# zhuzhui-2000/mobilesuperresolution

Measured on AMD Instinct MI355X. Metric: HR megapixels/sec (WDSR-B x4, 48x48 LR patches), full training step, higher is better.
Workload: dtype bf16; 1 GPU; WDSR-B x4, 16 blocks / 24 units, 48x48 LR patches, batch 32 per GPU, fwd+L1+bwd+Adam; global_batch=32, parallelism=dp1

## Files before the change

include/sr_hotpath.h:

```cpp
#ifndef SR_HOTPATH_H
#define SR_HOTPATH_H
#include <stddef.h>
#include <stdint.h>

#ifdef __cplusplus
extern "C" {
#endif

typedef void* sr_stream_t;

#define SR_DTYPE_F32 0
#define SR_DTYPE_BF16 1

int sr_abi_version(void);

int sr_wdsr_block_fwd(const void* x, void* y, const void* wblob, const float* cinit,
                      int N, int H, int W, int F, int dtype, sr_stream_t stream);

int sr_wdsr_block2_fwd(const void* x, void* ya, void* yb, const void* wblob_a, const void* wblob_b,
                       const float* cinit_a, const float* cinit_b, void* tsave_a, void* tsave_b, int N, int H, int W,
                       int F, int dtype, sr_stream_t stream);

int sr_wdsr_block2_bwd_data(const void* xa, const void* xb, const void* dyb, void* dxb, void* dxa,
                            const void* wblob_a, const void* wblob_b, const float* cinit_a, const float* cinit_b,
                            void* dtsave_a, void* dtsave_b, int N, int H, int W, int F, int dtype, sr_stream_t stream);
int sr_wdsr_block_wgrad_saved(const void* x, const void* dy, const void* tsave, const void* dtsave,
                              const void* wblob, const float* cinit, float* partial_a, float* partial_b, int layers,
                              int wgs, int N, int H, int W, int F, int dtype, long x_ls, long dy_ls, long side_ls,
                              long w_ls, long c_ls, sr_stream_t stream);

int sr_wdsr_fwd_rs(const void* x, void* ya, void* yb, const void* wblob_a, const void* wblob_b, const float* cinit_a,
                   const float* cinit_b, void* tsave_a, void* tsave_b, int nblk, int N, int H, int W, int F, int dtype,
                   sr_stream_t stream);
int sr_wdsr_fwd_rs_repeat(void* x, void* ya, void* yb, const void* wblob_a, const void* wblob_b, const float* cinit_a,
                          const float* cinit_b, void* tsave_a, void* tsave_b, int nblk, int N, int H, int W, int F, int dtype,
                          int reps, sr_stream_t stream);

int sr_wdsr_block_fwd_repeat(void* x, void* y, const void* wblob, const float* cinit,
                             int N, int H, int W, int F, int dtype, int reps, sr_stream_t stream);
int sr_wdsr_block2_fwd_repeat(void* x, void* ya, void* yb, const void* wblob_a, const void* wblob_b,
                              const float* cinit_a, const float* cinit_b, int N, int H, int W, int F, int dtype,
                              int reps, sr_stream_t stream);


int sr_wdsr_block_bwd_data(const void* x, const void* dy, void* dx, const void* wblob, const float* cinit,
                           int N, int H, int W, int F, int dtype, sr_stream_t stream);

int sr_wdsr_block_wgrad(const void* x, const void* dy, const void* wblob, const float* cinit,
                        float* partial_a, float* partial_b, int layers, int wgs_per_layer,
                        int N, int H, int W, int F, int dtype,
                        long x_ls, long dy_ls, long w_ls, long c_ls, sr_stream_t stream);
int sr_wdsr_block_slab_sizes(int F, int* slab_a, int* slab_b);

int sr_head_fwd(const float* x_nchw, void* y, const void* wblob, float mean, int N, int H, int W, int F,
                int dtype, sr_stream_t stream);
int sr_tail_fwd(const void* feat, const float* x_nchw, float* out, const void* wblob, float mean,
                int N, int H, int W, int F, int R, int dtype, sr_stream_t stream);
int sr_tail_bwd_data(const float* dout, void* dfeat, const void* wblob, int N, int H, int W, int F, int R,
                     int dtype, sr_stream_t stream);
int sr_tail_wgrad(const float* dout, const void* feat, const float* x_nchw, float mean, float* partial,
                  int wgs, int N, int H, int W, int F, int R, int dtype, sr_stream_t stream);
int sr_tail_bwd(const float* dout, const void* feat, const float* x, float mean, const void* wblob, void* dfeat,
                float* partial, int wgs, int N, int H, int W, int F, int R, int dtype, sr_stream_t stream);
int sr_head_wgrad(const void* dy0, const float* x_nchw, float mean, float* partial, int wgs,
                  int N, int H, int W, int F, int dtype, sr_stream_t stream);

int sr_c3_fwd(const void* x, const void* res, void* y, const void* wblob, int N, int H, int W, int CI, int act,
              int dtype, sr_stream_t stream);
int sr_c3_bwd_data(const void* dA, const void* A, const void* add, void* dx, const void* wblob, int N, int H,
                   int W, int CI, int act, int dtype, sr_stream_t stream);
int sr_c3_wgrad(const void* x, const void* dA, const void* A, float* partial, int wgs, int N, int H, int W,
                int CI, int act, int dtype, sr_stream_t stream);

typedef struct sr_c3_warp {
  const float* frame; long frame_bs;
  const void* state;
  const float* flow; long flow_bs;
  const float* flow_bound;
  void* dstate;
  float* dflow; long dflow_bs;
  void* x0_save;
} sr_c3_warp_t;

typedef struct sr_c3_unpack {
  const int* sidx0; const int* dst0; int n0;
  const int* sidx1; const int* dst1; int n1;
  float* gflat;
} sr_c3_unpack_t;

int sr_c3_trunk_fwd(const void* x0, const sr_c3_warp_t* warp, void* acts, void* mids, const void* blob,
                    const long* blob_off, int nb, int N, int H, int W, int ci0, int dtype, int n_dir, long blob_dir_stride,
                    sr_stream_t stream);
int sr_c3_trunk_bwd(const void* x0, const sr_c3_warp_t* warp, const void* acts, const void* mids, void* ga, void* gt,
                    const void* blob, const long* blob_off, float* parts, void* dx0, const sr_c3_unpack_t* unpack, int nb,
                    int wgs, int N, int H, int W, int ci0, int dtype, int n_dir, long blob_dir_stride, sr_stream_t stream);

int sr_c64_trunk_fwd(const void* x0, const sr_c3_warp_t* warp, void* ping, void* pong, void* out, const void* blob,
                     const long* blob_off, int nb, int N, int H, int W, int ci0, int dtype, int n_dir, long blob_dir_stride,
                     sr_stream_t stream);

int sr_c64_recon_fwd(const void* feat_b, const void* feat_f, int cw, const float* frame, long frame_bs, const void* blob,
                     const long* blob_off, void* fused, void* up1, void* up2, void* hr, float* out, long out_bs, int N, int H,
                     int W, int dtype, int stages, sr_stream_t stream);

int sr_mv_recon_fwd(const void* const* feat_b, const void* const* feat_f, int cw, const float* x, long x_bs, long x_fs,
                    const void* blob, float* out, long out_bs, long out_fs, void* u_save, int NF, int B, int H, int W, int dtype,
                    sr_stream_t stream);
int sr_mv_recon_bwd(const void* const* feat_b, const void* const* feat_f, const void* u_save, const float* g, long g_bs, long g_fs,
                    const void* blob, void* const* dfeat_b, void* const* dfeat_f, float* parts, int wgs, float* grads, int F, int NF,
                    int B, int H, int W, int dtype, sr_stream_t stream);
int sr_mv_recon_slab(void);

int sr_rm_block_fwd(const void* x, void* y, unsigned* mask, const void* wp, const float* bias, int N, int H, int W, int F, int K,
                    int dtype, sr_stream_t stream);
int sr_rm_block_bwd_data(const void* dy, const unsigned* mask, void* dx, const void* wpt, int N, int H, int W, int F, int K,
                         int dtype, sr_stream_t stream);
int sr_rm_wgrad(const void* g, const unsigned* mask, const void* xin, float* partial, int wgs, int N, int H, int W, int CA, int CB,
                int K, int dtype, sr_stream_t stream);
int sr_rm_tail_fwd(const void* feat, float* out, const void* wp, int N, int H, int W, int F, int R, int K, int dtype,
                   sr_stream_t stream);
int sr_rm_unshuffle(const float* dout, void* dconv, int N, int H, int W, int R, int dtype, sr_stream_t stream);
int sr_rm_tail_bwd_data(const void* dconv, void* dfeat, const void* wpt, int N, int H, int W, int F, int R, int K, int dtype,
                        sr_stream_t stream);

typedef struct sr_patch_rec {
  long lr_off, hr_off;
  int lr_w, hr_w;
  int x, y;
  int flags;
  int pad_;
} sr_patch_rec_t;
int sr_patch_gather(const unsigned char* cache, const void* recs, float* lr_out, float* hr_out, int B, int P, int scale,
                    sr_stream_t stream);

int sr_bicubic_resize_u8(const unsigned char* img, unsigned char* out_u8, float* out_f32, float* src_f32, int H, int W, int scale,
                         const double* wr, const int* ir, int taps_r, const double* wc, const int* ic, int taps_c,
                         sr_stream_t stream);

typedef struct sr_bicubic_rec {
  long hr_off;
  int hr_w;
  int x, y;
  int flags;
} sr_bicubic_rec_t;
int sr_bicubic_patch_gather(const unsigned char* cache, const void* recs, float* lr_out, float* hr_out, int B, int P, int scale,
                            int ig, const double* w, const int* idx, int taps, sr_stream_t stream);

typedef struct sr_clip_rec {
  long ids_off;
  int x, y;
  int flags;
  int T;
} sr_clip_rec_t;
typedef struct sr_clip_frame {
  long lr_off, hr_off;
  long mv_off;
  int lr_w, hr_w;
} sr_clip_frame_t;
int sr_clip_gather(const unsigned char* cache, const float* mv_cache, const void* frames, const int* ids, const void* recs,
                   float* lr_out, float* hr_out, int B, int T, int P, int scale, sr_stream_t stream);

int sr_psnr(const float* sr, const float* hr, float* partial, float* out, int N, int C, int H, int W, int shave, int luma,
            int wgs, sr_stream_t stream);

int sr_ssim(const float* sr, const float* hr, double* partial, double* out, int N, int H, int W, int shave, long n_partial,
            sr_stream_t stream);

int sr_eval_clip(const float* sr, const float* lr, const float* hr, float* partial, float* out, int F, int H, int W, int h,
                 int w, int lr_channels, int shave, int align_corners, int wgs, sr_stream_t stream);

int sr_eval_u8(const float* src, unsigned char* out, int F, int H, int W, int h, int w, int src_channels, int from_lr,
               int align_corners, sr_stream_t stream);

int sr_eval_variation(const float* lr, float* partial, float* out, int B, int N, int C, int h, int w, int wgs,
                      sr_stream_t stream);

int sr_flow_warp_fwd(const float* x, const float* flow, float* out, int N, int C, int H, int W, sr_stream_t stream);
int sr_flow_warp_bwd(const float* x, const float* flow, const float* gout, float* dx, float* dflow, int N, int C,
                     int H, int W, sr_stream_t stream);

int sr_nas_dw_fwd(const void* yin, void* V, const float* dwp, int N, int H, int W, int F, int dtype, sr_stream_t stream);
int sr_nas_pw_fwd(const void* yin, const void* V, void* y, const void* frags, const float* tabs, const float* scal,
                  int N, int H, int W, int F, int dtype, sr_stream_t stream);
int sr_nas_pw_bwd(const void* yin, const void* V, const void* gy, void* GZ, const void* frags, const float* tabs,
                  const float* scal, float* partial, int wgs, int N, int H, int W, int F, int dtype,
                  sr_stream_t stream);
int sr_nas_dw_bwd(const void* yin, const void* GZ, const void* gy, void* gyin, const float* dwp, float* partial,
                  int wgs, int N, int H, int W, int F, int dtype, sr_stream_t stream);
int sr_nas_dw_wgrad(const void* yin, const void* GZ, const float* dwp, float* partial, int wgs, int N, int H, int W,
                    int F, int dtype, sr_stream_t stream);

int sr_nas_scalars(const float* mask_w, const float* split_w, const float* alpha, const float* alpha1, const float* alpha2,
                   int nb, int F, float* out, float* src, long src_stride, int off_mg, float* scal, sr_stream_t stream);
int sr_nas_mask_grads(const float* dsrc, long ds, int off_r, int off_sxy, int off_sA, int off_sB, const float* ms, const float* p,
                      const float* beta, int nb, int F, float* out, sr_stream_t stream);
int sr_nas_body_fwd(void* ys, void* V, const float* dwp, long dwp_bs, const void* frags, long frags_bs, const float* tabs,
                    long tabs_bs, const float* scal, long scal_bs, int nb, int N, int H, int W, int F, int dtype,
                    int split, sr_stream_t stream);
int sr_nas_body_bwd(const void* ys, const void* V, const void* g_out, void* g_tmp0, void* g_tmp1, void* GZ, const float* dwp,
                    long dwp_bs, const void* frags, long frags_bs, const float* tabs, long tabs_bs, const float* scal,
                    long scal_bs, float* part_pw, long pw_bs, float* part_dw, long dw_bs, int wgs, int nb, int N, int H, int W,
                    int F, int dtype, int split, void** g_in, sr_stream_t stream);

typedef struct { const int* idx; void* out; long src_off, src_stride; int n, reps, as_float; } sr_pack_seg_t;
typedef struct { const float* partial; const int* sidx; const int* dst; long dst_off, dst_stride, slab; int wgs, n, reps; } sr_unpack_seg_t;
int sr_param_pack(const float* flat, float* src, const int* chan_tab, int n_chan, const int* bias_tab, const float* bias_const,
                  int n_bias, const sr_pack_seg_t* segs, int nseg, int dtype, sr_stream_t stream);
int sr_param_grads(const float* flat, float* dsrc, float* gflat, const int* chan_tab, int n_chan, const int* bias_tab,
                   int n_bias, const sr_unpack_seg_t* segs, int nseg, sr_stream_t stream);

typedef struct {
  int F, NB, R, dtype, N, H, W;
  float mean;
  const float* flat; float* gflat;
  const int* chan_tab; int n_chan;
  const int* bias_tab; const float* bias_const; int n_bias;
  float* src; float* dsrc;
  long src_head_off, src_body_off, src_body_stride, src_tail_off;
  const int* idx_head; int n_idx_head;
  const int* idx_body; int n_idx_body;
  const int* idx_cinit; int n_idx_cinit;
  const int* idx_tail; int n_idx_tail;
  void* blob_head; void* blob_body; float* cinit_body; void* blob_tail;
  float* part_a; float* part_b; float* part_tail; float* part_head;
  int wgs_body, wgs_tail, wgs_head;
  int slab_a, slab_b, slab_tail, slab_head;
  const int* ga_sidx; const int* ga_dst; int n_ga;
  const int* gb_sidx; const int* gb_dst; int n_gb;
  const int* gt_sidx; const int* gt_dst; int n_gt;
  const int* gh_sidx; const int* gh_dst; int n_gh;
  const float* x; void* acts; void* grads; float* out; const float* dout;
  void* tsave; void* dtsave;
  const float* hr; int loss_kind; float loss_gscale; float* loss_part;
  int nb_split, chan_split, bias_split;
  int adam_in_wn_bwd;
  int one_block32;
} sr_wdsr_net_t;

#define SR_NET_SAVE_ACTS 1
#define SR_NET_WEIGHTS_PACKED 2
#define SR_NET_PACK_ONLY 4
#define SR_NET_SKIP_TAIL 8
int sr_wdsr_net_forward(const sr_wdsr_net_t* net, int flags, sr_stream_t stream);
int sr_wdsr_net_backward(const sr_wdsr_net_t* net, sr_stream_t stream);
int sr_wdsr_net_backward_part(const sr_wdsr_net_t* net, int part, sr_stream_t stream);

int sr_pixel_shuffle(const float* in, float* out, int N, int C, int H, int W, int r, int inverse, sr_stream_t stream);

int sr_tail_bwd_loss(const float* sr, const float* hr, int loss_kind, float gscale, float* loss_part, const void* feat,
                     const float* x_nchw, float mean, const void* wblob, void* dfeat, float* partial, int wgs, int N, int H,
                     int W, int F, int R, int dtype, sr_stream_t stream);

int sr_tail_train(const float* hr, int loss_kind, float gscale, float* loss_part, const void* feat, const float* x_nchw, float mean,
                  const void* wblob, void* dfeat, float* partial, int wgs, int N, int H, int W, int F, int R, int dtype,
                  sr_stream_t stream);

typedef struct { float w_lerp, beta2, one_minus_beta2, bc2_sqrt, eps, neg_step_size; } sr_adam_t;
int sr_adam_step(float* param, const float* grad, float* exp_avg, float* exp_avg_sq, long n, const sr_adam_t* a,
                 const float* loss_part, int n_loss, float loss_scale, float* loss_out, sr_stream_t stream);
int sr_loss_value(const float* loss_part, int n_loss, float loss_scale, float* loss_out, sr_stream_t stream);
int sr_scale_by(void* y, const void* x, long n, const float* scale, int dtype, sr_stream_t stream);
int sr_wdsr_net_train_step(const sr_wdsr_net_t* net, float* exp_avg, float* exp_avg_sq, long n_params, const sr_adam_t* a,
                           float loss_scale, float* loss_out, sr_stream_t stream);

int sr_conv7_fwd(const void* x, const void* wpacked, const float* bias, void* y, int N, int H, int W, int CIN, int COUT, int relu,
                 int out_f32, sr_stream_t stream);

#define SR_FN_ENCODER 1
#define SR_FN_BLOCKS 2
#define SR_FN_LAST 4
#define SR_FN_UP 8
#define SR_FN_WRITE_D 16
#define SR_FN_ALL 15
int sr_fn_net_fwd(const float* frames, const void* blob, const long* conv_off, const void* head_blob, void* s0, void* s1, void* s2,
                  float* out, long out_is, int nb, int N, int H, int W, int dtype, int stages, sr_stream_t stream);

int sr_probe_mfma_bf16(const void* a_frag, const void* b_frag, float* acc_out, sr_stream_t stream);
int sr_probe_mfma_f32(const float* a_frag, const float* b_frag, float* acc_out, sr_stream_t stream);
int sr_probe_tr_read(const void* img_bf16, int n_elems, const int* lane_elem_off, void* out_bf16x4,
                     sr_stream_t stream);
int sr_probe_copy(const void* src, void* dst, size_t n_bytes, sr_stream_t stream);
int sr_probe_launch_floor(void* out, int gx, int gy, int threads, int lds_bytes, int reps, sr_stream_t stream);
int sr_probe_launch_floor_graph(void* out, int gx, int gy, int threads, int lds_bytes, int reps, int iters,
                                float* us_per_launch, float* host_us_per_graph );
int sr_debug_set_stamps(void* buf, long n_workgroups);

#ifdef __cplusplus
}
#endif
#endif
```

mobilesuperresolution_amd/_lib.py:

```python
from __future__ import annotations

import ctypes
import os
from ctypes import c_int, c_size_t, c_void_p

import torch

_HERE = os.path.dirname(os.path.abspath(__file__))
LIB_PATH = os.environ.get("SR_HOTPATH_LIB_PATH") or os.path.join(
    _HERE, "libsr_hotpath_dbg.so" if os.environ.get("SR_HOTPATH_DEBUG_LIB") == "1" else "libsr_hotpath.so")
ABI_VERSION = 23
DTYPE_CODE = {torch.float32: 0, torch.bfloat16: 1}
_HOT_DTYPES = {"fp32": torch.float32, "float32": torch.float32, "bf16": torch.bfloat16, "bfloat16": torch.bfloat16}


def hot_dtype(name=None) -> torch.dtype:
    name = name or os.environ.get("SR_HOT_DTYPE", "fp32")
    return name if isinstance(name, torch.dtype) else _HOT_DTYPES[str(name).lower()]


_P, _I, _Z, _L, _F = c_void_p, c_int, c_size_t, ctypes.c_long, ctypes.c_float
SIGNATURES = {
    "sr_abi_version": ([], _I),
    "sr_wdsr_block_fwd": ([_P, _P, _P, _P, _I, _I, _I, _I, _I, _P], _I),
    "sr_wdsr_block2_fwd": ([_P] * 9 + [_I] * 5 + [_P], _I),
    "sr_wdsr_fwd_rs": ([_P] * 9 + [_I] * 6 + [_P], _I),
    "sr_conv7_fwd": ([_P] * 4 + [_I] * 7 + [_P], _I),
    "sr_wdsr_fwd_rs_repeat": ([_P] * 9 + [_I] * 7 + [_P], _I),
    "sr_wdsr_block_wgrad_saved": ([_P] * 8 + [_I] * 7 + [_L] * 5 + [_P], _I),
    "sr_wdsr_block2_bwd_data": ([_P] * 11 + [_I] * 5 + [_P], _I),
    "sr_wdsr_block2_fwd_repeat": ([_P] * 7 + [_I] * 6 + [_P], _I),
    "sr_probe_launch_floor": ([_P, _I, _I, _I, _I, _I, _P], _I),
    "sr_probe_launch_floor_graph": ([_P, _I, _I, _I, _I, _I, _I, _P, _P], _I),
    "sr_debug_set_stamps": ([_P, _L], _I),
    "sr_c3_trunk_fwd": ([_P] * 6 + [_I] * 7 + [_L, _P], _I),
    "sr_c3_trunk_bwd": ([_P] * 11 + [_I] * 8 + [_L, _P], _I),
    "sr_c64_trunk_fwd": ([_P] * 7 + [_I] * 7 + [_L, _P], _I),
    "sr_c64_recon_fwd": ([_P, _P, _I, _P, _L, _P, _P, _P, _P, _P, _P, _P, _L] + [_I] * 5 + [_P], _I),
    "sr_mv_recon_fwd": ([_P, _P, _I, _P, _L, _L, _P, _P, _L, _L, _P] + [_I] * 5 + [_P], _I),
    "sr_mv_recon_bwd": ([_P, _P, _P, _P, _L, _L, _P, _P, _P, _P, _I, _P] + [_I] * 6 + [_P], _I),
    "sr_mv_recon_slab": ([], _I),
    "sr_tail_bwd": ([_P, _P, _P, _F, _P, _P, _P] + [_I] * 7 + [_P], _I),
    "sr_nas_dw_wgrad": ([_P, _P, _P, _P, _I, _I, _I, _I, _I, _I, _P], _I),
    "sr_wdsr_block_fwd_repeat": ([_P, _P, _P, _P, _I, _I, _I, _I, _I, _I, _P], _I),
    "sr_wdsr_block_bwd_data": ([_P, _P, _P, _P, _P, _I, _I, _I, _I, _I, _P], _I),
    "sr_wdsr_block_wgrad": ([_P, _P, _P, _P, _P, _P, _I, _I, _I, _I, _I, _I, _I, _L, _L, _L, _L, _P], _I),
    "sr_wdsr_block_slab_sizes": ([_I, _P, _P], _I),
    "sr_head_fwd": ([_P, _P, _P, _F, _I, _I, _I, _I, _I, _P], _I),
    "sr_tail_fwd": ([_P, _P, _P, _P, _F, _I, _I, _I, _I, _I, _I, _P], _I),
    "sr_tail_bwd_data": ([_P, _P, _P, _I, _I, _I, _I, _I, _I, _P], _I),
    "sr_tail_wgrad": ([_P, _P, _P, _F, _P, _I, _I, _I, _I, _I, _I, _I, _P], _I),
    "sr_head_wgrad": ([_P, _P, _F, _P, _I, _I, _I, _I, _I, _I, _P], _I),
    "sr_c3_fwd": ([_P, _P, _P, _P, _I, _I, _I, _I, _I, _I, _P], _I),
    "sr_c3_bwd_data": ([_P, _P, _P, _P, _P, _I, _I, _I, _I, _I, _I, _P], _I),
    "sr_c3_wgrad": ([_P, _P, _P, _P, _I, _I, _I, _I, _I, _I, _I, _P], _I),
    "sr_flow_warp_fwd": ([_P, _P, _P, _I, _I, _I, _I, _P], _I),
    "sr_flow_warp_bwd": ([_P, _P, _P, _P, _P, _I, _I, _I, _I, _P], _I),
    "sr_nas_dw_fwd": ([_P, _P, _P, _I, _I, _I, _I, _I, _P], _I),
    "sr_nas_pw_fwd": ([_P, _P, _P, _P, _P, _P, _I, _I, _I, _I, _I, _P], _I),
    "sr_nas_pw_bwd": ([_P, _P, _P, _P, _P, _P, _P, _P, _I, _I, _I, _I, _I, _I, _P], _I),
    "sr_nas_dw_bwd": ([_P, _P, _P, _P, _P, _P, _I, _I, _I, _I, _I, _I, _P], _I),
    "sr_patch_gather": ([_P, _P, _P, _P, _I, _I, _I, _P], _I),
    "sr_clip_gather": ([_P] * 7 + [_I] * 4 + [_P], _I),
    "sr_bicubic_resize_u8": ([_P] * 4 + [_I] * 3 + [_P, _P, _I, _P, _P, _I, _P], _I),
    "sr_bicubic_patch_gather": ([_P] * 4 + [_I] * 4 + [_P, _P, _I, _P], _I),
    "sr_param_pack": ([_P, _P, _P, _I, _P, _P, _I, _P, _I, _I, _P], _I),
    "sr_param_grads": ([_P, _P, _P, _P, _I, _P, _I, _P, _I, _P], _I),
    "sr_nas_scalars": ([_P] * 5 + [_I, _I, _P, _P, _L, _I, _P, _P], _I),
    "sr_nas_mask_grads": ([_P, _L, _I, _I, _I, _I, _P, _P, _P, _I, _I, _P, _P], _I),
    "sr_nas_body_fwd": ([_P, _P, _P, _L, _P, _L, _P, _L, _P, _L] + [_I] * 7 + [_P], _I),
    "sr_nas_body_bwd": ([_P] * 7 + [_L, _P, _L, _P, _L, _P, _L, _P, _L, _P, _L] + [_I] * 8 + [_P, _P], _I),
    "sr_psnr": ([_P, _P, _P, _P] + [_I] * 7 + [_P], _I),
    "sr_ssim": ([_P, _P, _P, _P] + [_I] * 4 + [_L, _P], _I),
    "sr_eval_clip": ([_P] * 5 + [_I] * 9 + [_P], _I),
    "sr_eval_u8": ([_P, _P] + [_I] * 8 + [_P], _I),
    "sr_eval_variation": ([_P] * 3 + [_I] * 6 + [_P], _I),
    "sr_pixel_shuffle": ([_P, _P, _I, _I, _I, _I, _I, _I, _P], _I),
    "sr_tail_bwd_loss": ([_P, _P, _I, _F, _P, _P, _P, _F, _P, _P, _P] + [_I] * 7 + [_P], _I),
    "sr_tail_train": ([_P, _I, _F, _P, _P, _P, _F, _P, _P, _P] + [_I] * 7 + [_P], _I),
    "sr_adam_step": ([_P, _P, _P, _P, _L, _P, _P, _I, _F, _P, _P], _I),
    "sr_loss_value": ([_P, _I, _F, _P, _P], _I),
    "sr_scale_by": ([_P, _P, _L, _P, _I, _P], _I),
    "sr_wdsr_net_train_step": ([_P, _P, _P, _L, _P, _F, _P, _P], _I),
    "sr_wdsr_net_forward": ([_P, _I, _P], _I),
    "sr_wdsr_net_backward": ([_P, _P], _I),
    "sr_wdsr_net_backward_part": ([_P, _I, _P], _I),
    "sr_probe_mfma_bf16": ([_P, _P, _P, _P], _I),
    "sr_probe_mfma_f32": ([_P, _P, _P, _P], _I),
    "sr_probe_tr_read": ([_P, _I, _P, _P, _P], _I),
    "sr_probe_copy": ([_P, _P, _Z, _P], _I),
    "sr_rm_block_fwd": ([_P] * 5 + [_I] * 6 + [_P], _I),
    "sr_rm_block_bwd_data": ([_P] * 4 + [_I] * 6 + [_P], _I),
    "sr_rm_wgrad": ([_P] * 4 + [_I] * 8 + [_P], _I),
    "sr_rm_tail_fwd": ([_P] * 3 + [_I] * 7 + [_P], _I),
    "sr_rm_unshuffle": ([_P, _P] + [_I] * 5 + [_P], _I),
    "sr_rm_tail_bwd_data": ([_P] * 3 + [_I] * 7 + [_P], _I),
    "sr_fn_net_fwd": ([_P] * 8 + [_L] + [_I] * 6 + [_P], _I),
}

class WdsrNet(ctypes.Structure):
    _fields_ = (
        [(n, _I) for n in ("F", "NB", "R", "dtype", "N", "H", "W")] + [("mean", _F)] +
        [("flat", _P), ("gflat", _P), ("chan_tab", _P), ("n_chan", _I),
         ("bias_tab", _P), ("bias_const", _P), ("n_bias", _I), ("src", _P), ("dsrc", _P)] +
        [(n, _L) for n in ("src_head_off", "src_body_off", "src_body_stride", "src_tail_off")] +
        [("idx_head", _P), ("n_idx_head", _I), ("idx_body", _P), ("n_idx_body", _I),
         ("idx_cinit", _P), ("n_idx_cinit", _I), ("idx_tail", _P), ("n_idx_tail", _I),
         ("blob_head", _P), ("blob_body", _P), ("cinit_body", _P), ("blob_tail", _P),
         ("part_a", _P), ("part_b", _P), ("part_tail", _P), ("part_head", _P)] +
        [(n, _I) for n in ("wgs_body", "wgs_tail", "wgs_head", "slab_a", "slab_b", "slab_tail", "slab_head")] +
        [("ga_sidx", _P), ("ga_dst", _P), ("n_ga", _I), ("gb_sidx", _P), ("gb_dst", _P), ("n_gb", _I),
         ("gt_sidx", _P), ("gt_dst", _P), ("n_gt", _I), ("gh_sidx", _P), ("gh_dst", _P), ("n_gh", _I),
         ("x", _P), ("acts", _P), ("grads", _P), ("out", _P), ("dout", _P), ("tsave", _P), ("dtsave", _P),
         ("hr", _P), ("loss_kind", _I), ("loss_gscale", _F), ("loss_part", _P),
         ("nb_split", _I), ("chan_split", _I), ("bias_split", _I), ("adam_in_wn_bwd", _I),
         ("one_block32", _I)])


class C3Warp(ctypes.Structure):
    _fields_ = [("frame", _P), ("frame_bs", _L), ("state", _P), ("flow", _P), ("flow_bs", _L), ("flow_bound", _P),
                ("dstate", _P), ("dflow", _P), ("dflow_bs", _L), ("x0_save", _P)]


class C3Unpack(ctypes.Structure):
    _fields_ = [("sidx0", _P), ("dst0", _P), ("n0", _I), ("sidx1", _P), ("dst1", _P), ("n1", _I), ("gflat", _P)]


class PackSeg(ctypes.Structure):
    _fields_ = [("idx", _P), ("out", _P), ("src_off", _L), ("src_stride", _L), ("n", _I), ("reps", _I), ("as_float", _I)]


class UnpackSeg(ctypes.Structure):
    _fields_ = [("partial", _P), ("sidx", _P), ("dst", _P), ("dst_off", _L), ("dst_stride", _L), ("slab", _L), ("wgs", _I),
                ("n", _I), ("reps", _I)]


class AdamScalars(ctypes.Structure):
    _fields_ = [(n, _F) for n in ("w_lerp", "beta2", "one_minus_beta2", "bc2_sqrt", "eps", "neg_step_size")]


_lib = None


class HotpathError(RuntimeError):
    pass


def _declare(lib):
    for name, (args, res) in SIGNATURES.items():
        fn = getattr(lib, name)
        fn.argtypes = args
        fn.restype = res


def lib():
    global _lib
    if _lib is None:
        if not os.path.exists(LIB_PATH):
            raise HotpathError(
                f"{LIB_PATH} not found: build it with `python -m mobilesuperresolution_amd.build` "
                "(the SR hot path has no CPU / ATen fallback)")
        if os.environ.get("SR_HOTPATH_LIB_PATH") or os.environ.get("SR_HOTPATH_DEBUG_LIB") == "1":
            import warnings
            warnings.warn(f"SR hot path: loading a NON-DEFAULT library ({LIB_PATH}) because SR_HOTPATH_LIB_PATH / "
                          "SR_HOTPATH_DEBUG_LIB is set (meant for tools/ only)", RuntimeWarning, stacklevel=2)
        l = ctypes.CDLL(LIB_PATH)
        _declare(l)
        if l.sr_abi_version() != ABI_VERSION:
            raise HotpathError(f"libsr_hotpath ABI {l.sr_abi_version()} != expected {ABI_VERSION}; rebuild")
        _lib = l
    return _lib


def stream_ptr(device=None) -> int:
    return torch.cuda.current_stream(device).cuda_stream


class _NoGuard:
    __slots__ = ()

    def __enter__(self):
        return self

    def __exit__(self, *exc):
        return False


_NOGUARD = _NoGuard()


def device_guard(device):
    idx = device.index
    if idx is None or idx == torch.cuda.current_device():
        return _NOGUARD
    return torch.cuda.device(idx)


def check(rc: int, what: str):
    if rc != 0:
        kind = {-1: "unsupported geometry/dtype", -2: "bad argument"}.get(rc, f"hipError_t {rc}")
        raise HotpathError(f"{what} failed: {kind}")


def ptr(t: torch.Tensor) -> int:
    if not t.is_cuda:
        raise HotpathError("SR hot path needs device tensors (no CPU fallback)")
    if not t.is_contiguous():
        raise HotpathError("SR hot path needs contiguous tensors")
    return t.data_ptr()


class KernelTimer:

    def __init__(self):
        self.events = {}

    def run(self, name, fn, *args):
        e0, e1 = torch.cuda.Event(enable_timing=True), torch.cuda.Event(enable_timing=True)
        e0.record()
        rc = fn(*args)
        e1.record()
        self.events.setdefault(name, []).append((e0, e1))
        return rc

    def summary(self):
        torch.cuda.synchronize()
        return {k: (len(v), sum(a.elapsed_time(b) for a, b in v) / len(v)) for k, v in self.events.items()}


_TIMER = None


def set_timer(t):
    global _TIMER
    _TIMER = t


def launch(name, fn, *args):
    rc = fn(*args) if _TIMER is None else _TIMER.run(name, fn, *args)
    check(rc, name)
```

mobilesuperresolution_amd/csrc/sr_abi.hip:

```cpp
#include <algorithm>
#include <cmath>
#include "../../include/sr_hotpath.h"
#include "wdsr_block.h"
#include "wdsr_fwd_rs.h"
#include "wdsr_fwd_stream.h"
#include "wdsr_bwd_rs.h"
#include "wdsr_bwd_pair_lds.h"
#include "wdsr_wgrad_rs.h"
#include "wdsr_ends.h"
#include "wdsr_prep.h"
#include "conv3x3.h"
#include "conv64.h"
#include "vsr_recon.h"
#include "mv_recon.h"
#include "spynet_conv.h"
#include "nas_block.h"
#include "nas_dw_lc.h"
#include "nas_bwd_fused.h"
#include "flow_warp.h"
#include "metrics.h"
#include "ssim.h"
#include "eval.h"
#include "patches.h"
#include "clips.h"
#include "bicubic.h"
#include "train_step.h"
#include "pixel_shuffle.h"
#include "result_block.h"
#include "frame_net.h"

extern "C" int sr_abi_version(void) { return 23; }

namespace {

template <int F_, int E_, int L_>
struct WdsrDimsOf {
  static constexpr int F = F_, E = E_, L = L_;
  typedef BlockCfg<F_, E_, L_> Cfg;
};
template <int F> struct WdsrDims;
template <> struct WdsrDims<24> : WdsrDimsOf<24, 144, 20> {};
template <> struct WdsrDims<32> : WdsrDimsOf<32, 192, 26> {};

template <typename Fn>
int dispatch_f(int F, Fn&& fn) {
  if (F == 24) return fn(WdsrDims<24>{});
  if (F == 32) return fn(WdsrDims<32>{});
  return -1;
}
template <typename Fn>
int dispatch_ft(int F, int dtype, Fn&& fn) {
  return dispatch_f(F, [&](auto d) {
    if (dtype == SR_DTYPE_BF16) return fn(d, __bf16{});
    if (dtype == SR_DTYPE_F32) return fn(d, float{});
    return -1;
  });
}

struct Tiles { int x, y; };
template <typename C = WdsrDims<24>::Cfg>
Tiles block_tiles(int H, int W) {
  return Tiles{(W + C::TW - 1) / C::TW, (H + C::TH - 1) / C::TH};
}

template <typename T, int F>
int launch_block_fwd(const void* x, void* y, const void* wblob, const float* cinit, int N, int H, int W,
                     hipStream_t st, void* tsave = nullptr) {
  typedef typename WdsrDims<F>::Cfg C;
  const auto [tiles_x, tiles_y] = block_tiles<C>(H, W);
  dim3 grid(tiles_x * tiles_y, N), block(64 * C::NPT_H);
  hipLaunchKernelGGL((wdsr_block_fwd_kernel<T, F, C::E, C::L>), grid, block, 0, st, (const T*)x, (T*)y, (const T*)wblob,
                     cinit, H, W, tiles_x, (T*)tsave);
  SR_HIP_CHECK_LAUNCH();
  return 0;
}

template <typename T, int F>
int launch_block_bwd_data(const void* x, const void* dy, void* dx, const void* wblob, const float* cinit, int N,
                          int H, int W, hipStream_t st, void* dtsave = nullptr) {
  typedef typename WdsrDims<F>::Cfg C;
  const auto [tiles_x, tiles_y] = block_tiles<C>(H, W);
  dim3 grid(tiles_x * tiles_y, N), block(64 * C::NPT_O);
  hipLaunchKernelGGL((wdsr_block_bwd_data_kernel<T, F, C::E, C::L>), grid, block, 0, st, (const T*)x, (const T*)dy, (T*)dx,
                     (const T*)wblob, cinit, H, W, tiles_x, (T*)dtsave);
  SR_HIP_CHECK_LAUNCH();
  return 0;
}

template <typename T, int F>
int launch_block_wgrad(const void* x, const void* dy, const void* wblob, const float* cinit, float* pa, float* pb,
                       int layers, int wgs, int N, int H, int W, long x_ls, long dy_ls, long w_ls, long c_ls,
                       hipStream_t st) {
  typedef typename WdsrDims<F>::Cfg C;
  const auto [tiles_x, tiles_y] = block_tiles<C>(H, W);
  dim3 grid(wgs, layers);
  hipLaunchKernelGGL((wdsr_block_wgrad_kernel<T, F, C::E, C::L, 0>), grid, dim3(64 * WgradCfg<F, C::E, C::L, 0>::NWAVES), 0, st,
                     (const T*)x, (const T*)dy, (const T*)wblob, cinit, pa, N, H, W, tiles_x, tiles_x * tiles_y, x_ls,
                     dy_ls, w_ls, c_ls);
  hipLaunchKernelGGL((wdsr_block_wgrad_kernel<T, F, C::E, C::L, 1>), grid, dim3(64 * WgradCfg<F, C::E, C::L, 1>::NWAVES), 0, st,
                     (const T*)x, (const T*)dy, (const T*)wblob, cinit, pb, N, H, W, tiles_x, tiles_x * tiles_y, x_ls,
                     dy_ls, w_ls, c_ls);
  SR_HIP_CHECK_LAUNCH();
  return 0;
}

}

static bool fwd_stream_applies(long N, int H, int W) {
  if (W != 48 || H % 4 != 0 || H < 8 || H > 4096 || N < 256) return false;
  const long rounds = (N + 255) / 256;
  return N * 10 >= rounds * 256 * 7;
}

template <int F, int NBLK>
static int launch_fwd_rs16(const void* x, void* ya, void* yb, const void* wa, const void* wb, const float* cia, const float* cib,
                           void* tsa, void* tsb, int N, int H, int W, hipStream_t st) {
  typedef typename WdsrDims<F>::Cfg C;
  typedef __bf16 T;
  constexpr int E = C::E, L = C::L;
  const auto [tiles_x, tiles_y] = block_tiles<C>(H, W);
  if (tsa && (NBLK == 1 || tsb))
    hipLaunchKernelGGL((wdsr_fwd_rs16_kernel<F, E, L, NBLK, true>), dim3(tiles_x * tiles_y, N), dim3(1024), 0, st, (const T*)x, (T*)ya,
                       (T*)yb, (const T*)wa, (const T*)wb, cia, cib, (T*)tsa, (T*)tsb, H, W, tiles_x);
  else
    hipLaunchKernelGGL((wdsr_fwd_rs16_kernel<F, E, L, NBLK, false>), dim3(tiles_x * tiles_y, N), dim3(1024), 0, st, (const T*)x, (T*)ya,
                       (T*)yb, (const T*)wa, (const T*)wb, cia, cib, (T*)tsa, (T*)tsb, H, W, tiles_x);
  SR_HIP_CHECK_LAUNCH();
  return 0;
}

template <int F, int NBLK>
static int launch_fwd_rs(const void* x, void* ya, void* yb, const void* wa, const void* wb, const float* cia, const float* cib,
                         void* tsa, void* tsb, int N, int H, int W, hipStream_t st) {
  typedef typename WdsrDims<F>::Cfg C;
  typedef __bf16 T;
  constexpr int E = C::E, L = C::L;
  const auto [tiles_x, tiles_y] = block_tiles<C>(H, W);
  constexpr int persist_from = 768;
  const long total = (long)N * tiles_x * tiles_y;
  if constexpr (NBLK == 2) {
    if (fwd_stream_applies(N, H, W)) {
      if (tsa && tsb)
        hipLaunchKernelGGL((wdsr_fwd_stream12_kernel<F, E, L, true>), dim3(256), dim3(768), 0, st, (const T*)x, (T*)ya, (T*)yb, (const T*)wa,
                           (const T*)wb, cia, cib, (T*)tsa, (T*)tsb, N, H);
      else
        hipLaunchKernelGGL((wdsr_fwd_stream12_kernel<F, E, L, false>), dim3(256), dim3(768), 0, st, (const T*)x, (T*)ya, (T*)yb, (const T*)wa,
                           (const T*)wb, cia, cib, (T*)nullptr, (T*)nullptr, N, H);
      SR_HIP_CHECK_LAUNCH();
      return 0;
    }
  }
  if (total >= persist_from && total < (1L << 31)) {
    const int wgs = 256;
    const bool save = tsa && (NBLK == 1 || tsb);
    if (save && NBLK == 1) {
      hipLaunchKernelGGL((wdsr_fwd_rs_persist_kernel<F, E, L, 1, true>), dim3(wgs), dim3(512), 0, st, (const T*)x, (T*)ya, (T*)yb,
                         (const T*)wa, (const T*)wb, cia, cib, (T*)tsa, (T*)tsb, N, H, W, tiles_x, tiles_x * tiles_y);
      SR_HIP_CHECK_LAUNCH();
      return 0;
    }
    if constexpr (NBLK == 2) {
      if (!save) {
        hipLaunchKernelGGL((wdsr_fwd_rs_pipe_kernel<F, E, L>), dim3(wgs), dim3(512), 0, st, (const T*)x, (T*)ya, (T*)yb, (const T*)wa,
                           (const T*)wb, cia, cib, N, H, W, tiles_x, tiles_x * tiles_y);
        SR_HIP_CHECK_LAUNCH();
        return 0;
      }
    } else if (!save) {
      hipLaunchKernelGGL((wdsr_fwd_rs_persist_kernel<F, E, L, 1, false>), dim3(wgs), dim3(512), 0, st, (const T*)x, (T*)ya, (T*)yb,
                         (const T*)wa, (const T*)wb, cia, cib, (T*)tsa, (T*)tsb, N, H, W, tiles_x, tiles_x * tiles_y);
      SR_HIP_CHECK_LAUNCH();
      return 0;
    }
  }
  if (tsa && (NBLK == 1 || tsb))
    hipLaunchKernelGGL((wdsr_fwd_rs_kernel<F, E, L, NBLK, true>), dim3(tiles_x * tiles_y, N), dim3(512), 0, st, (const T*)x, (T*)ya,
                       (T*)yb, (const T*)wa, (const T*)wb, cia, cib, (T*)tsa, (T*)tsb, H, W, tiles_x);
  else
    hipLaunchKernelGGL((wdsr_fwd_rs_kernel<F, E, L, NBLK, false>), dim3(tiles_x * tiles_y, N), dim3(512), 0, st, (const T*)x, (T*)ya,
                       (T*)yb, (const T*)wa, (const T*)wb, cia, cib, (T*)tsa, (T*)tsb, H, W, tiles_x);
  SR_HIP_CHECK_LAUNCH();
  return 0;
}
template <int F, int NBLK>
static int launch_fwd_rs_any(const void* x, void* ya, void* yb, const void* wa, const void* wb, const float* cia, const float* cib,
                             void* tsa, void* tsb, int N, int H, int W, hipStream_t st) {
  if constexpr (F == 24) return launch_fwd_rs<F, NBLK>(x, ya, yb, wa, wb, cia, cib, tsa, tsb, N, H, W, st);
  else return launch_fwd_rs16<F, NBLK>(x, ya, yb, wa, wb, cia, cib, tsa, tsb, N, H, W, st);
}
extern "C" int sr_wdsr_fwd_rs(const void* x, void* ya, void* yb, const void* wa, const void* wb, const float* cia,
                              const float* cib, void* tsa, void* tsb, int nblk, int N, int H, int W, int F, int dtype,
                              sr_stream_t stream) {
  if (!x || !yb || !wa || !cia || N <= 0 || H <= 0 || W <= 0 || N > 65535 || (nblk == 2 && (!wb || !cib))) return -2;
  if (dtype != SR_DTYPE_BF16) return -1;
  hipStream_t st = (hipStream_t)stream;
  return dispatch_f(F, [&](auto d) {
    if (nblk == 2) return launch_fwd_rs_any<decltype(d)::F, 2>(x, ya, yb, wa, wb, cia, cib, tsa, tsb, N, H, W, st);
    if (nblk == 1) return launch_fwd_rs_any<decltype(d)::F, 1>(x, nullptr, yb, wa, nullptr, cia, nullptr, tsa, nullptr, N, H, W, st);
    return -1;
  });
}
extern "C" int sr_wdsr_block2_fwd(const void* x, void* ya, void* yb, const void* wa, const void* wb, const float* cia,
                                  const float* cib, void* tsa, void* tsb, int N, int H, int W, int F, int dtype,
                                  sr_stream_t stream) {
  if (F != 24 && F != 32) return (!x || !yb || !wa || !wb || !cia || !cib || N <= 0 || H <= 0 || W <= 0 || N > 65535) ? -2 : -1;
  return sr_wdsr_fwd_rs(x, ya, yb, wa, wb, cia, cib, tsa, tsb, 2, N, H, W, F, dtype, stream);
}
extern "C" int sr_wdsr_fwd_rs_repeat(void* x, void* ya, void* yb, const void* wa, const void* wb, const float* cia,
                                     const float* cib, void* tsa, void* tsb, int nblk, int N, int H, int W, int F, int dtype,
                                     int reps, sr_stream_t stream) {
  for (int i = 0; i < reps; ++i) {
    const int rc = (i & 1) ? sr_wdsr_fwd_rs(yb, ya, x, wa, wb, cia, cib, tsa, tsb, nblk, N, H, W, F, dtype, stream)
                           : sr_wdsr_fwd_rs(x, ya, yb, wa, wb, cia, cib, tsa, tsb, nblk, N, H, W, F, dtype, stream);
    if (rc) return rc;
  }
  return 0;
}

extern "C" int sr_wdsr_block_fwd_repeat(void* x, void* y, const void* wblob, const float* cinit, int N, int H, int W,
                                        int F, int dtype, int reps, sr_stream_t stream) {
  for (int i = 0; i < reps; ++i) {
    const int rc = (i & 1) ? sr_wdsr_block_fwd(y, x, wblob, cinit, N, H, W, F, dtype, stream)
                           : sr_wdsr_block_fwd(x, y, wblob, cinit, N, H, W, F, dtype, stream);
    if (rc) return rc;
  }
  return 0;
}

extern "C" int sr_wdsr_block2_fwd_repeat(void* x, void* ya, void* yb, const void* wa, const void* wb, const float* cia,
                                         const float* cib, int N, int H, int W, int F, int dtype, int reps,
                                         sr_stream_t stream) {
  for (int i = 0; i < reps; ++i) {
    const int rc = (i & 1) ? sr_wdsr_block2_fwd(yb, ya, x, wa, wb, cia, cib, nullptr, nullptr, N, H, W, F, dtype, stream)
                           : sr_wdsr_block2_fwd(x, ya, yb, wa, wb, cia, cib, nullptr, nullptr, N, H, W, F, dtype, stream);
    if (rc) return rc;
  }
  return 0;
}

extern "C" int sr_wdsr_block_bwd_data(const void* x, const void* dy, void* dx, const void* wblob,
                                      const float* cinit, int N, int H, int W, int F, int dtype,
                                      sr_stream_t stream) {
  if (!x || !dy || !dx || !wblob || !cinit || N <= 0 || H <= 0 || W <= 0 || N > 65535) return -2;
  return dispatch_ft(F, dtype, [&](auto d, auto t) {
    return launch_block_bwd_data<decltype(t), decltype(d)::F>(x, dy, dx, wblob, cinit, N, H, W, (hipStream_t)stream);
  });
}

extern "C" int sr_wdsr_block2_bwd_data(const void* xa, const void* xb, const void* dyb, void* dxb, void* dxa,
                                       const void* wa, const void* wb, const float* cia, const float* cib, void* dta,
                                       void* dtb, int N, int H, int W, int F, int dtype, sr_stream_t stream) {
  if (!xa || !xb || !dyb || !dxb || !dxa || !wa || !wb || !cia || !cib || N <= 0 || H <= 0 || W <= 0 || N > 65535)
    return -2;
  if ((F != 24 && F != 32) || dtype != SR_DTYPE_BF16) return -1;
  const auto [tiles_x, tiles_y] = block_tiles(H, W);
  if (F == 32) {
    typedef WdsrDims<32> D;
    hipLaunchKernelGGL((wdsr_bwd_pair_lds_kernel<32, D::E, D::L>), dim3(tiles_x * tiles_y, N), dim3(BwdPairCfg<32, D::E, D::L>::NTHREADS),
                       0, (hipStream_t)stream, (const __bf16*)xa, (const __bf16*)xb, (const __bf16*)dyb, (__bf16*)dxb, (__bf16*)dxa,
                       (const __bf16*)wa, (const __bf16*)wb, cia, cib, (__bf16*)dta, (__bf16*)dtb, H, W, tiles_x);
  } else {
    typedef WdsrDims<24> D;
    hipLaunchKernelGGL((wdsr_bwd_rs_kernel<24, D::E, D::L>), dim3(tiles_x * tiles_y, N), dim3(512), 0, (hipStream_t)stream,
                       (const __bf16*)xa, (const __bf16*)xb, (const __bf16*)dyb, (__bf16*)dxb, (__bf16*)dxa, (const __bf16*)wa,
                       (const __bf16*)wb, (__bf16*)dta, (__bf16*)dtb, H, W, tiles_x);
  }
  SR_HIP_CHECK_LAUNCH();
  return 0;
}

extern "C" int sr_wdsr_block_wgrad(const void* x, const void* dy, const void* wblob, const float* cinit,
                                   float* pa, float* pb, int layers, int wgs, int N, int H, int W, int F,
                                   int dtype, long x_ls, long dy_ls, long w_ls, long c_ls, sr_stream_t stream) {
  if (!x || !dy || !wblob || !cinit || !pa || !pb || layers <= 0 || wgs <= 0 || N <= 0 || H <= 0 || W <= 0 ||
      layers > 65535)
    return -2;
  return dispatch_ft(F, dtype, [&](auto d, auto t) {
    return launch_block_wgrad<decltype(t), decltype(d)::F>(x, dy, wblob, cinit, pa, pb, layers, wgs, N, H, W, x_ls, dy_ls, w_ls, c_ls,
                                                           (hipStream_t)stream);
  });
}

namespace {
template <int F>
int launch_wgrad_saved(const void* x, const void* dy, const void* tsave, const void* dtsave, const void* wblob,
                       const float* cinit, float* pa, float* pb, int layers, int wgs, int N, int H, int W, long x_ls,
                       long dy_ls, long side_ls, long w_ls, long c_ls, hipStream_t st) {
  typedef typename WdsrDims<F>::Cfg C;
  typedef __bf16 T;
  constexpr int E = C::E, L = C::L;
  const auto [tiles_x, tiles_y] = block_tiles<C>(H, W);
  dim3 grid(wgs, layers);
  const bool old_a = (long)N * tiles_x * tiles_y * C::TH * C::TW >= (1L << 31);
  if constexpr (F == 24) {
    if (!old_a)
      hipLaunchKernelGGL((wdsr_wgrad_a8_kernel<F, E, L>), grid, dim3(WgradA8Cfg<F, E, L>::NTHREADS), 0, st, (const T*)x, (const T*)dtsave,
                         (const T*)wblob, pa, N, H, W, tiles_x, tiles_x * tiles_y, x_ls, side_ls, w_ls);
  }
  if (F != 24 || old_a)
    hipLaunchKernelGGL((wdsr_block_wgrad_saved_kernel<T, F, E, L, 0>), grid, dim3(64 * WgradSavedCfg<F, E, L>::NWAVES), 0, st,
                       (const T*)x, (const T*)dtsave, (const T*)wblob, cinit, pa, N, H, W, tiles_x, tiles_x * tiles_y, x_ls,
                       side_ls, w_ls, c_ls);
  hipLaunchKernelGGL((wdsr_wgrad_b8_kernel<F, E, L>), grid, dim3(WgradB8Cfg<F, E, L>::NTHREADS), 0, st, (const T*)dy, (const T*)tsave,
                     pb, N, H, W, tiles_x, tiles_x * tiles_y, dy_ls, side_ls);
  SR_HIP_CHECK_LAUNCH();
  return 0;
}
}

extern "C" int sr_wdsr_block_wgrad_saved(const void* x, const void* dy, const void* tsave, const void* dtsave,
                                         const void* wblob, const float* cinit, float* pa, float* pb, int layers, int wgs,
                                         int N, int H, int W, int F, int dtype, long x_ls, long dy_ls, long side_ls,
                                         long w_ls, long c_ls, sr_stream_t stream) {
  if (!x || !dy || !tsave || !dtsave || !wblob || !cinit || !pa || !pb || layers <= 0 || wgs <= 0 || N <= 0 || H <= 0 ||
      W <= 0 || layers > 65535)
    return -2;
  if (dtype != SR_DTYPE_BF16) return -1;
  return dispatch_f(F, [&](auto d) {
    return launch_wgrad_saved<decltype(d)::F>(x, dy, tsave, dtsave, wblob, cinit, pa, pb, layers, wgs, N, H, W, x_ls, dy_ls, side_ls,
                                                  w_ls, c_ls, (hipStream_t)stream);
  });
}

extern "C" int sr_wdsr_block_slab_sizes(int F, int* slab_a, int* slab_b) {
  if (!slab_a || !slab_b) return -2;
  return dispatch_f(F, [&](auto d) {
    typedef BwdCfg<typename decltype(d)::Cfg> B;
    *slab_a = B::SLAB_A;
    *slab_b = B::SLAB_B;
    return 0;
  });
}

extern "C" int sr_wdsr_block_fwd(const void* x, void* y, const void* wblob, const float* cinit, int N, int H,
                                 int W, int F, int dtype, sr_stream_t stream) {
  if (!x || !y || !wblob || !cinit || N <= 0 || H <= 0 || W <= 0 || N > 65535) return -2;
  return dispatch_ft(F, dtype, [&](auto d, auto t) {
    return launch_block_fwd<decltype(t), decltype(d)::F>(x, y, wblob, cinit, N, H, W, (hipStream_t)stream);
  });
}

namespace {
template <typename E> dim3 tile_grid(int N, int H, int W, int* tiles_x) {
  *tiles_x = (W + E::TW - 1) / E::TW;
  return dim3(*tiles_x * ((H + E::TH - 1) / E::TH), N);
}
#define SR_DISPATCH_TF(CALL)                                                     \
  if (F == 24 && dtype == SR_DTYPE_BF16) { CALL(__bf16, 24) }                    \
  else if (F == 24 && dtype == SR_DTYPE_F32) { CALL(float, 24) }                 \
  else if (F == 32 && dtype == SR_DTYPE_BF16) { CALL(__bf16, 32) }               \
  else if (F == 32 && dtype == SR_DTYPE_F32) { CALL(float, 32) }                 \
  else return -1;
#define SR_DISPATCH_R(CALL, T, F_)                                               \
  if (R == 4) { CALL(T, F_, 4) } else if (R == 2) { CALL(T, F_, 2) } else if (R == 3) { CALL(T, F_, 3) } else return -1;
// ... 556 lines not shown

extern "C" int sr_flow_warp_fwd(const float* x, const float* flow, float* out, int N, int C, int H, int W,
                                sr_stream_t stream) {
  if (!x || !flow || !out || N <= 0 || C <= 0 || H <= 0 || W <= 0 || N > 65535) return -2;
  const int blocks = std::min((H * W + 15) / 16, 8192);
  hipLaunchKernelGGL(flow_warp_fwd_kernel, dim3(blocks, N), dim3(64), 0, (hipStream_t)stream, x, flow, out, C, H, W);
  SR_HIP_CHECK_LAUNCH();
  return 0;
}
extern "C" int sr_flow_warp_bwd(const float* x, const float* flow, const float* gout, float* dx, float* dflow, int N,
                                int C, int H, int W, sr_stream_t stream) {
  if (!x || !flow || !gout || N <= 0 || C <= 0 || H <= 0 || W <= 0 || N > 65535) return -2;
  const int blocks = std::min((H * W + 15) / 16, 8192);
  hipLaunchKernelGGL(flow_warp_bwd_kernel, dim3(blocks, N), dim3(64), 0, (hipStream_t)stream, x, flow, gout, dx, dflow,
                     C, H, W);
  SR_HIP_CHECK_LAUNCH();
  return 0;
}

#define SR_NAS_DISPATCH(CALL)                                                                   \
  if (F == 24 && dtype == SR_DTYPE_BF16) { CALL(__bf16, 24) } else if (F == 24 && dtype == SR_DTYPE_F32) { CALL(float, 24) } \
  else if (F == 32 && dtype == SR_DTYPE_BF16) { CALL(__bf16, 32) } else if (F == 32 && dtype == SR_DTYPE_F32) { CALL(float, 32) } \
  else return -1;
#define SR_NAS_DISPATCH_F32(CALL)                                                               \
  if (F == 24 && dtype == SR_DTYPE_F32) { CALL(float, 24) } else if (F == 32 && dtype == SR_DTYPE_F32) { CALL(float, 32) } \
  else return -1;

extern "C" int sr_nas_dw_fwd(const void* yin, void* V, const float* dwp, int N, int H, int W, int F, int dtype,
                             sr_stream_t stream) {
  if (!yin || !V || !dwp || N <= 0 || H <= 0 || W <= 0 || N > 65535) return -2;
  hipStream_t st = (hipStream_t)stream;
  const long vs = (long)N * H * W * F;
  if (dtype == SR_DTYPE_BF16) {
    typedef NasCfg<24> C;
    const int tx = (W + C::TW - 1) / C::TW;
    dim3 g(tx * ((H + C::TH - 1) / C::TH), N);
    if (F == 24) hipLaunchKernelGGL((nas_dw_fwd_lc_kernel<24>), g, dim3(512), 0, st, (const __bf16*)yin, (__bf16*)V, dwp, H, W, tx, vs);
    else if (F == 32) hipLaunchKernelGGL((nas_dw_fwd_lc_kernel<32>), g, dim3(512), 0, st, (const __bf16*)yin, (__bf16*)V, dwp, H, W, tx, vs);
    else return -1;
    SR_HIP_CHECK_LAUNCH();
    return 0;
  }
#define CALL(T, F_) { typedef NasCfg<F_> C; const int tx = (W + C::TW - 1) / C::TW; dim3 g(tx * ((H + C::TH - 1) / C::TH), N); \
    hipLaunchKernelGGL((nas_dw_fwd_kernel<T, F_>), g, dim3(512), 0, st, (const T*)yin, (T*)V, dwp, H, W, tx, vs); }
  SR_NAS_DISPATCH_F32(CALL)
#undef CALL
  SR_HIP_CHECK_LAUNCH();
  return 0;
}
extern "C" int sr_nas_pw_fwd(const void* yin, const void* V, void* y, const void* frags, const float* tabs,
                             const float* scal, int N, int H, int W, int F, int dtype, sr_stream_t stream) {
  if (!yin || !V || !y || !frags || !tabs || !scal || N <= 0 || H <= 0 || W <= 0 || N > 65535) return -2;
  hipStream_t st = (hipStream_t)stream;
  const long vs = (long)N * H * W * F;
#define CALL(T, F_) { typedef NasCfg<F_> C; const int tx = (W + C::TW - 1) / C::TW; dim3 g(tx * ((H + C::TH - 1) / C::TH), N); \
    hipLaunchKernelGGL((nas_pw_fwd_kernel<T, F_>), g, dim3(576), 0, st, (const T*)yin, (const T*)V, (T*)y, (const T*)frags, tabs, scal, H, W, tx, vs); }
  SR_NAS_DISPATCH(CALL)
#undef CALL
  SR_HIP_CHECK_LAUNCH();
  return 0;
}
extern "C" int sr_nas_pw_bwd(const void* yin, const void* V, const void* gy, void* GZ, const void* frags,
                             const float* tabs, const float* scal, float* partial, int wgs, int N, int H, int W, int F,
                             int dtype, sr_stream_t stream) {
  if (!yin || !V || !gy || !GZ || !frags || !tabs || !scal || !partial || wgs <= 0 || N <= 0 || H <= 0 || W <= 0) return -2;
  hipStream_t st = (hipStream_t)stream;
  const long vs = (long)N * H * W * F;
#define CALL(T, F_) { typedef NasCfg<F_> C; const int tx = (W + C::TW - 1) / C::TW, tpi = tx * ((H + C::TH - 1) / C::TH); \
    hipLaunchKernelGGL((nas_pw_bwd_kernel<T, F_>), dim3(wgs), dim3(NasPwb<T>::THREADS), 0, st, (const T*)yin, (const T*)V, (const T*)gy, (T*)GZ, (const T*)frags, tabs, scal, partial, N, H, W, tx, tpi, vs); }
  SR_NAS_DISPATCH(CALL)
#undef CALL
  SR_HIP_CHECK_LAUNCH();
  return 0;
}
extern "C" int sr_nas_dw_bwd(const void* yin, const void* GZ, const void* gy, void* gyin, const float* dwp,
                             float* partial, int wgs, int N, int H, int W, int F, int dtype, sr_stream_t stream) {
  if (!yin || !GZ || !gy || !gyin || !dwp || !partial || wgs <= 0 || N <= 0 || H <= 0 || W <= 0) return -2;
  hipStream_t st = (hipStream_t)stream;
  const long vs = (long)N * H * W * F;
  if (dtype == SR_DTYPE_BF16) {
    typedef NasCfg<24> C;
    const int tx = (W + C::TW - 1) / C::TW, tpi = tx * ((H + C::TH - 1) / C::TH);
    if (F == 24) hipLaunchKernelGGL((nas_dw_bwd_lc_kernel<24>), dim3(wgs), dim3(NAS_DW_BWD_THREADS), 0, st, (const __bf16*)yin, (const __bf16*)GZ, (const __bf16*)gy, (__bf16*)gyin, dwp, partial, N, H, W, tx, tpi, vs);
    else if (F == 32) hipLaunchKernelGGL((nas_dw_bwd_lc_kernel<32>), dim3(wgs), dim3(NAS_DW_BWD_THREADS), 0, st, (const __bf16*)yin, (const __bf16*)GZ, (const __bf16*)gy, (__bf16*)gyin, dwp, partial, N, H, W, tx, tpi, vs);
    else return -1;
    SR_HIP_CHECK_LAUNCH();
    return 0;
  }
#define CALL(T, F_) { typedef NasCfg<F_> C; const int tx = (W + C::TW - 1) / C::TW, tpi = tx * ((H + C::TH - 1) / C::TH); \
    hipLaunchKernelGGL((nas_dw_bwd_kernel<T, F_>), dim3(wgs), dim3(512), 0, st, (const T*)yin, (const T*)GZ, (const T*)gy, (T*)gyin, dwp, partial, N, H, W, tx, tpi, vs); }
  SR_NAS_DISPATCH_F32(CALL)
#undef CALL
  SR_HIP_CHECK_LAUNCH();
  return 0;
}

extern "C" int sr_nas_dw_wgrad(const void* yin, const void* GZ, const float* dwp, float* partial, int wgs, int N, int H,
                               int W, int F, int dtype, sr_stream_t stream) {
  if (!yin || !GZ || !dwp || !partial || wgs <= 0 || N <= 0 || H <= 0 || W <= 0) return -2;
  hipStream_t st = (hipStream_t)stream;
  const long vs = (long)N * H * W * F;
  if (dtype == SR_DTYPE_BF16) {
    typedef NasCfg<24> C;
    const int tx = (W + C::TW - 1) / C::TW, tpi = tx * ((H + C::TH - 1) / C::TH);
    if (F == 24) hipLaunchKernelGGL((nas_dw_wgrad3_kernel<24>), dim3(wgs), dim3(768), 0, st, (const __bf16*)yin, (const __bf16*)GZ, dwp, partial, N, H, W, tx, tpi, vs);
    else if (F == 32) hipLaunchKernelGGL((nas_dw_wgrad3_kernel<32>), dim3(wgs), dim3(768), 0, st, (const __bf16*)yin, (const __bf16*)GZ, dwp, partial, N, H, W, tx, tpi, vs);
    else return -1;
    SR_HIP_CHECK_LAUNCH();
    return 0;
  }
#define CALL(T, F_) { typedef NasCfg<F_> C; const int tx = (W + C::TW - 1) / C::TW, tpi = tx * ((H + C::TH - 1) / C::TH); \
    hipLaunchKernelGGL((nas_dw_wgrad_kernel<T, F_>), dim3(wgs, 3), dim3(768), 0, st, (const T*)yin, (const T*)GZ, dwp, partial, N, H, W, tx, tpi, vs); }
  SR_NAS_DISPATCH_F32(CALL)
#undef CALL
  SR_HIP_CHECK_LAUNCH();
  return 0;
}

namespace {
template <typename T> int net_pack(const sr_wdsr_net_t* n, hipStream_t st) {
  const int cb = (n->n_chan + 3) / 4, bb = (n->n_bias + 255) / 256;
  hipLaunchKernelGGL(wn_src_kernel, dim3(cb + bb), dim3(256), 0, st, n->flat, n->src, (const int4*)n->chan_tab,
                     n->n_chan, n->bias_tab, n->bias_const, n->n_bias, cb);
  PackSegs ps;
  ps.nseg = 4;
  int blk = 0;
  auto add = [&](int k, const int* idx, void* out, long off, long stride, int cnt, int reps, int as_float) {
    ps.s[k] = PackSeg{idx, out, off, stride, cnt, reps, as_float, blk};
    blk += reps * ((cnt + 255) / 256);
  };
  add(0, n->idx_head, n->blob_head, n->src_head_off, 0, n->n_idx_head, 1, 0);
  add(1, n->idx_body, n->blob_body, n->src_body_off, n->src_body_stride, n->n_idx_body, n->NB, 0);
  add(2, n->idx_cinit, n->cinit_body, n->src_body_off, n->src_body_stride, n->n_idx_cinit, n->NB, 1);
  add(3, n->idx_tail, n->blob_tail, n->src_tail_off, 0, n->n_idx_tail, 1, 0);
  hipLaunchKernelGGL((pack_all_kernel<T>), dim3(blk), dim3(256), 0, st, n->src, ps);
  SR_HIP_CHECK_LAUNCH();
  return 0;
}
}

static bool net_saves_side_images(const sr_wdsr_net_t* n, bool backward) {
  return (n->F == 24 || n->F == 32) && n->dtype == SR_DTYPE_BF16 && n->tsave && (!backward || n->dtsave);
}
static long net_tiles(const sr_wdsr_net_t* n) {
  const Tiles t = block_tiles(n->H, n->W);
  return (long)n->N * t.x * t.y;
}
static bool net_uses_pairs(const sr_wdsr_net_t* n) {
  return n->dtype == SR_DTYPE_BF16 && net_tiles(n) <= 384 && (n->F == 24 || (n->F == 32 && !n->one_block32));
}
static bool net_step_fuses_tail(const sr_wdsr_net_t* n) {
  return n->dtype == SR_DTYPE_BF16 && n->R == 4 && (n->F == 24 || n->F == 32) && n->hr && n->N <= 65535;
}
static size_t side_image_bytes(const sr_wdsr_net_t* n) {
  typedef WdsrDims<24>::Cfg C;
  const Tiles t = block_tiles<C>(n->H, n->W);
  const int lp = n->F == 24 ? C::LP : WdsrDims<32>::Cfg::LP;
  return (size_t)n->N * ((size_t)t.x * t.y) * C::TH * C::TW * lp * 2;
}
struct NetView {
  const sr_wdsr_net_t* n;
  bool keeps_side;
  size_t esz = n->dtype == SR_DTYPE_BF16 ? 2 : 4;
  size_t act_bytes = (size_t)n->N * n->H * n->W * n->F * esz, blob_bytes = (size_t)n->n_idx_body * esz;
  size_t side_bytes = side_image_bytes(n);
  char* act(int i) const { return (char*)n->acts + (size_t)i * act_bytes; }
  char* grad(int i) const { return (char*)n->grads + (size_t)i * act_bytes; }
  char* blob(int i) const { return (char*)n->blob_body + (size_t)i * blob_bytes; }
  const float* cinit(int i) const { return n->cinit_body + (size_t)i * n->n_idx_cinit; }
  char* tsave(int i) const { return keeps_side ? (char*)n->tsave + (size_t)i * side_bytes : nullptr; }
  char* dtsave(int i) const { return keeps_side ? (char*)n->dtsave + (size_t)i * side_bytes : nullptr; }
};

extern "C" int sr_wdsr_net_forward(const sr_wdsr_net_t* n, int flags, sr_stream_t stream) {
  if (!n || !n->flat || !n->src) return -2;
  if (!(flags & SR_NET_PACK_ONLY) && (!n->x || !n->acts || !n->out)) return -2;
  hipStream_t st = (hipStream_t)stream;
  const int save_acts = flags & SR_NET_SAVE_ACTS;
  int rc = 0;
  if (!(flags & SR_NET_WEIGHTS_PACKED)) rc = n->dtype == SR_DTYPE_BF16 ? net_pack<__bf16>(n, st) : net_pack<float>(n, st);
  if (rc || (flags & SR_NET_PACK_ONLY)) return rc;
  const NetView v{n, save_acts && net_saves_side_images(n, false)};
  char* acts = v.act(0);
  if ((rc = sr_head_fwd(n->x, acts, n->blob_head, n->mean, n->N, n->H, n->W, n->F, n->dtype, stream))) return rc;
  char* cur = acts;
  const bool pairs = net_uses_pairs(n) || (n->F == 24 && n->dtype == SR_DTYPE_BF16 &&
                                           ((!save_acts && net_tiles(n) >= 768) || fwd_stream_applies(n->N, n->H, n->W)));
  for (int i = 0, nb; i < n->NB; i += nb) {
    nb = pairs && i + 1 < n->NB ? 2 : 1;
    char* nxt = save_acts ? v.act(i + nb) : (cur == acts ? v.act(1) : acts);
    if (nb == 2)
      rc = sr_wdsr_block2_fwd(cur, save_acts ? v.act(i + 1) : nullptr, nxt, v.blob(i), v.blob(i + 1), v.cinit(i), v.cinit(i + 1),
                              v.tsave(i), v.tsave(i + 1), n->N, n->H, n->W, n->F, n->dtype, stream);
    else if (pairs)
      rc = sr_wdsr_fwd_rs(cur, nullptr, nxt, v.blob(i), nullptr, v.cinit(i), nullptr, v.tsave(i), nullptr, 1, n->N, n->H, n->W, n->F,
                          n->dtype, stream);
    else if (v.keeps_side)
      rc = dispatch_f(n->F, [&](auto d) {
        return launch_block_fwd<__bf16, decltype(d)::F>(cur, nxt, v.blob(i), v.cinit(i), n->N, n->H, n->W, st, v.tsave(i));
      });
    else
      rc = sr_wdsr_block_fwd(cur, nxt, v.blob(i), v.cinit(i), n->N, n->H, n->W, n->F, n->dtype, stream);
    if (rc) return rc;
    cur = nxt;
  }
  if (flags & SR_NET_SKIP_TAIL) return 0;
  return sr_tail_fwd(cur, n->x, n->out, n->blob_tail, n->mean, n->N, n->H, n->W, n->F, n->R, n->dtype, stream);
}

namespace {
struct FusedAdam { float* m; float* v; AdamArgs a; const float* loss_part; int n_loss; float loss_scale; float* loss_out; };
}
static int net_backward_part_impl(const sr_wdsr_net_t* n, int part, sr_stream_t stream, const FusedAdam* fa, bool tail_train = false) {
  if (!n || !n->flat || !n->gflat || !n->dsrc || !n->x || !n->acts || !n->grads || part < 0 || part > 2) return -2;
  if (tail_train && (part != 0 || !n->hr)) return -2;
  if (part != 2 && (n->hr ? ((!n->out && !tail_train) || !n->loss_part || (n->loss_kind != 1 && n->loss_kind != 2)) : !n->dout)) return -2;
  hipStream_t st = (hipStream_t)stream;
  const long act_e = (long)n->N * n->H * n->W * n->F;
  const bool pairs = net_uses_pairs(n);
  const bool saved = net_saves_side_images(n, true);
  const NetView v{n, saved};
  int split = part == 0 ? 0 : n->nb_split;
  if (part != 0 && (split <= 0 || split >= n->NB || (pairs && ((n->NB - split) & 1)))) return -2;
  const int b0 = part == 1 ? split : 0, b1 = part == 2 ? split : n->NB;
  int rc;
  if (part != 2) {
    if (tail_train)
      rc = sr_tail_train(n->hr, n->loss_kind, n->loss_gscale, n->loss_part, v.act(n->NB), n->x, n->mean, n->blob_tail, v.grad(n->NB),
                         n->part_tail, n->wgs_tail, n->N, n->H, n->W, n->F, n->R, n->dtype, stream);
    else if (n->hr)
      rc = sr_tail_bwd_loss(n->out, n->hr, n->loss_kind, n->loss_gscale, n->loss_part, v.act(n->NB), n->x, n->mean, n->blob_tail,
                            v.grad(n->NB), n->part_tail, n->wgs_tail, n->N, n->H, n->W, n->F, n->R, n->dtype, stream);
    else if (n->dtype == SR_DTYPE_BF16)
      rc = sr_tail_bwd(n->dout, v.act(n->NB), n->x, n->mean, n->blob_tail, v.grad(n->NB), n->part_tail, n->wgs_tail, n->N, n->H, n->W,
                       n->F, n->R, n->dtype, stream);
    else if (!(rc = sr_tail_bwd_data(n->dout, v.grad(n->NB), n->blob_tail, n->N, n->H, n->W, n->F, n->R, n->dtype, stream)))
      rc = sr_tail_wgrad(n->dout, v.act(n->NB), n->x, n->mean, n->part_tail, n->wgs_tail, n->N, n->H, n->W, n->F, n->R, n->dtype,
                         stream);
    if (rc) return rc;
  }
  for (int i = b1 - 1, nb; i >= b0; i -= nb) {
    nb = pairs && i >= b0 + 1 ? 2 : 1;
    if (nb == 2)
      rc = sr_wdsr_block2_bwd_data(v.act(i - 1), v.act(i), v.grad(i + 1), v.grad(i), v.grad(i - 1), v.blob(i - 1), v.blob(i),
                                   v.cinit(i - 1), v.cinit(i), v.dtsave(i - 1), v.dtsave(i), n->N, n->H, n->W, n->F, n->dtype, stream);
    else if (saved)
      rc = dispatch_f(n->F, [&](auto d) {
        return launch_block_bwd_data<__bf16, decltype(d)::F>(v.act(i), v.grad(i + 1), v.grad(i), v.blob(i), v.cinit(i), n->N, n->H,
                                                                 n->W, st, v.dtsave(i));
      });
    else
      rc = sr_wdsr_block_bwd_data(v.act(i), v.grad(i + 1), v.grad(i), v.blob(i), v.cinit(i), n->N, n->H, n->W, n->F, n->dtype, stream);
    if (rc) return rc;
  }
  const int nl = b1 - b0;
  const int wgs_part = nl > 0 ? (n->wgs_body * n->NB) / nl : 0;
  if (nl > 0) {
    float* pa0 = n->part_a;
    float* pb0 = n->part_b;
    if (saved)
      rc = sr_wdsr_block_wgrad_saved(v.act(b0), v.grad(b0 + 1), v.tsave(b0), v.dtsave(b0), v.blob(b0), v.cinit(b0), pa0, pb0, nl,
                                     wgs_part, n->N, n->H, n->W, n->F, n->dtype, act_e, act_e, (long)(v.side_bytes / v.esz),
                                     (long)n->n_idx_body, (long)n->n_idx_cinit, stream);
    else
      rc = sr_wdsr_block_wgrad(v.act(b0), v.grad(b0 + 1), v.blob(b0), v.cinit(b0), pa0, pb0, nl, wgs_part, n->N, n->H, n->W, n->F,
                               n->dtype, act_e, act_e, (long)n->n_idx_body, (long)n->n_idx_cinit, stream);
    if (rc) return rc;
  }
  if (part != 1)
    if ((rc = sr_head_wgrad(v.grad(0), n->x, n->mean, n->part_head, n->wgs_head, n->N, n->H, n->W, n->F, n->dtype, stream)))
      return rc;
  {
    UnpackSegs us;
    us.nseg = 0;
    int blk = 0;
    auto add = [&](const float* part_, const int* sidx, const int* dst, long off, long stride, long slab, int wgs, int cnt,
                   int reps) {
      us.s[us.nseg++] = UnpackSeg{part_, sidx, dst, off, stride, slab, wgs, cnt, reps, blk};
      blk += reps * unpack_blocks(cnt, wgs);
    };
    if (nl > 0) {
      add(n->part_a, n->ga_sidx, n->ga_dst, n->src_body_off + b0 * n->src_body_stride, n->src_body_stride, n->slab_a, wgs_part,
          n->n_ga, nl);
      add(n->part_b, n->gb_sidx, n->gb_dst, n->src_body_off + b0 * n->src_body_stride, n->src_body_stride, n->slab_b, wgs_part,
          n->n_gb, nl);
    }
    if (part != 2) add(n->part_tail, n->gt_sidx, n->gt_dst, n->src_tail_off, 0, n->slab_tail, n->wgs_tail, n->n_gt, 1);
    if (part != 1) add(n->part_head, n->gh_sidx, n->gh_dst, n->src_head_off, 0, n->slab_head, n->wgs_head, n->n_gh, 1);
    hipLaunchKernelGGL(unpack_all_kernel, dim3(blk), dim3(64 * UNPACK_Q), 0, st, n->dsrc, us);
  }
  const int c0 = part == 1 ? n->chan_split : 0, c1 = part == 2 ? n->chan_split : n->n_chan;
  const int d0 = part == 1 ? n->bias_split : 0, d1 = part == 2 ? n->bias_split : n->n_bias;
  const int cb = (c1 - c0 + 3) / 4, bb = (d1 - d0 + 255) / 256;
  if (fa)
    hipLaunchKernelGGL(wn_bwd_adam_kernel, dim3(cb + bb), dim3(256), 0, st, const_cast<float*>(n->flat), n->dsrc, n->gflat, fa->m, fa->v,
                       (const int4*)n->chan_tab + c0, c1 - c0, n->bias_tab + 3 * d0, d1 - d0, cb, fa->a, fa->loss_part, fa->n_loss,
                       fa->loss_scale, fa->loss_out);
  else
    hipLaunchKernelGGL(wn_bwd_kernel, dim3(cb + bb), dim3(256), 0, st, n->flat, n->dsrc, n->gflat, (const int4*)n->chan_tab + c0,
                       c1 - c0, n->bias_tab + 3 * d0, d1 - d0, cb);
  SR_HIP_CHECK_LAUNCH();
  return 0;
}
extern "C" int sr_wdsr_net_backward_part(const sr_wdsr_net_t* n, int part, sr_stream_t stream) {
  return net_backward_part_impl(n, part, stream, nullptr);
}

extern "C" int sr_wdsr_net_backward(const sr_wdsr_net_t* n, sr_stream_t stream) { return sr_wdsr_net_backward_part(n, 0, stream); }

extern "C" int sr_param_pack(const float* flat, float* src, const int* chan_tab, int n_chan, const int* bias_tab,
                             const float* bias_const, int n_bias, const sr_pack_seg_t* segs, int nseg, int dtype,
                             sr_stream_t stream) {
  if (!flat || !src || !chan_tab || n_chan <= 0 || n_bias < 0 || (n_bias > 0 && (!bias_tab || !bias_const)) || !segs || nseg < 1 ||
      nseg > 4 || (dtype != SR_DTYPE_F32 && dtype != SR_DTYPE_BF16))
    return -2;
  hipStream_t st = (hipStream_t)stream;
  const int cb = (n_chan + 3) / 4, bb = (n_bias + 255) / 256;
  hipLaunchKernelGGL(wn_src_kernel, dim3(cb + bb), dim3(256), 0, st, flat, src, (const int4*)chan_tab, n_chan, bias_tab, bias_const,
                     n_bias, cb);
  PackSegs ps;
  ps.nseg = nseg;
  int blk = 0;
  for (int k = 0; k < nseg; ++k) {
    const sr_pack_seg_t& g = segs[k];
    if (!g.idx || !g.out || g.n <= 0 || g.reps <= 0) return -2;
    ps.s[k] = PackSeg{g.idx, g.out, g.src_off, g.src_stride, g.n, g.reps, g.as_float, blk};
    blk += g.reps * ((g.n + 255) / 256);
  }
  if (dtype == SR_DTYPE_BF16) hipLaunchKernelGGL((pack_all_kernel<__bf16>), dim3(blk), dim3(256), 0, st, src, ps);
  else hipLaunchKernelGGL((pack_all_kernel<float>), dim3(blk), dim3(256), 0, st, src, ps);
  SR_HIP_CHECK_LAUNCH();
  return 0;
}

extern "C" int sr_param_grads(const float* flat, float* dsrc, float* gflat, const int* chan_tab, int n_chan, const int* bias_tab,
                              int n_bias, const sr_unpack_seg_t* segs, int nseg, sr_stream_t stream) {
  if (!flat || !dsrc || !gflat || !chan_tab || n_chan <= 0 || n_bias < 0 || (n_bias > 0 && !bias_tab) || !segs || nseg < 1 || nseg > 4)
    return -2;
  hipStream_t st = (hipStream_t)stream;
  UnpackSegs us;
  us.nseg = nseg;
  int blk = 0;
  for (int k = 0; k < nseg; ++k) {
    const sr_unpack_seg_t& g = segs[k];
    if (!g.partial || !g.sidx || !g.dst || g.n <= 0 || g.reps <= 0 || g.wgs <= 0) return -2;
    us.s[k] = UnpackSeg{g.partial, g.sidx, g.dst, g.dst_off, g.dst_stride, g.slab, g.wgs, g.n, g.reps, blk};
    blk += g.reps * unpack_blocks(g.n, g.wgs);
  }
  hipLaunchKernelGGL(unpack_all_kernel, dim3(blk), dim3(64 * UNPACK_Q), 0, st, dsrc, us);
  const int cb = (n_chan + 3) / 4, bb = (n_bias + 255) / 256;
  hipLaunchKernelGGL(wn_bwd_kernel, dim3(cb + bb), dim3(256), 0, st, flat, dsrc, gflat, (const int4*)chan_tab, n_chan, bias_tab,
                     n_bias, cb);
  SR_HIP_CHECK_LAUNCH();
  return 0;
}

extern "C" int sr_nas_scalars(const float* mask_w, const float* split_w, const float* alpha, const float* alpha1,
                              const float* alpha2, int nb, int F, float* out, float* src, long src_stride, int off_mg, float* scal,
                              sr_stream_t stream) {
  if (!mask_w || !split_w || !alpha || !alpha1 || !alpha2 || !out || nb <= 0 || F < 8 || (src && (src_stride <= 0 || off_mg < 0)))
    return -2;
  if ((long)(nb + 1) * F > NAS_SCALARS_MAX) return -1;
  hipLaunchKernelGGL(nas_scalars_kernel, dim3(1), dim3(1024), 0, (hipStream_t)stream, mask_w, split_w, alpha, alpha1, alpha2, nb,
                     F, out, src, src_stride, off_mg, scal);
  SR_HIP_CHECK_LAUNCH();
  return 0;
}

extern "C" int sr_nas_mask_grads(const float* dsrc, long ds, int off_r, int off_sxy, int off_sA, int off_sB, const float* ms,
                                 const float* p, const float* beta, int nb, int F, float* out, sr_stream_t stream) {
  if (!dsrc || !ms || !p || !beta || !out || nb <= 0 || nb > 1024 || F <= 0 || ds <= 0) return -2;
  hipLaunchKernelGGL(nas_mask_grads_kernel, dim3(1), dim3(1024), 0, (hipStream_t)stream, dsrc, ds, off_r, off_sxy, off_sA, off_sB, ms,
                     p, beta, nb, F, out);
  SR_HIP_CHECK_LAUNCH();
  return 0;
}

extern "C" int sr_nas_body_fwd(void* ys, void* V, const float* dwp, long dwp_bs, const void* frags, long frags_bs, const float* tabs,
                               long tabs_bs, const float* scal, long scal_bs, int nb, int N, int H, int W, int F, int dtype,
                               int split, sr_stream_t stream) {
  if (!ys || !V || !dwp || !frags || !tabs || !scal || nb <= 0 || N <= 0 || H <= 0 || W <= 0) return -2;
  const size_t act = (size_t)N * H * W * F * (dtype == SR_DTYPE_BF16 ? 2 : 4);
  const bool fused = dtype == SR_DTYPE_BF16 && (F == 24 || F == 32) && N <= 65535 && !split;
  for (int i = 0; i < nb; ++i) {
    char* yi = (char*)ys + (size_t)i * act;
    char* Vi = (char*)V + (size_t)i * 3 * act;
    int rc;
    if (fused) {
      typedef NasCfg<24> C;
      const int tx = (W + C::TW - 1) / C::TW;
      const dim3 g(tx * ((H + C::TH - 1) / C::TH), N);
      const long vs = (long)N * H * W * F;
      const float* dw_i = (const float*)((const char*)dwp + (size_t)i * dwp_bs);
      const __bf16* fr_i = (const __bf16*)((const char*)frags + (size_t)i * frags_bs);
      const float* tb_i = (const float*)((const char*)tabs + (size_t)i * tabs_bs);
      const float* sc_i = (const float*)((const char*)scal + (size_t)i * scal_bs);
// ... 608 lines not shown
```

mobilesuperresolution_amd/csrc/wdsr_bwd_rs.h:

```cpp
#pragma once
#include <type_traits>
#include "wdsr_fwd_rs.h"

template <int F_, int E_, int L_> struct BwdRsCfg {
  typedef BlockCfg<F_, E_, L_> C;
  typedef BwdCfg<C> B;
  static constexpr int NW = 8, NTHREADS = 64 * NW;
  static constexpr int rw(int k) { return C::TW + 2 * (2 - k); }
  static constexpr int rh(int k) { return C::TH + 2 * (2 - k); }
  static constexpr int np(int k) { return rw(k) * rh(k); }
  static constexpr int npad(int k) { return (np(k) + 31) / 32 * 32; }
  static constexpr int KXL = C::F;
  static constexpr int DTL = 24;
  static_assert(C::F == 24 && C::L <= DTL && C::FOLD_B1, "24 units");
  static constexpr int PXP = 63 / C::FC;
  static constexpr int pieces(int npx) { return (npx + PXP - 1) / PXP; }
  static constexpr int dma_bytes(int npx) { return pieces(npx) * PXP * C::FC * 16 + 16; }
  static constexpr int DY_ELEMS = npad(0) * KXL;
  static constexpr int DT_ELEMS = npad(1) * DTL;
  static constexpr int XB_ELEMS = npad(1) * KXL;
  static constexpr int DX_ELEMS = (npad(1) + 2) * KXL;
  static_assert(dma_bytes(npad(0)) <= (DY_ELEMS + DT_ELEMS) * 2, "dy staging spills into the (not yet written) dt image only");
  static_assert(dma_bytes(npad(1)) <= (XB_ELEMS + DX_ELEMS) * 2, "x_b staging spills into the (not yet written) dx image only");
  static_assert(dma_bytes(np(2)) <= DY_ELEMS * 2, "x_a fits the dy buffer");
  static constexpr int NF1 = C::NET * C::KS1, NF3 = B::KS3B, NF2T = 2 * C::NET, NF1T = C::KS2;
  static constexpr int NFR = NF1 + NF3 + NF2T + NF1T;
  static constexpr int L_W1 = 0, L_W3T = NF1, L_W2T = L_W3T + NF3, L_W1T = L_W2T + NF2T;
  static constexpr int src_frag(int fr) { return fr < NF1 ? fr : B::W3T_OFF + (fr - NF1); }
  static_assert(B::W2T_OFF == B::W3T_OFF + NF3 && B::W1T_OFF == B::W2T_OFF + NF2T, "W3T | W2T | W1T are contiguous in the blob");
  static constexpr int W_ELEMS = NFR * 512;
  static constexpr int ONES_ELEMS = 8;
  static constexpr int LDS_BYTES = (DY_ELEMS + DT_ELEMS + XB_ELEMS + DX_ELEMS + W_ELEMS + ONES_ELEMS) * 2;
  static_assert(LDS_BYTES <= 160 * 1024, "LDS budget");
};

template <typename R> struct BwP1 {
  static constexpr int N = R::NF3;
  bf16x8 w[N];
  SR_DEV void load_one(const __bf16* wl, int lane, int i) { if (i < N) w[i] = lds_chunk<__bf16>(wl, ((R::L_W3T + i) * 64 + lane) * 8); }
  SR_DEV void load(const __bf16* wl, int lane) {
#pragma unroll
    for (int i = 0; i < N; ++i) load_one(wl, lane, i);
  }
};
template <typename R> struct BwP2 {
  static constexpr int N = R::NF1 + R::NF2T + R::NF1T;
  bf16x8 w1[R::NF1], w2t[R::NF2T], w1t[R::NF1T];
  SR_DEV void load_one(const __bf16* wl, int lane, int i) {
    if (i < R::NF1) w1[i] = lds_chunk<__bf16>(wl, ((R::L_W1 + i) * 64 + lane) * 8);
    else if (i < R::NF1 + R::NF2T) w2t[i - R::NF1] = lds_chunk<__bf16>(wl, ((R::L_W2T + i - R::NF1) * 64 + lane) * 8);
    else if (i < N) w1t[i - R::NF1 - R::NF2T] = lds_chunk<__bf16>(wl, ((R::L_W1T + i - R::NF1 - R::NF2T) * 64 + lane) * 8);
  }
  SR_DEV void load(const __bf16* wl, int lane) {
#pragma unroll
    for (int i = 0; i < N; ++i) load_one(wl, lane, i);
  }
};

template <typename R, int RWO, int NPO, int HALOO, typename PF>
SR_DEV void bw_phase_dt(const __bf16* DYimg, __bf16* DT, const BwP1<R>& w, __bf16* dtsave_tile, int H, int W, int ty0, int tx0, int wave,
                        int lane, PF prefetch) {
  typedef typename R::C C;
  constexpr int NT = (NPO + 31) / 32, RWI = RWO + 2, KS = R::NF3;
  static_assert(KS == 14, "27 chunks of 8 channels + one of padding");
  const int r = lane & 31, hh = lane >> 5;
  auto do_tile = [&](int tile, auto pfon) {
    const int hp = tile * 32 + r;
    const int hpc = hp < NPO ? hp : 0;
    const int hy = hpc / RWO, hx = hpc - hy * RWO;
    const __bf16* const base = DYimg + (hy * RWI + hx) * R::KXL + hh * 8;
    const __bf16* const alt4 = hh ? DYimg + ((hy + 1) * RWI + hx) * R::KXL : base + 8 * 8;
    const __bf16* const alt13 = hh ? base : base + 2 * RWI * R::KXL + 8 * 8;
    auto frag = [&](int s) {
      const int q0 = 2 * s;
      const int off = (q0 / 9) * RWI * R::KXL + (q0 % 9) * 8;
      if (s == 4) return *reinterpret_cast<const bf16x8*>(alt4);
      if (s == 13) return *reinterpret_cast<const bf16x8*>(alt13);
      return *reinterpret_cast<const bf16x8*>(base + off);
    };
    bf16x8 f[KS];
#pragma unroll
    for (int s = 0; s < 4; ++s) f[s] = frag(s);
    f32x16 acc = zero16();
    __builtin_amdgcn_s_setprio(2);
    __builtin_amdgcn_sched_barrier(0);
#pragma unroll
    for (int s = 0; s < KS; ++s) {
      acc = mma16<__bf16>(w.w[s], f[s], acc);
      if (s + 4 < KS) f[s + 4] = frag(s + 4);
      if constexpr (decltype(pfon)::value) prefetch(2 * s, 2 * s + 2);
      __builtin_amdgcn_sched_barrier(0);
    }
    __builtin_amdgcn_s_setprio(0);
    if constexpr (decltype(pfon)::value) prefetch(2 * KS, 64);
    bf16x4 v[3];
#pragma unroll
    for (int g = 0; g < 3; ++g) v[g] = acc_group<__bf16>(acc, g);
#pragma unroll
    for (int g = 0; g < 3; ++g) *reinterpret_cast<bf16x4*>(DT + hp * R::DTL + (g < 2 ? 8 * hh + 4 * g : 16 + 4 * hh)) = v[g];
    if (dtsave_tile) {
      const int cy = hy - HALOO, cx = hx - HALOO;
      if (hp < NPO && cy >= 0 && cy < C::TH && cx >= 0 && cx < C::TW) {
        if (!(ty0 + cy < H && tx0 + cx < W)) {
#pragma unroll
          for (int g = 0; g < 3; ++g)
#pragma unroll
            for (int k = 0; k < 4; ++k) v[g][k] = (__bf16)0.f;
        }
        __bf16* o = dtsave_tile + (cy * C::TW + cx) * C::LP + hh * 4;
#pragma unroll
        for (int g = 0; g < 3; ++g) stream_store(reinterpret_cast<bf16x4*>(o + g * 8), v[g]);
      }
    }
  };
  if (wave >= NT) {
    prefetch(0, 64);
    return;
  }
  do_tile(wave, std::true_type{});
#pragma unroll 1
  for (int tile = wave + R::NW; tile < NT; tile += R::NW) do_tile(tile, std::false_type{});
}

template <typename R, int RWO, int NPO, int HALOO>
SR_DEV void bw_phase_dx(const __bf16* Ximg, const __bf16* ones, const __bf16* DT, const __bf16* DYimg, __bf16* DXimg, __bf16* dxout,
                        const BwP2<R>& w, int H, int W, int ty0, int tx0, int wave, int lane) {
  typedef typename R::C C;
  typedef __attribute__((ext_vector_type(4))) unsigned u32x4_;
  typedef __attribute__((ext_vector_type(2))) unsigned u32x2_;
  constexpr int NT = (NPO + 31) / 32, RWI = RWO + 2;
  const int r = lane & 31, hh = lane >> 5;
  const __amdgpu_buffer_rsrc_t yrs = __builtin_amdgcn_make_buffer_rsrc(dxout, 0, H * W * C::F * 2, 0x00020000);
#pragma unroll 1
  for (int tile = wave; tile < NT; tile += R::NW) {
    const int hp = tile * 32 + r;
    const int hpc = hp < NPO ? hp : 0;
    const int hy = hpc / RWO, hx = hpc - hy * RWO;
    bf16x8 xb[C::KS1], dtb[2];
    rw_x_frags<C, R::KXL>(xb, Ximg, ones, hpc, hh);
#pragma unroll
    for (int s = 0; s < 2; ++s) dtb[s] = *reinterpret_cast<const bf16x8*>(DT + hpc * R::DTL + 16 * s + 8 * hh);
    f32x16 dx = rw_resid_init<C>(DYimg + ((hy + 1) * RWI + hx + 1) * R::KXL, hh);
    auto conv1 = [&](int et) {
      f32x16 h = mma16<__bf16>(w.w1[et * C::KS1], xb[0], zero16());
      return mma16<__bf16>(w.w1[et * C::KS1 + 1], xb[1], h);
    };
    auto dhof = [&](int et) {
      f32x16 d = mma16<__bf16>(w.w2t[2 * et], dtb[0], zero16());
      return mma16<__bf16>(w.w2t[2 * et + 1], dtb[1], d);
    };
    __builtin_amdgcn_s_setprio(2);
    f32x16 h = conv1(0), dh = dhof(0);
#pragma unroll
    for (int et = 0; et < C::NET; ++et) {
      f32x16 hn = h, dhn = dh;
      if (et + 1 < C::NET) {
        hn = conv1(et + 1);
        dhn = dhof(et + 1);
      }
      bf16x8 hr[2] = {acc_to_frag_relu<__bf16, 0>(h), acc_to_frag_relu<__bf16, 1>(h)};
      bf16x8 dq[2] = {acc_to_frag<__bf16, 0>(dh), acc_to_frag<__bf16, 1>(dh)};
#pragma unroll
      for (int s = 0; s < 2; ++s) {
        const u32x4_ hq = __builtin_bit_cast(u32x4_, hr[s]);
        u32x4_ dd = __builtin_bit_cast(u32x4_, dq[s]);
#pragma unroll
        for (int j = 0; j < 4; ++j) {
          unsigned m;
          asm volatile("v_pk_min_u16 %0, %1, %2" : "=v"(m) : "v"(hq[j]), "s"(0x00010001u));
          asm volatile("v_pk_mul_lo_u16 %0, %1, %2" : "=v"(dd[j]) : "v"(dd[j]), "v"(m));
        }
        dq[s] = __builtin_bit_cast(bf16x8, dd);
      }
      asm volatile("s_nop 4" ::: "memory");
      if (2 * et < C::KS2) dx = mma16<__bf16>(w.w1t[2 * et], dq[0], dx);
      if (2 * et + 1 < C::KS2) dx = mma16<__bf16>(w.w1t[2 * et + 1], dq[1], dx);
      h = hn;
      dh = dhn;
    }
    __builtin_amdgcn_s_setprio(0);
    const int Y = ty0 - HALOO + hy, X = tx0 - HALOO + hx;
    const bool live = hp < NPO, inimg = live && Y >= 0 && Y < H && X >= 0 && X < W;
    bf16x4 v[C::FC];
#pragma unroll
    for (int g = 0; g < C::FC; ++g) {
      v[g] = acc_group<__bf16>(dx, g);
      if (!inimg) {
#pragma unroll
        for (int k = 0; k < 4; ++k) v[g][k] = (__bf16)0.f;
      }
    }
    if (DXimg) {
#pragma unroll
      for (int g = 0; g < C::FC; ++g) *reinterpret_cast<bf16x4*>(DXimg + hp * R::KXL + g * 8 + hh * 4) = v[g];
    }
    const int cy = hy - HALOO, cx = hx - HALOO;
    const bool core = inimg && cy >= 0 && cy < C::TH && cx >= 0 && cx < C::TW;
    const unsigned off = core ? (unsigned)((Y * W + X) * C::F * 2) + hh * 8 : 0xFFFFFF00u;
#pragma unroll
    for (int g = 0; g < C::FC; ++g)
      __builtin_amdgcn_raw_buffer_store_b64(__builtin_bit_cast(u32x2_, v[g]), yrs, off + g * 16, 0, 2 );
  }
}

template <int F, int E, int L>
__global__ __launch_bounds__(512) void wdsr_bwd_rs_kernel(const __bf16* __restrict__ xa, const __bf16* __restrict__ xb,
                                                          const __bf16* __restrict__ dyb, __bf16* __restrict__ dxb,
                                                          __bf16* __restrict__ dxa, const __bf16* __restrict__ wa,
                                                          const __bf16* __restrict__ wb, __bf16* __restrict__ dta,
                                                          __bf16* __restrict__ dtb, int H, int W, int tiles_x) {
  typedef BwdRsCfg<F, E, L> R;
  typedef typename R::C C;
  __shared__ __attribute__((aligned(16))) char smem_raw[R::LDS_BYTES];
  __bf16* const DY = reinterpret_cast<__bf16*>(smem_raw);
  __bf16* const DT = DY + R::DY_ELEMS;
  __bf16* const XB = DT + R::DT_ELEMS;
  __bf16* const DX = XB + R::XB_ELEMS;
  __bf16* const WL = DX + R::DX_ELEMS;
  __bf16* const ONES = WL + R::W_ELEMS;
  const int tid = threadIdx.x, lane = tid & 63;
  const int wave = __builtin_amdgcn_readfirstlane(tid >> 6);
  const int n = blockIdx.y, tile = blockIdx.x;
  const int ty0 = (tile / tiles_x) * C::TH, tx0 = (tile % tiles_x) * C::TW;
  const size_t img = (size_t)n * H * W * F;
  const size_t tile_g = (size_t)n * gridDim.x + tile;
  const char* zeros = reinterpret_cast<const char*>(g_sr_const_chunks) + 16;
  const int lq = lane / C::FC, lc = lane - lq * C::FC;
  SR_STAMP_DECL;
  SR_STAMP();

  auto stage_region = [&](__bf16* dst, const __bf16* src, int y0, int x0, int rw, int npx, int p0) {
    const int np_ = R::pieces(npx);
#pragma unroll 1
    for (int p = (wave - p0) & 7; p < np_; p += 8) {
      const int px_ = p * R::PXP + lq;
      const int py = px_ / rw, pxx = px_ - py * rw;
      const int Y = y0 + py, X = x0 + pxx;
      const char* s = zeros;
      if (px_ < npx && Y >= 0 && Y < H && X >= 0 && X < W) s = reinterpret_cast<const char*>(src + img + ((size_t)Y * W + X) * C::F + lc * 8);
      dma_piece16(s, lds_addr(dst) + p * (R::PXP * C::FC * 16));
    }
  };
  auto stage_w = [&](const __bf16* wsrc, int lo, int hi, int p0) {
#pragma unroll 1
    for (int fr = lo + ((wave - p0 - lo) & 7); fr < hi; fr += 8)
      dma_piece16(reinterpret_cast<const char*>(wsrc + (size_t)R::src_frag(fr) * 512 + lane * 8), lds_addr(WL) + fr * 1024);
  };
  constexpr int SET2_REAL = R::pieces(R::np(1)) + R::NF1 + R::NF2T + R::NF1T;
  constexpr int SET2 = (SET2_REAL + 7) / 8 * 8;
  stage_w(wb, R::L_W3T, R::L_W3T + R::NF3, 0);
  stage_region(DY, dyb, ty0 - 2, tx0 - 2, R::rw(0), R::np(0), 6);
  {
    constexpr int NPX1 = R::pieces(R::np(1));
#pragma unroll 1
    for (int p = wave; p < SET2; p += 8) {
      if (p < NPX1) {
        const int px_ = p * R::PXP + lq;
        const int py = px_ / R::rw(1), pxx = px_ - py * R::rw(1);
        const int Y = ty0 - 1 + py, X = tx0 - 1 + pxx;
        const char* sp = zeros;
        if (px_ < R::np(1) && Y >= 0 && Y < H && X >= 0 && X < W) sp = reinterpret_cast<const char*>(xb + img + ((size_t)Y * W + X) * C::F + lc * 8);
        dma_piece16(sp, lds_addr(XB) + p * (R::PXP * C::FC * 16));
      } else {
        const int k0 = p - NPX1, k = k0 < R::NF1 + R::NF2T + R::NF1T ? k0 : 0, fr = k < R::NF1 ? k : R::L_W2T + (k - R::NF1);
        dma_piece16(reinterpret_cast<const char*>(wb + (size_t)R::src_frag(fr) * 512 + lane * 8), lds_addr(WL) + fr * 1024);
      }
    }
  }
  if (tid < 8) ONES[tid] = tid == 0 ? (__bf16)1.f : (__bf16)0.f;
  for (int i = tid; i < (R::npad(1) + 2 - R::np(1)) * R::KXL / 8; i += R::NTHREADS) {
    bf16x8 z;
#pragma unroll
    for (int j = 0; j < 8; ++j) z[j] = (__bf16)0.f;
    *reinterpret_cast<bf16x8*>(DX + R::np(1) * R::KXL + i * 8) = z;
  }
  SR_STAMP();
  wait_vmcnt<SET2 / 8>();
  __syncthreads();
  SR_STAMP();

  BwP1<R> w1;
  BwP2<R> w2;
  w1.load(WL, lane);
  auto pf2 = [&](int lo, int hi) {
#pragma unroll
    for (int i = 0; i < BwP2<R>::N; ++i)
      if (i >= lo && i < hi) w2.load_one(WL, lane, i);
  };
  __bf16* const dtb_tile = dtb ? dtb + tile_g * (C::TH * C::TW) * C::LP : nullptr;
  __bf16* const dta_tile = dta ? dta + tile_g * (C::TH * C::TW) * C::LP : nullptr;
  bw_phase_dt<R, R::rw(1), R::np(1), 1>(DY, DT, w1, dtb_tile, H, W, ty0, tx0, wave, lane, [](int, int) {});
  SR_STAMP();
  wait_vmcnt<3>();
  if (!dtb_tile) wait_vmcnt<0>();
  __syncthreads();
  w2.load(WL, lane);
  __syncthreads();
  stage_w(wa, 0, R::NFR, 0);
  SR_STAMP();
  bw_phase_dx<R, R::rw(1), R::np(1), 1>(XB, ONES, DT, DY, DX, dxb + img, w2, H, W, ty0, tx0, wave, lane);
  SR_STAMP();
  static_assert((R::np(1) + 31) / 32 >= R::NW, "every wave stores at least one tile of dx_b after its weight pieces");
  wait_vmcnt<3>();
  __syncthreads();
  SR_STAMP();
  stage_region(DY, xa, ty0, tx0, R::rw(2), R::np(2), 0);
  w1.load(WL, lane);
  bw_phase_dt<R, R::rw(2), R::np(2), 0>(DX, DT, w1, dta_tile, H, W, ty0, tx0, wave, lane, pf2);
  SR_STAMP();
  static_assert((R::np(2) + 31) / 32 >= R::NW, "every wave has a tile of dt_a");
  if (dta_tile) wait_vmcnt<3>();
  else wait_vmcnt<0>();
  __syncthreads();
  SR_STAMP();
  bw_phase_dx<R, R::rw(2), R::np(2), 0>(DY, ONES, DT, DX, nullptr, dxa + img, w2, H, W, ty0, tx0, wave, lane);
  SR_STAMP();
}
```

mobilesuperresolution_amd/csrc/wdsr_fwd_rs.h:

```cpp
#pragma once
#include <type_traits>
#include "wdsr_block.h"

__device__ __attribute__((aligned(16))) const unsigned short g_sr_const_chunks[16] = {0x3F80, 0, 0, 0, 0, 0, 0, 0,
                                                                                      0,      0, 0, 0, 0, 0, 0, 0};

SR_DEV unsigned lds_addr(const void* p) {
  return (unsigned)(size_t)(__attribute__((address_space(3))) const char*)p;
}
SR_DEV void dma_piece16(const void* gsrc, unsigned lds_base) {
  unsigned keep;
  const unsigned base = __builtin_amdgcn_readfirstlane(lds_base);
  asm volatile("s_mov_b32 %0, m0\n\ts_mov_b32 m0, %2\n\ts_nop 0\n\tglobal_load_lds_dwordx4 %1, off\n\ts_mov_b32 m0, %0"
               : "=&s"(keep) : "v"(gsrc), "s"(base) : "memory");
}
SR_DEV void dma_piece4(const void* gsrc, unsigned lds_base) {
  unsigned keep;
  const unsigned base = __builtin_amdgcn_readfirstlane(lds_base);
  asm volatile("s_mov_b32 %0, m0\n\ts_mov_b32 m0, %2\n\ts_nop 0\n\tglobal_load_lds_dword %1, off\n\ts_mov_b32 m0, %0"
               : "=&s"(keep) : "v"(gsrc), "s"(base) : "memory");
}
template <int N> SR_DEV void wait_vmcnt() {
  static_assert(N >= 0 && N < 64, "vmcnt is 6 bits");
  asm volatile("s_waitcnt vmcnt(%0)" :: "n"(N) : "memory");
}
constexpr int pieces_of_wave(int lo, int hi, int w, int nw) {
  int c = 0;
  for (int p = lo; p < hi; ++p) c += (p % nw == w) ? 1 : 0;
  return c;
}

template <int F_, int E_, int L_, int NBLK_> struct RsCfg {
  typedef BlockCfg<F_, E_, L_> C;
  static constexpr int NBLK = NBLK_, NWAVES = 8, NTHREADS = 64 * NWAVES;
  static constexpr int rw(int k) { return C::TW + 2 * (NBLK - k); }
  static constexpr int rh(int k) { return C::TH + 2 * (NBLK - k); }
  static constexpr int np(int k) { return rw(k) * rh(k); }
  static constexpr int npad(int k) { return (np(k) + 31) / 32 * 32; }
  static constexpr int KXL = C::F;
  static constexpr int X0_ELEMS = npad(0) * KXL;
  static_assert(C::DENSE3, "the register-resident forward runs the 3x3 conv in its dense-K form");
  static constexpr int TD = C::TD;
  static constexpr int TT_ELEMS = npad(0) * TD;
  static constexpr int X1_ELEMS = NBLK > 1 ? npad(1) * KXL : 0;
  static constexpr int ONES_ELEMS = 8;
  static constexpr int NFR_A = C::W2_OFF + C::KS2, NFR = NFR_A + C::KS3D, W3D_SRC = BwdCfg<C>::NFRAG;
  static constexpr int W_ELEMS = NFR * 512;
  static constexpr int src_frag(int fr) { return fr < NFR_A ? fr : W3D_SRC + (fr - NFR_A); }
  static constexpr int CL_FLOATS = (C::CINIT_FWD + 63) / 64 * 64;
  static constexpr bool REUSE_W = (X0_ELEMS + TT_ELEMS + X1_ELEMS + NBLK * W_ELEMS + ONES_ELEMS) * 2 + NBLK * CL_FLOATS * 4 > 160 * 1024;
  static constexpr int W_REGIONS = REUSE_W ? 1 : NBLK;
  static constexpr int LDS_BYTES = (X0_ELEMS + TT_ELEMS + X1_ELEMS + W_REGIONS * W_ELEMS + ONES_ELEMS) * 2 + NBLK * CL_FLOATS * 4;
  static_assert(LDS_BYTES <= 160 * 1024, "LDS budget");
  static constexpr int PXP = (C::FC == 3 ? 63 : 64) / C::FC, P_X = 0, NPX = (npad(0) + PXP - 1) / PXP;
  static_assert(C::FC == 3 || C::FC == 4, "piece geometry: 3 or 4 chunks per pixel");
  static_assert(NPX * PXP * C::FC * 16 + 16 <= (X0_ELEMS + TT_ELEMS) * 2, "the last x piece may spill into the (not yet written) t image only");
  static constexpr int P_C = P_X + NPX, NPC = NBLK * (CL_FLOATS / 64);
  static constexpr int P_W = P_C + NPC, P_W1 = P_W + NFR, P_END = P_W + NBLK * NFR;
};

template <typename C> struct RwA {
  static constexpr int N = C::NET * C::KS1 + C::KS2;
  bf16x8 w1[C::NET * C::KS1], w2[C::KS2];
  SR_DEV void load_one(const __bf16* wl, int lane, int i) {
    if (i < C::NET * C::KS1) w1[i] = lds_chunk<__bf16>(wl, ((C::W1_OFF + i) * 64 + lane) * 8);
    else if (i < N) w2[i - C::NET * C::KS1] = lds_chunk<__bf16>(wl, ((C::W2_OFF + i - C::NET * C::KS1) * 64 + lane) * 8);
  }
  SR_DEV void load(const __bf16* wl, int lane) {
#pragma unroll
    for (int i = 0; i < C::NET * C::KS1; ++i) w1[i] = lds_chunk<__bf16>(wl, ((C::W1_OFF + i) * 64 + lane) * 8);
#pragma unroll
    for (int i = 0; i < C::KS2; ++i) w2[i] = lds_chunk<__bf16>(wl, ((C::W2_OFF + i) * 64 + lane) * 8);
  }
};
template <typename C> struct RwB {
  static constexpr int N = C::KS3D, OFF = C::W2_OFF + C::KS2;
  bf16x8 w3[N];
  SR_DEV void load_one(const __bf16* wl, int lane, int i) {
    if (i < N) w3[i] = lds_chunk<__bf16>(wl, ((OFF + i) * 64 + lane) * 8);
  }
  SR_DEV void load(const __bf16* wl, int lane) {
#pragma unroll
    for (int i = 0; i < N; ++i) w3[i] = lds_chunk<__bf16>(wl, ((OFF + i) * 64 + lane) * 8);
  }
};

template <typename C, int PFN = 0, typename PF>
SR_DEV f32x16 rw_t_tile(const bf16x8 (&xb)[C::KS1], const RwA<C>& w, const float* cl, int hh, PF pf) {
  typedef __attribute__((ext_vector_type(8))) short s16x8;
  f32x16 tacc = load_cinit(cl, hh);
  auto conv1_step = [&](f32x16 acc, int et, int s) { return mma16<__bf16>(w.w1[et * C::KS1 + s], xb[s], acc); };
  auto conv1_init = [&](int et) { return C::FOLD_B1 ? zero16() : load_cinit(cl + 32 + et * 32, hh); };
  auto cvt4 = [&](const f32x16& a, int base) {
    bf16x8 f;
#pragma unroll
    for (int j = 0; j < 8; j += 2) {
      __bf16 lo, hi;
      cvt_pair<__bf16>(lo, hi, a[base + j], a[base + j + 1]);
      f[j] = lo;
      f[j + 1] = hi;
    }
    return f;
  };
  auto relu8 = [&](bf16x8 f) {
    s16x8 v = __builtin_bit_cast(s16x8, f);
    const s16x8 z = {0, 0, 0, 0, 0, 0, 0, 0};
    return __builtin_bit_cast(bf16x8, __builtin_elementwise_max(v, z));
  };
  static_assert(C::KS1 == 2, "two conv1 k-steps per e-tile");
  __builtin_amdgcn_s_setprio(2);
  f32x16 h = conv1_init(0);
  h = conv1_step(h, 0, 0);
  h = conv1_step(h, 0, 1);
  bf16x8 f1prev = {};
#pragma unroll
  for (int et = 0; et < C::NET; ++et) {
    const bool more = et + 1 < C::NET;
    f32x16 hn = h;
    pf(et);
    if (more) hn = conv1_step(conv1_init(et + 1), et + 1, 0);
    bf16x8 f0 = cvt4(h, 0);
    if (more) hn = conv1_step(hn, et + 1, 1);
    f0 = relu8(f0);
    if (et > 0 && 2 * (et - 1) + 1 < C::KS2) tacc = mma16<__bf16>(w.w2[2 * et - 1], f1prev, tacc);
    bf16x8 f1 = cvt4(h, 8);
    if (2 * et < C::KS2) tacc = mma16<__bf16>(w.w2[2 * et], f0, tacc);
    f1prev = relu8(f1);
    h = hn;
#pragma unroll
    for (int k = 0; k < 4; ++k) {
      __builtin_amdgcn_sched_group_barrier(0x008, 1, 0);
      __builtin_amdgcn_sched_group_barrier(0x002, 4, 0);
      if (k < PFN) __builtin_amdgcn_sched_group_barrier(0x100, 1, 0);
    }
  }
  if (2 * (C::NET - 1) + 1 < C::KS2) tacc = mma16<__bf16>(w.w2[2 * C::NET - 1], f1prev, tacc);
  __builtin_amdgcn_s_setprio(0);
  return tacc;
}

struct RwPix {
  int hp;
  int tso;
  bool valid;
};
template <typename C, int RW, int NP, int HALO>
SR_DEV RwPix rw_pix_a(int hp, int H, int W, int ty0, int tx0) {
  RwPix p;
  p.hp = hp;
  const int hy = hp / RW, hx = hp - hy * RW;
  const int Y = ty0 - HALO + hy, X = tx0 - HALO + hx;
  p.valid = hp < NP && Y >= 0 && Y < H && X >= 0 && X < W;
  const bool core = hp < NP && hy >= HALO && hy < HALO + C::TH && hx >= HALO && hx < HALO + C::TW;
  p.tso = core ? ((hy - HALO) * C::TW + hx - HALO) * C::LP : -1;
  return p;
}
template <typename C, bool SAVE_T>
SR_DEV void rw_store_t(const f32x16& tacc, const RwPix& p, __bf16* TT, __bf16* tsave_tile, int hh) {
  bf16x4 v[C::CPT];
#pragma unroll
  for (int g = 0; g < C::CPT; ++g) {
    v[g] = acc_group<__bf16>(tacc, g);
    if (!p.valid) {
#pragma unroll
      for (int j = 0; j < 4; ++j) v[g][j] = (__bf16)0.f;
    }
  }
#pragma unroll
  for (int g = 0; g < C::CPT; ++g) {
    if (g * 8 + 8 <= C::TD) *reinterpret_cast<bf16x4*>(TT + p.hp * C::TD + g * 8 + hh * 4) = v[g];
    else if (g * 8 + 4 <= C::TD) { if (hh == 0) *reinterpret_cast<bf16x4*>(TT + p.hp * C::TD + g * 8) = v[g]; }
  }
  if constexpr (SAVE_T) {
    if (p.tso >= 0) {
#pragma unroll
      for (int g = 0; g < C::CPT; ++g) stream_store(reinterpret_cast<bf16x4*>(tsave_tile + p.tso + g * 8 + hh * 4), v[g]);
    }
  }
}

template <typename C, int KXL>
SR_DEV void rw_x_frags(bf16x8 (&xb)[C::KS1], const __bf16* Xin, const __bf16* ones, int hp, int hh) {
#pragma unroll
  for (int s = 0; s < C::KS1; ++s) {
    const int q = 2 * s + hh;
    const __bf16* src = Xin + hp * KXL + q * 8;
    if (C::FOLD_B1 && 2 * s + 1 >= C::FC) src = q < C::FC ? src : ones;
    xb[s] = *reinterpret_cast<const bf16x8*>(src);
  }
}

template <typename C, int KXL, int RW, int NP, int HALO, int NW, bool SAVE_T, typename PF, typename BS>
SR_DEV void rw_phase_a(const __bf16* Xin, const __bf16* ones, __bf16* TT, const RwA<C>& w, const float* cl, __bf16* tsave_tile,
                       int H, int W, int ty0, int tx0, int wave, int lane, PF prefetch, BS before_stores) {
  constexpr int NT = (NP + 31) / 32;
  const int r = lane & 31, hh = lane >> 5;
  if (wave >= NT) {
    prefetch(0, 64);
    before_stores();
    return;
  }
  RwPix p = rw_pix_a<C, RW, NP, HALO>(wave * 32 + r, H, W, ty0, tx0);
  bf16x8 xb[C::KS1];
  rw_x_frags<C, KXL>(xb, Xin, ones, p.hp, hh);
  SR_STAMP_AT(11);
  constexpr int PFN = 4;
  {
    const f32x16 t = rw_t_tile<C, PFN>(xb, w, cl, hh, [&](int et) { prefetch(et * PFN, et * PFN + PFN); });
    SR_STAMP_AT(12);
    const RwPix pc = p;
    if (wave + NW < NT) {
      p = rw_pix_a<C, RW, NP, HALO>((wave + NW) * 32 + r, H, W, ty0, tx0);
      rw_x_frags<C, KXL>(xb, Xin, ones, p.hp, hh);
    }
    prefetch(C::NET * PFN, 64);
    before_stores();
    rw_store_t<C, SAVE_T>(t, pc, TT, tsave_tile, hh);
    SR_STAMP_AT(13);
  }
#pragma unroll 1
  for (int tile = wave + NW; tile < NT; tile += NW) {
    const f32x16 t = rw_t_tile<C>(xb, w, cl, hh, [](int) {});
    const RwPix pc = p;
    if (tile + NW < NT) {
      p = rw_pix_a<C, RW, NP, HALO>((tile + NW) * 32 + r, H, W, ty0, tx0);
      rw_x_frags<C, KXL>(xb, Xin, ones, p.hp, hh);
    }
    rw_store_t<C, SAVE_T>(t, pc, TT, tsave_tile, hh);
  }
}

template <typename C, int RWI> struct RwBAddrD {
  static constexpr int TD = C::TD, KS = C::KS3D, KPR = C::KPR;
  static_assert(C::DENSE3, "dense-K layout");
  typedef __attribute__((address_space(3))) const volatile bf16x4* lds_chunk_p;
  lds_chunk_p b0;
  lds_chunk_p last;
  SR_DEV void init(const __bf16* TT, const __bf16* ones, int hy, int hx, int hh) {
    const __bf16* g0 = TT + (hy * RWI + hx) * TD + hh * (C::HALF * 4);
    b0 = (lds_chunk_p)(g0);
    last = (lds_chunk_p)(hh ? ones : g0 + 2 * RWI * TD + C::QONE * 8 + 4);
  }
  SR_DEV bf16x8 frag(int s) const {
    const int off = ((s / KPR) * RWI * TD + (s % KPR) * 8) / 4;
    const bf16x4 lo = b0[off];
    const bf16x4 hi = s == 2 * KPR + C::QONE ? *last : b0[off + 1];
    bf16x8 f;
    f[0] = lo[0]; f[1] = lo[1]; f[2] = lo[2]; f[3] = lo[3];
    f[4] = hi[0]; f[5] = hi[1]; f[6] = hi[2]; f[7] = hi[3];
    return f;
  }
};
template <typename C> SR_DEV f32x16 rw_resid_init(const __bf16* xrow, int hh) {
  f32x16 acc;
#pragma unroll
  for (int g = 0; g < 4; ++g) {
    if (g < C::FC) {
      const bf16x4 v = *reinterpret_cast<const bf16x4*>(xrow + g * 8 + hh * 4);
#pragma unroll
      for (int k = 0; k < 4; ++k) acc[4 * g + k] = (float)v[k];
    } else {
#pragma unroll
      for (int k = 0; k < 4; ++k) acc[4 * g + k] = 0.f;
    }
  }
  return acc;
}

struct RwPixB {
  int hy, hx;
  int xno;
  unsigned go;
};
template <typename C, int KXL, int RWO, int NPO, int HALOO>
SR_DEV RwPixB rw_pix_b(int tile, int r, int H, int W, int ty0, int tx0) {
  RwPixB p;
  const int hp = tile * 32 + r;
  const int hpc = hp < NPO ? hp : 0;
  p.hy = hpc / RWO;
  p.hx = hpc - p.hy * RWO;
  p.xno = hp * KXL;
  const int Y = ty0 - HALOO + p.hy, X = tx0 - HALOO + p.hx;
  const bool st = hp < NPO && p.hy >= HALOO && p.hy < HALOO + C::TH && p.hx >= HALOO && p.hx < HALOO + C::TW && Y < H && X < W;
  p.go = st ? (unsigned)((Y * W + X) * C::F * 2) : 0xFFFFFF00u;
  return p;
}
template <typename C>
SR_DEV void rw_store_y(const f32x16& oacc, const RwPixB& p, __bf16* Xnext, __amdgpu_buffer_rsrc_t yrs, bool to_global, int hh) {
  typedef __attribute__((ext_vector_type(2))) unsigned u32x2_;
  bf16x4 v[C::FC];
#pragma unroll
  for (int g = 0; g < C::FC; ++g) v[g] = acc_group<__bf16>(oacc, g);
  if (Xnext) {
#pragma unroll
    for (int g = 0; g < C::FC; ++g) *reinterpret_cast<bf16x4*>(Xnext + p.xno + g * 8 + hh * 4) = v[g];
  }
  if (to_global) {
    const unsigned off = p.go + hh * 8;
#pragma unroll
    for (int g = 0; g < C::FC; ++g) {
      __builtin_amdgcn_raw_buffer_store_b64(__builtin_bit_cast(u32x2_, v[g]), yrs, off + g * 16, 0, 2 );
    }
  }
}

template <typename C, typename A, int AHEAD, int LAG, typename MID, typename PF>
SR_DEV f32x16 rw_b_chain(const A& a, const RwB<C>& w, f32x16 acc, MID mid, PF pf) {
  constexpr int KS = C::KS3D;
  bf16x8 f[KS];
#pragma unroll
  for (int s = 0; s < AHEAD; ++s) f[s] = a.frag(s);
  __builtin_amdgcn_s_setprio(2);
  __builtin_amdgcn_sched_barrier(0);
#pragma unroll
  for (int s = 0; s < KS; ++s) {
    acc = mma16<__bf16>(w.w3[s], f[s], acc);
    if (s + AHEAD < KS) f[s + AHEAD] = a.frag(s + AHEAD);
    pf(s);
    __builtin_amdgcn_sched_barrier(0);
    if (s == LAG) {
      mid();
      __builtin_amdgcn_sched_barrier(0);
    }
  }
  __builtin_amdgcn_s_setprio(0);
  return acc;
}

template <typename C, int KXL, int RWO, int NPO, int HALOO, int NW, typename PF>
SR_DEV void rw_phase_b(const __bf16* TT, const __bf16* Xin, const __bf16* ones, __bf16* Xnext, __bf16* yout, const RwB<C>& w, int H,
                       int W, int ty0, int tx0, int wave, int lane, PF prefetch) {
  constexpr int NT = (NPO + 31) / 32, RWI = RWO + 2, AHEAD = 4, LAG = 4;
  typedef RwBAddrD<C, RWI> A;
  const int r = lane & 31, hh = lane >> 5;
  if (wave >= NT) {
    prefetch(0, 64);
    return;
  }
  SR_STAMP_AT(6);
  const bool to_global = yout != nullptr;
  const __amdgpu_buffer_rsrc_t yrs = __builtin_amdgcn_make_buffer_rsrc(yout, 0, to_global ? H * W * C::F * 2 : 0, 0x00020000);
  RwPixB p = rw_pix_b<C, KXL, RWO, NPO, HALOO>(wave, r, H, W, ty0, tx0);
  A a;
  a.init(TT, ones, p.hy, p.hx, hh);
  SR_STAMP_AT(7);
  f32x16 acc = rw_b_chain<C, A, AHEAD, LAG>(a, w, rw_resid_init<C>(Xin + ((p.hy + 1) * RWI + p.hx + 1) * KXL, hh), [] {},
                                            [&](int s) { prefetch(2 * s, 2 * s + 2); });
  prefetch(2 * C::KS3D, 128);
  SR_STAMP_AT(8);
#pragma unroll 1
  for (int tile = wave + NW; tile < NT; tile += NW) {
    const RwPixB pp = p;
    const f32x16 pacc = acc;
    p = rw_pix_b<C, KXL, RWO, NPO, HALOO>(tile, r, H, W, ty0, tx0);
    a.init(TT, ones, p.hy, p.hx, hh);
    acc = rw_b_chain<C, A, AHEAD, LAG>(a, w, rw_resid_init<C>(Xin + ((p.hy + 1) * RWI + p.hx + 1) * KXL, hh),
                                       [&] { rw_store_y<C>(pacc, pp, Xnext, yrs, to_global, hh); }, [](int) {});
  }
  SR_STAMP_AT(9);
  rw_store_y<C>(acc, p, Xnext, yrs, to_global, hh);
  SR_STAMP_AT(10);
}

template <int F, int E, int L, int NBLK, bool SAVE_T>
__global__ __launch_bounds__(512) void wdsr_fwd_rs_kernel(const __bf16* __restrict__ x, __bf16* __restrict__ ya,
                                                          __bf16* __restrict__ yb, const __bf16* __restrict__ wa,
                                                          const __bf16* __restrict__ wb, const float* __restrict__ cia,
                                                          const float* __restrict__ cib, __bf16* __restrict__ tsa,
                                                          __bf16* __restrict__ tsb, int H, int W, int tiles_x) {
  typedef BlockCfg<F, E, L> C;
  typedef RsCfg<F, E, L, NBLK> R;
  constexpr int NTHREADS = R::NTHREADS, NW = R::NWAVES;
  __shared__ __attribute__((aligned(16))) char smem_raw[R::LDS_BYTES];
  __bf16* const X0 = reinterpret_cast<__bf16*>(smem_raw);
  __bf16* const TT = X0 + R::X0_ELEMS;
  __bf16* const X1 = TT + R::TT_ELEMS;
  __bf16* const WL = X1 + R::X1_ELEMS;
  __bf16* const ONES = WL + NBLK * R::W_ELEMS;
  float* const CL = reinterpret_cast<float*>(ONES + R::ONES_ELEMS);
  constexpr int KXL = R::KXL;
  const int tid = threadIdx.x, lane = tid & 63;
  const int wave = __builtin_amdgcn_readfirstlane(tid >> 6);
  const int n = blockIdx.y, tile = blockIdx.x;
  const int ty0 = (tile / tiles_x) * C::TH, tx0 = (tile % tiles_x) * C::TW;
  const size_t img = (size_t)n * H * W * F;
  const size_t tile_g = (size_t)n * gridDim.x + tile;
  SR_STAMP_DECL;
  SR_STAMP();

  auto stage_pieces = [&](int lo, int hi) {
    const char* zeros = reinterpret_cast<const char*>(g_sr_const_chunks) + 16;
    const int y0 = ty0 - NBLK, x0 = tx0 - NBLK;
    const int lq = lane / C::FC, lc = lane - lq * C::FC;
#pragma unroll 1
    for (int p = lo + ((wave - lo) & (NW - 1)); p < hi; p += NW) {
      if (p < R::P_C) {
        const int px_ = p * R::PXP + lq;
        const int py = px_ / R::rw(0), pxx = px_ - py * R::rw(0);
        const int Y = y0 + py, X = x0 + pxx;
        const char* src = zeros;
        if (px_ < R::np(0) && Y >= 0 && Y < H && X >= 0 && X < W)
          src = reinterpret_cast<const char*>(x + img + ((size_t)Y * W + X) * C::F + lc * 8);
        dma_piece16(src, lds_addr(X0) + p * (R::PXP * C::FC * 16));
      } else if (p < R::P_W) {
        const int k = p - R::P_C, blk = k / (R::CL_FLOATS / 64), i = (k % (R::CL_FLOATS / 64)) * 64 + lane;
        const float* tab = (NBLK > 1 && blk == 1) ? cib : cia;
        const char* src = i < C::CINIT_FWD ? reinterpret_cast<const char*>(tab + i) : zeros + (lane & 3) * 4;
        dma_piece4(src, lds_addr(CL) + k * 256);
      } else {
        const int fr = p - R::P_W;
        const __bf16* wsrc = (NBLK > 1 && fr >= R::NFR) ? wb + (size_t)R::src_frag(fr - R::NFR) * 512 : wa + (size_t)R::src_frag(fr) * 512;
        dma_piece16(reinterpret_cast<const char*>(wsrc + lane * 8), lds_addr(WL) + fr * 1024);
      }
    }
  };
  static_assert((NW & (NW - 1)) == 0, "power-of-two wave count");
  stage_pieces(0, R::P_W1);
  if (tid < 8) ONES[tid] = tid == 0 ? (__bf16)1.f : (__bf16)0.f;
  SR_STAMP();
  wait_vmcnt<0>();
  __syncthreads();
  SR_STAMP();
  if constexpr (NBLK > 1) stage_pieces(R::P_W1, R::P_END);

  __bf16* const tsa_tile = SAVE_T ? tsa + tile_g * (C::TH * C::TW) * C::LP : nullptr;
  __bf16* const tsb_tile = (SAVE_T && NBLK > 1) ? tsb + tile_g * (C::TH * C::TW) * C::LP : nullptr;
  RwA<C> rwa;
  RwB<C> rwb;
  rwa.load(WL, lane);
  auto pf_a = [&](const __bf16* wl, int lo, int hi) {
#pragma unroll
    for (int i = 0; i < RwA<C>::N; ++i)
      if (i >= lo && i < hi) rwa.load_one(wl, lane, i);
  };
  auto pf_b = [&](const __bf16* wl, int lo, int hi) {
#pragma unroll
    for (int i = 0; i < RwB<C>::N; ++i)
      if (i >= lo && i < hi) rwb.load_one(wl, lane, i);
  };
  rw_phase_a<C, KXL, R::rw(0), R::np(0), NBLK, NW, SAVE_T>(X0, ONES, TT, rwa, CL, tsa_tile, H, W, ty0, tx0, wave, lane,
                                                             [&](int lo, int hi) { pf_b(WL, lo, hi); }, [] { wait_vmcnt<0>(); });
  SR_STAMP();
  __syncthreads();
  SR_STAMP();
  if constexpr (NBLK == 1) {
    rw_phase_b<C, KXL, C::TW, C::TH * C::TW, 0, NW>(TT, X0, ONES, nullptr, yb + img, rwb, H, W, ty0, tx0, wave, lane, [](int, int) {});
  } else {
    rw_phase_b<C, KXL, R::rw(1), R::np(1), NBLK - 1, NW>(TT, X0, ONES, X1, ya ? ya + img : nullptr, rwb, H, W, ty0, tx0, wave, lane,
                                                         [&](int lo, int hi) { pf_a(WL + R::W_ELEMS, lo, hi); });
    SR_STAMP();
    __syncthreads();
    SR_STAMP();
    rw_phase_a<C, KXL, R::rw(1), R::np(1), NBLK - 1, NW, SAVE_T>(X1, ONES, TT, rwa, CL + R::CL_FLOATS, tsb_tile, H, W, ty0, tx0, wave,
                                                                 lane, [&](int lo, int hi) { pf_b(WL + R::W_ELEMS, lo, hi); }, [] {});
    SR_STAMP();
    __syncthreads();
    SR_STAMP();
    rw_phase_b<C, KXL, C::TW, C::TH * C::TW, 0, NW>(TT, X1, ONES, nullptr, yb + img, rwb, H, W, ty0, tx0, wave, lane, [](int, int) {});
  }
  SR_STAMP();
}

template <typename C>
SR_DEV f32x16 rw_t_tile_lds(const bf16x8 (&xb)[C::KS1], const __bf16* wl, int lane, const float* cl, int hh) {
  typedef __attribute__((ext_vector_type(8))) short s16x8;
  static_assert(C::KS1 == 2, "two conv1 k-steps per e-tile");
  RwA<C> w;
  constexpr int W2 = C::NET * C::KS1;
  auto need = [&](int et) {
    if (et < 0) { w.load_one(wl, lane, 0); w.load_one(wl, lane, 1); return; }
    if (et + 1 < C::NET) { w.load_one(wl, lane, 2 * (et + 1)); w.load_one(wl, lane, 2 * (et + 1) + 1); }
    if (et > 0 && 2 * et - 1 < C::KS2) w.load_one(wl, lane, W2 + 2 * et - 1);
    if (2 * et < C::KS2) w.load_one(wl, lane, W2 + 2 * et);
  };
  f32x16 tacc = load_cinit(cl, hh);
  auto cvt4 = [&](const f32x16& a, int base) {
    bf16x8 f;
#pragma unroll
    for (int j = 0; j < 8; j += 2) {
      __bf16 lo, hi;
      cvt_pair<__bf16>(lo, hi, a[base + j], a[base + j + 1]);
      f[j] = lo;
      f[j + 1] = hi;
    }
    return f;
  };
  auto relu8 = [&](bf16x8 f) {
    s16x8 v = __builtin_bit_cast(s16x8, f);
    const s16x8 z = {0, 0, 0, 0, 0, 0, 0, 0};
    return __builtin_bit_cast(bf16x8, __builtin_elementwise_max(v, z));
  };
  need(-1);
  need(0);
  auto conv1_init = [&](int et) { return C::FOLD_B1 ? zero16() : load_cinit(cl + 32 + et * 32, hh); };
  f32x16 h = conv1_init(0);
  h = mma16<__bf16>(w.w1[0], xb[0], h);
  h = mma16<__bf16>(w.w1[1], xb[1], h);
  bf16x8 f1prev = {};
#pragma unroll
  for (int et = 0; et < C::NET; ++et) {
    const bool more = et + 1 < C::NET;
    f32x16 hn = h;
    if (more) need(et + 1);
    else if (2 * C::NET - 1 < C::KS2) w.load_one(wl, lane, W2 + 2 * C::NET - 1);
    if (more) hn = mma16<__bf16>(w.w1[2 * (et + 1)], xb[0], conv1_init(et + 1));
    bf16x8 f0 = cvt4(h, 0);
    if (more) hn = mma16<__bf16>(w.w1[2 * (et + 1) + 1], xb[1], hn);
    f0 = relu8(f0);
    if (et > 0 && 2 * (et - 1) + 1 < C::KS2) tacc = mma16<__bf16>(w.w2[2 * et - 1], f1prev, tacc);
    bf16x8 f1 = cvt4(h, 8);
    if (2 * et < C::KS2) tacc = mma16<__bf16>(w.w2[2 * et], f0, tacc);
    f1prev = relu8(f1);
    h = hn;
#pragma unroll
    for (int k = 0; k < 4; ++k) {
      __builtin_amdgcn_sched_group_barrier(0x008, 1, 0);
      __builtin_amdgcn_sched_group_barrier(0x002, 4, 0);
      __builtin_amdgcn_sched_group_barrier(0x100, 1, 0);
    }
  }
  if (2 * (C::NET - 1) + 1 < C::KS2) tacc = mma16<__bf16>(w.w2[2 * C::NET - 1], f1prev, tacc);
  return tacc;
}

template <typename C, typename A, int AHEAD>
SR_DEV f32x16 rw_b_chain_lds(const A& a, const __bf16* wl, int lane, f32x16 acc) {
  constexpr int KS = C::KS3D;
  RwB<C> w;
  bf16x8 f[KS];
#pragma unroll
  for (int s = 0; s < AHEAD; ++s) {
    w.load_one(wl, lane, s);
    f[s] = a.frag(s);
  }
  __builtin_amdgcn_sched_barrier(0);
#pragma unroll
  for (int s = 0; s < KS; ++s) {
    acc = mma16<__bf16>(w.w3[s], f[s], acc);
    if (s + AHEAD < KS) {
      w.load_one(wl, lane, s + AHEAD);
      f[s + AHEAD] = a.frag(s + AHEAD);
    }
    __builtin_amdgcn_sched_barrier(0);
  }
  return acc;
}

template <int F, int E, int L, int NBLK, bool SAVE_T>
__global__ __launch_bounds__(1024) void wdsr_fwd_rs16_kernel(const __bf16* __restrict__ x, __bf16* __restrict__ ya,
                                                             __bf16* __restrict__ yb, const __bf16* __restrict__ wa,
                                                             const __bf16* __restrict__ wb, const float* __restrict__ cia,
                                                             const float* __restrict__ cib, __bf16* __restrict__ tsa,
                                                             __bf16* __restrict__ tsb, int H, int W, int tiles_x) {
  typedef BlockCfg<F, E, L> C;
  typedef RsCfg<F, E, L, NBLK> R;
  constexpr int NW = 16;
  __shared__ __attribute__((aligned(16))) char smem_raw[R::LDS_BYTES];
  __bf16* const X0 = reinterpret_cast<__bf16*>(smem_raw);
  __bf16* const TT = X0 + R::X0_ELEMS;
  __bf16* const X1 = TT + R::TT_ELEMS;
  __bf16* const WL = X1 + R::X1_ELEMS;
  __bf16* const ONES = WL + R::W_REGIONS * R::W_ELEMS;
  __bf16* const WL1 = R::REUSE_W ? WL : WL + R::W_ELEMS;
  float* const CL = reinterpret_cast<float*>(ONES + R::ONES_ELEMS);
  constexpr int KXL = R::KXL;
  const int tid = threadIdx.x, lane = tid & 63, r = lane & 31, hh = lane >> 5;
  const int wave = __builtin_amdgcn_readfirstlane(tid >> 6);
  const int n = blockIdx.y, tile = blockIdx.x;
  const int ty0 = (tile / tiles_x) * C::TH, tx0 = (tile % tiles_x) * C::TW;
  const size_t img = (size_t)n * H * W * F;
  const size_t tile_g = (size_t)n * gridDim.x + tile;

  auto stage_pieces = [&](int lo, int hi) {
    const char* zeros = reinterpret_cast<const char*>(g_sr_const_chunks) + 16;
    const int y0 = ty0 - NBLK, x0 = tx0 - NBLK;
    const int lq = lane / C::FC, lc = lane - lq * C::FC;
#pragma unroll 1
    for (int p = lo + ((wave - lo) & (NW - 1)); p < hi; p += NW) {
      if (p < R::P_C) {
        const int px_ = p * R::PXP + lq;
        const int py = px_ / R::rw(0), pxx = px_ - py * R::rw(0);
        const int Y = y0 + py, X = x0 + pxx;
        const char* src = zeros;
        if (px_ < R::np(0) && Y >= 0 && Y < H && X >= 0 && X < W)
          src = reinterpret_cast<const char*>(x + img + ((size_t)Y * W + X) * C::F + lc * 8);
        dma_piece16(src, lds_addr(X0) + p * (R::PXP * C::FC * 16));
      } else if (p < R::P_W) {
        const int k = p - R::P_C, blk = k / (R::CL_FLOATS / 64), i = (k % (R::CL_FLOATS / 64)) * 64 + lane;
        const float* tab = (NBLK > 1 && blk == 1) ? cib : cia;
        const char* src = i < C::CINIT_FWD ? reinterpret_cast<const char*>(tab + i) : zeros + (lane & 3) * 4;
        dma_piece4(src, lds_addr(CL) + k * 256);
      } else {
        const int fr = p - R::P_W;
        const __bf16* wsrc = (NBLK > 1 && fr >= R::NFR) ? wb + (size_t)R::src_frag(fr - R::NFR) * 512 : wa + (size_t)R::src_frag(fr) * 512;
        dma_piece16(reinterpret_cast<const char*>(wsrc + lane * 8), lds_addr(WL) + ((R::REUSE_W && fr >= R::NFR) ? fr - R::NFR : fr) * 1024);
      }
    }
  };
  stage_pieces(0, R::P_W1);
  if (tid < 8) ONES[tid] = tid == 0 ? (__bf16)1.f : (__bf16)0.f;
  wait_vmcnt<0>();
  __syncthreads();
  if constexpr (NBLK > 1 && !R::REUSE_W) stage_pieces(R::P_W1, R::P_END);

  __bf16* const tsa_tile = SAVE_T ? tsa + tile_g * (C::TH * C::TW) * C::LP : nullptr;
  __bf16* const tsb_tile = (SAVE_T && NBLK > 1) ? tsb + tile_g * (C::TH * C::TW) * C::LP : nullptr;

  auto phase_a = [&](auto rw_c, auto np_c, auto halo_c, const __bf16* Xin, const __bf16* wl, const float* cl, __bf16* ts_tile, bool join_dma) {
    constexpr int RW = decltype(rw_c)::value, NP = decltype(np_c)::value, HALO = decltype(halo_c)::value, NT = (NP + 31) / 32;
    bool waited = false;
#pragma unroll 1
    for (int t_ = wave; t_ < NT; t_ += NW) {
      const RwPix p = rw_pix_a<C, RW, NP, HALO>(t_ * 32 + r, H, W, ty0, tx0);
// ... 285 lines not shown
```

mobilesuperresolution_amd/models/basic_wdsr_b.py:

```python
from __future__ import annotations

import ctypes
import math
import os
from collections import OrderedDict

import numpy as np
import torch
import torch.nn as nn

from .. import _lib as L
from ..layout import get_layout

__all__ = ["BASIC_MODEL"]


class _DeviceState:

    def __init__(self, model: "BASIC_MODEL", device: torch.device):
        lay = model.layout
        t = lambda a: torch.from_numpy(np.ascontiguousarray(a)).to(device)
        f32 = lambda n: torch.empty(n, dtype=torch.float32, device=device)
        self.chan_tab, self.bias_tab = t(lay.chan_tab), t(lay.bias_tab)
        bc = lay.bias_const.copy()
        bc[np.isnan(bc)] = model.image_mean
        self.bias_const = t(bc)
        self.idx = {k: t(getattr(lay, "idx_" + k)) for k in ("head", "body", "cinit", "tail")}
        self.g = {k: (t(getattr(lay, k)[0]), t(getattr(lay, k)[1])) for k in ("ga", "gb", "gt", "gh")}
        self.src = torch.zeros(lay.src_total, dtype=torch.float32, device=device)
        self.src[torch.from_numpy(lay.src_ones).to(device)] = 1.0
        self.dsrc = torch.zeros(lay.src_total, dtype=torch.float32, device=device)
        dt = model.hot_dtype
        self.blob_head = torch.empty(lay.idx_head.size, dtype=dt, device=device)
        self.blob_body = torch.empty((lay.NB, lay.idx_body.size), dtype=dt, device=device)
        self.cinit_body = torch.empty((lay.NB, lay.idx_cinit.size), dtype=torch.float32, device=device)
        self.blob_tail = torch.empty(lay.idx_tail.size, dtype=dt, device=device)
        self.packed_key = None
        self.wgs_body = model.wgs_body
        self.wgs_tail = int(os.environ.get("SR_WGS_TAIL", 256))
        self.wgs_head = int(os.environ.get("SR_WGS_HEAD", 256))
        self.part_a = f32(lay.NB * self.wgs_body * lay.slab_a)
        self.part_b = f32(lay.NB * self.wgs_body * lay.slab_b)
        self.part_tail = f32(self.wgs_tail * lay.slab_tail)
        self.part_head = f32(self.wgs_head * lay.slab_head)
        self.loss_part = torch.zeros(self.wgs_tail, dtype=torch.float32, device=device)
        n = L.WdsrNet()
        n.F, n.NB, n.R, n.dtype, n.mean = lay.F, lay.NB, lay.R, L.DTYPE_CODE[dt], model.image_mean
        n.chan_tab, n.n_chan = self.chan_tab.data_ptr(), lay.chan_tab.shape[0]
        n.bias_tab, n.bias_const, n.n_bias = self.bias_tab.data_ptr(), self.bias_const.data_ptr(), lay.bias_tab.shape[0]
        n.src, n.dsrc = self.src.data_ptr(), self.dsrc.data_ptr()
        n.src_head_off, n.src_body_off = lay.src_head_off, lay.src_body_off
        n.src_body_stride, n.src_tail_off = lay.src_body_stride, lay.src_tail_off
        for k in ("head", "body", "cinit", "tail"):
            setattr(n, "idx_" + k, self.idx[k].data_ptr())
            setattr(n, "n_idx_" + k, self.idx[k].numel())
        n.blob_head, n.blob_body = self.blob_head.data_ptr(), self.blob_body.data_ptr()
        n.cinit_body, n.blob_tail = self.cinit_body.data_ptr(), self.blob_tail.data_ptr()
        n.part_a, n.part_b = self.part_a.data_ptr(), self.part_b.data_ptr()
        n.part_tail, n.part_head = self.part_tail.data_ptr(), self.part_head.data_ptr()
        n.wgs_body, n.wgs_tail, n.wgs_head = self.wgs_body, self.wgs_tail, self.wgs_head
        n.slab_a, n.slab_b, n.slab_tail, n.slab_head = lay.slab_a, lay.slab_b, lay.slab_tail, lay.slab_head
        for k in ("ga", "gb", "gt", "gh"):
            setattr(n, k + "_sidx", self.g[k][0].data_ptr())
            setattr(n, k + "_dst", self.g[k][1].data_ptr())
            setattr(n, "n_" + k, self.g[k][0].numel())
        n.loss_part = self.loss_part.data_ptr()
        ct, bt = lay.chan_tab, lay.bias_tab
        cover = np.zeros(int(model.flat.numel()), dtype=np.int32)
        for v_off, g_off, K, _dst in ct:
            cover[v_off:v_off + K] += 1
            cover[g_off] += 1
        for a_, b_, _d in bt:
            cover[a_] += 1
            if b_ >= 0:
                cover[b_] += 1
        n.adam_in_wn_bwd = int(bool((cover == 1).all()))
        n.one_block32 = int(model.one_block32)
        if model.nb_split:
            _, n.chan_split, n.bias_split = lay.split_at(model.nb_split)
            n.nb_split = model.nb_split
        self.net = n

    def call_struct(self) -> "L.WdsrNet":
        return L.WdsrNet.from_buffer_copy(self.net)

    def call_net(self, x, flat, acts, out=None, dout=None, grads=None, gflat=None, side=None, dtsave=None, hr=None,
                 kind=0, gscale=0.0) -> "L.WdsrNet":
        net = self.call_struct()
        net.N, net.H, net.W = x.shape[0], x.shape[2], x.shape[3]
        net.flat, net.x, net.acts = flat.data_ptr(), x.data_ptr(), acts.data_ptr()
        if out is not None:
            net.out = out.data_ptr()
        if dout is not None:
            net.dout = dout.data_ptr()
        if grads is not None:
            net.grads, net.gflat = grads.data_ptr(), gflat.data_ptr()
        if side is not None:
            net.tsave = side.data_ptr()
        if dtsave is not None:
            net.dtsave = dtsave.data_ptr()
        if hr is not None:
            net.hr, net.loss_kind, net.loss_gscale = hr.data_ptr(), kind, gscale
        return net

    def ensure_packed(self, net, key, sp):
        if self.packed_key != key:
            _launch_net("sr_wdsr_net_forward", net, 4, sp)
            self.packed_key = key


def _launch_net(name, net, *args):
    L.launch(name, getattr(L.lib(), name), ctypes.byref(net), *args)


def _backward_buffers(acts, flat, side):
    return torch.empty_like(acts), torch.empty_like(flat), torch.empty_like(side) if side is not None else None


class BASIC_MODEL(nn.Module):

    def __init__(self, params):
        super().__init__()
        self.image_mean = float(params.image_mean)
        self.scale = int(params.scale)
        self.remain_blocks = params.num_blocks
        nin = int(params.num_channels)
        f = int(params.num_residual_units)
        nb = int(params.num_blocks)
        self.num_residual_units, self.num_blocks = f, nb
        if nin != 3 or f not in (24, 32) or self.scale not in (2, 3, 4) or nb < 1:
            raise NotImplementedError(
                "MI355X hot path supports num_channels=3, num_residual_units in {24,32}, scale in {2,3,4} "
                f"(got {nin}, {f}, {self.scale}); there is no generic fallback")
        self.hot_dtype = L.hot_dtype(getattr(params, "hot_dtype", None))
        self.wgs_body = int(getattr(params, "hot_wgs_body", os.environ.get("SR_WGS_BODY", 16)))
        self.layout = get_layout(f, nb, self.scale)
        self.grad_segments = int(getattr(params, "hot_grad_segments", None) or os.environ.get("SR_GRAD_SEGMENTS", 1))
        if self.grad_segments not in (1, 2):
            raise NotImplementedError("hot_grad_segments must be 1 or 2")
        init = self._reference_init()
        self.nb_split = nb - 2 * ((nb // 2 + 1) // 2) if nb >= 2 else 0
        if self.grad_segments == 2 and nb >= 2:
            k = self.layout.split_at(self.nb_split)[0]
            self.flat_lo = nn.Parameter(init[:k])
            self.flat_hi = nn.Parameter(init[k:])
            self._flat_master = init
        else:
            self.grad_segments = 1
            self.flat = nn.Parameter(init)
        self._dev = {}
        self._one_block32 = False

    @property
    def one_block32(self) -> bool:
        return self._one_block32

    @one_block32.setter
    def one_block32(self, value: bool):
        self._one_block32 = bool(value)
        for st in self._dev.values():
            st.net.one_block32 = int(self._one_block32)

    def __getattr__(self, name):
        if name == "flat" and "_flat_master" in self.__dict__:
            return self.__dict__["_flat_master"]
        return super().__getattr__(name)

    def _apply(self, fn, recurse=True):
        if self.grad_segments == 2:
            with torch.no_grad():
                master = fn(self._flat_master)
            k = self.flat_lo.numel()
            self.flat_lo.data, self.flat_hi.data = master[:k], master[k:]
            for p in (self.flat_lo, self.flat_hi):
                if p.grad is not None:
                    p.grad.data = fn(p.grad.data)
            self._flat_master = master
            return self
        return super()._apply(fn, recurse)

    def __getstate__(self):
        d = self.__dict__.copy()
        d["_dev"] = {}
        return d

    def __deepcopy__(self, memo):
        import copy
        cls = self.__class__
        new = cls.__new__(cls)
        memo[id(self)] = new
        for k, v in self.__dict__.items():
            new.__dict__[k] = {} if k == "_dev" else copy.deepcopy(v, memo)
        if new.grad_segments == 2:
            k = new.flat_lo.numel()
            new.flat_lo.data, new.flat_hi.data = new._flat_master[:k], new._flat_master[k:]
        return new

    def __setstate__(self, d):
        self.__dict__.update(d)
        if self.grad_segments == 2:
            k = self.flat_lo.numel()
            self._flat_master = torch.cat([self.flat_lo.detach(), self.flat_hi.detach()])
            self.flat_lo.data, self.flat_hi.data = self._flat_master[:k], self._flat_master[k:]

    def _reference_init(self) -> torch.Tensor:
        lay = self.layout
        flat = torch.zeros(lay.total)
        gains = {"head": 1.0, "tail": 1.0, "skip.0": 1.0}
        for i in range(lay.NB):
            gains[f"body.{i}.body.0"] = 2.0
            gains[f"body.{i}.body.2"] = 2.0
            gains[f"body.{i}.body.3"] = 1 / math.sqrt(lay.NB)
        for c in lay.convs:
            conv = nn.Conv2d(c.cin, c.cout, c.k)
            off, shape = lay.entries[c.name + ".weight_v"]
            flat[off:off + conv.weight.numel()] = conv.weight.detach().reshape(-1)
            off, _ = lay.entries[c.name + ".weight_g"]
            flat[off:off + c.cout] = gains[c.name]
        return flat

    def named_tensors(self):
        for name, (off, shape) in self.layout.entries.items():
            yield name, self.flat.detach()[off:off + int(np.prod(shape))].view(shape)

    def state_dict(self, *args, destination=None, prefix="", keep_vars=False):
        if destination is None:
            destination = OrderedDict()
        for name, view in self.named_tensors():
            destination[prefix + name] = view
        return destination

    def _load_from_state_dict(self, state_dict, prefix, local_metadata, strict, missing_keys, unexpected_keys,
                              error_msgs):
        with torch.no_grad():
            for name, view in self.named_tensors():
                key = prefix + name
                if key not in state_dict:
                    missing_keys.append(key)
                    continue
                src = state_dict[key]
                if tuple(src.shape) != tuple(view.shape):
                    error_msgs.append(f"size mismatch for {key}: checkpoint {tuple(src.shape)} vs model {tuple(view.shape)}")
                    continue
                view.copy_(src)
        known = {prefix + n for n in self.layout.entries}
        for key in state_dict:
            if key.startswith(prefix) and key not in known and key not in (prefix + "flat", prefix + "flat_lo", prefix + "flat_hi"):
                unexpected_keys.append(key)

    def _state(self, device: torch.device) -> _DeviceState:
        key = (device.type, device.index)
        st = self._dev.get(key)
        if st is None or st.blob_head.dtype != self.hot_dtype:
            st = self._dev[key] = _DeviceState(self, device)
        return st

    def _check_input(self, x, *others):
        if not x.is_cuda or not self.flat.is_cuda:
            raise L.HotpathError("BASIC_MODEL (MI355X hot path) needs CUDA/HIP tensors; there is no CPU fallback")
        for t in (self.flat,) + others:
            if t.device != x.device:
                raise L.HotpathError(f"tensors on different devices ({x.device} vs {t.device}): the kernels take raw pointers "
                                     "and would dereference another GPU's memory")
        if x.dim() != 4 or x.shape[1] != 3:
            raise ValueError(f"expected N x 3 x H x W input, got {tuple(x.shape)}")
        if x.requires_grad:
            raise NotImplementedError("gradient w.r.t. the input image is not on the hot path "
                                      "(the reference trainers never request it)")

    def _forward_buffers(self, x, save_acts: bool):
        lay = self.layout
        n, _, h, w = x.shape
        slots = lay.NB + 1 if save_acts else 2
        acts = torch.empty((slots, n, h, w, lay.F), dtype=self.hot_dtype, device=x.device)
        out = torch.empty((n, 3, self.scale * h, self.scale * w), dtype=torch.float32, device=x.device)
        side = None
        if save_acts and self._saves_side_images():
            side = torch.empty(self._side_shape(n, h, w), dtype=self.hot_dtype, device=x.device)
        return out, acts, side

    def _forward_impl(self, x, flat, save_acts: bool):
        st = self._state(x.device)
        out, acts, side = self._forward_buffers(x, save_acts)
        net = st.call_net(x, flat, acts, out=out, side=side)
        if self.grad_segments == 2:
            key = (flat.data_ptr(), self.flat_lo._version, self.flat_hi._version)
        else:
            key = (flat.data_ptr(), flat._version)
        static = getattr(self, "assume_static_weights", False) and not save_acts and st.packed_key == key
        flags = (1 if save_acts else 0) | (2 if static else 0)
        with L.device_guard(x.device):
            _launch_net("sr_wdsr_net_forward", net, flags, L.stream_ptr(x.device))
        st.packed_key = key
        return out, acts, side

    def _saves_side_images(self) -> bool:
        lay = self.layout
        return (self.hot_dtype == torch.bfloat16 and lay.NB > 0 and os.environ.get("SR_RECOMPUTE_WGRAD", "0") != "1")

    def _side_shape(self, n, h, w):
        tiles = ((h + 11) // 12) * ((w + 23) // 24)
        return (self.layout.NB, n, tiles, 288, 24 if self.layout.F == 24 else 32)

    def forward(self, x: torch.Tensor) -> torch.Tensor:
        self._check_input(x)
        if x.dtype != torch.float32 or not x.is_contiguous():
            x = x.contiguous().float()
        if self.grad_segments == 2:
            if torch.is_grad_enabled() and (self.flat_lo.requires_grad or self.flat_hi.requires_grad):
                shared = _Shared()
                token = _NetLoFunction.apply(x, self.flat_lo, self, shared)
                return _NetHiFunction.apply(token, self.flat_hi, self, shared)
            return self._forward_impl(x, self.flat.detach(), False)[0]
        if torch.is_grad_enabled() and self.flat.requires_grad:
            return _NetFunction.apply(x, self.flat, self)
        return self._forward_impl(x, self.flat.detach(), False)[0]

    _LOSS_KINDS = {"l1": 1, "charbonnier": 2}

    @staticmethod
    def _gscale(weight: float, numel: int) -> float:
        return float(np.float32(weight) / np.float32(numel))

    def _loss_backward_impl(self, x, hr, flat, kind: str, weight: float, net_out=None):
        st = self._state(x.device)
        out, acts, side = self._forward_impl(x, flat, True)
        grads, gflat, dtsave = _backward_buffers(acts, flat, side)
        net = st.call_net(x, flat, acts, out=out, grads=grads, gflat=gflat, side=side, dtsave=dtsave, hr=hr,
                          kind=self._LOSS_KINDS[kind], gscale=self._gscale(weight, out.numel()))
        with L.device_guard(x.device):
            _launch_net("sr_wdsr_net_backward", net, L.stream_ptr(x.device))
        return net, out, gflat, (acts, grads, side, dtsave)

    def _can_fold(self, node, sr, hr) -> bool:
        return (self.grad_segments == 1 and sr.is_cuda and hr.is_cuda and hr.device == sr.device and sr.shape == hr.shape
                and sr.dtype == torch.float32 and sr.is_contiguous() and not hr.requires_grad and sr.data_ptr() == node.out_ptr)

    def _backward_folded(self, node, sr, hr, kind: str):
        x, acts, side = node.x, node.acts, node.tsave
        (flat,) = node.saved_tensors
        st = self._state(x.device)
        grads, gflat, dtsave = _backward_buffers(acts, flat, side)
        net = st.call_net(x, flat, acts, out=sr, grads=grads, gflat=gflat, side=side, dtsave=dtsave, hr=hr,
                          kind=self._LOSS_KINDS[kind], gscale=self._gscale(1.0, sr.numel()))
        with L.device_guard(x.device):
            sp = L.stream_ptr(x.device)
            st.ensure_packed(net, node.packed_key, sp)
            _launch_net("sr_wdsr_net_backward", net, sp)
        return gflat, (grads, dtsave, hr)

    def _check_target(self, x, hr):
        self._check_input(x, hr)
        want = (x.shape[0], 3, self.scale * x.shape[2], self.scale * x.shape[3])
        if tuple(hr.shape) != want:
            raise ValueError(f"target shape {tuple(hr.shape)} != network output shape {want}")
        return x.contiguous().float(), hr.contiguous().float()

    def loss(self, x: torch.Tensor, hr: torch.Tensor, kind: str = "l1", weight: float = 1.0) -> torch.Tensor:
        x, hr = self._check_target(x, hr)
        if self.grad_segments == 2:
            raise NotImplementedError("model.loss() is the one-parameter route; with hot_grad_segments = 2 use forward() + a torch "
                                      "loss (DistributedDataParallel hooks need the two gradient nodes)")
        return _NetLossFunction.apply(x, hr, self.flat, self, kind, float(weight))

    DP_OVERLAP_MIN_PARAMS = 4 * 1024 * 1024

    def receptive_halo(self) -> int:
        return self.num_blocks + 2

    def ddp_bucket_cap_mb(self) -> float:
        if self.grad_segments != 2:
            return 25.0
        return 0.5 * min(self.flat_lo.numel(), self.flat_hi.numel()) * 4 / (1 << 20)

    def make_train_state(self, lr: float = 1e-3, betas=(0.9, 0.999), eps: float = 1e-8):
        return AdamState(self.flat, lr, betas, eps)

    def train_step(self, x: torch.Tensor, hr: torch.Tensor, state: "AdamState", kind: str = "l1", weight: float = 1.0,
                   process_group=None, overlap=None):
        x, hr = self._check_target(x, hr)
        if state.exp_avg.device != x.device:
            raise L.HotpathError("optimizer state and input on different devices")
        st = self._state(x.device)
        flat = self.flat.detach()
        if self.grad_segments == 2:
            raise NotImplementedError("train_step is the single-GPU fused step; with hot_grad_segments = 2 train through "
                                      "DistributedDataParallel (forward / loss / backward / optimizer)")
        out, acts, side = self._forward_buffers(x, True)
        grads, gflat, dtsave = _backward_buffers(acts, flat, side)
        net = st.call_net(x, flat, acts, out=out, grads=grads, gflat=gflat, side=side, dtsave=dtsave, hr=hr,
                          kind=self._LOSS_KINDS[kind], gscale=self._gscale(weight, out.numel()))
        loss = torch.empty((), dtype=torch.float32, device=x.device)
        scal = state.next_scalars()
        import torch.distributed as dist
        pg = process_group
        if pg is None and dist.is_available() and dist.is_initialized() and dist.get_world_size() > 1:
            pg = dist.group.WORLD
        with L.device_guard(x.device):
            sp = L.stream_ptr(x.device)
            if pg is None:
                _launch_net("sr_wdsr_net_train_step", net, state.exp_avg.data_ptr(), state.exp_avg_sq.data_ptr(), flat.numel(),
                            ctypes.byref(scal), float(weight) / out.numel(), loss.data_ptr(), sp)
            else:
                if overlap is None:
                    overlap = flat.numel() >= self.DP_OVERLAP_MIN_PARAMS
                halves = bool(overlap and self.nb_split)
                _launch_net("sr_wdsr_net_forward", net, 1, sp)
                _launch_net("sr_wdsr_net_backward_part", net, 1 if halves else 0, sp)
                avg = dist.get_backend(pg) == "nccl"
                op = dist.ReduceOp.AVG if avg else dist.ReduceOp.SUM
                if not halves:
                    dist.all_reduce(gflat, op=op, group=pg)
                else:
                    k = self.layout.split_at(self.nb_split)[0]
                    h_hi = dist.all_reduce(gflat[k:], op=op, group=pg, async_op=True)
                    _launch_net("sr_wdsr_net_backward_part", net, 2, sp)
                    if os.environ.get("SR_DP_LAST_ASYNC") == "1":
                        h_lo = dist.all_reduce(gflat[:k], op=op, group=pg, async_op=True)
                        h_hi.wait()
                        h_lo.wait()
                    else:
                        h_hi.wait()
                        dist.all_reduce(gflat[:k], op=op, group=pg)
                if not avg:
                    gflat.div_(dist.get_world_size(pg))
                L.launch("sr_adam_step", L.lib().sr_adam_step, flat.data_ptr(), gflat.data_ptr(), state.exp_avg.data_ptr(),
                         state.exp_avg_sq.data_ptr(), flat.numel(), ctypes.byref(scal), st.loss_part.data_ptr(), st.wgs_tail,
                         float(weight) / out.numel(), loss.data_ptr(), sp)
        _bump_version(self.flat)
        st.packed_key = None
        return loss


def _bump_version(t: torch.Tensor):
    try:
        torch.autograd.graph.increment_version(t)
    except AttributeError:
        t.data.add_(0)


class AdamState:

    def __init__(self, flat: torch.Tensor, lr: float, betas, eps: float):
        self.lr, self.beta1, self.beta2, self.eps = float(lr), float(betas[0]), float(betas[1]), float(eps)
        self.step = 0
        self.exp_avg = torch.zeros_like(flat, memory_format=torch.preserve_format).detach()
        self.exp_avg_sq = torch.zeros_like(self.exp_avg)

    def next_scalars(self) -> "L.AdamScalars":
        self.step += 1
        bc1 = 1.0 - self.beta1 ** self.step
        bc2 = 1.0 - self.beta2 ** self.step
        return L.AdamScalars(1.0 - self.beta1, self.beta2, 1.0 - self.beta2, math.sqrt(bc2), self.eps, -(self.lr / bc1))

    def state_dict(self):
        return {"step": self.step, "exp_avg": self.exp_avg, "exp_avg_sq": self.exp_avg_sq, "lr": self.lr,
                "betas": (self.beta1, self.beta2), "eps": self.eps}

    def load_state_dict(self, d):
        self.step, self.lr, self.eps = int(d["step"]), float(d["lr"]), float(d["eps"])
        self.beta1, self.beta2 = (float(b) for b in d["betas"])
        self.exp_avg.copy_(d["exp_avg"])
        self.exp_avg_sq.copy_(d["exp_avg_sq"])


class _NetFunction(torch.autograd.Function):

    @staticmethod
    def forward(ctx, x, flat, model):
        out, acts, tsave = model._forward_impl(x, flat, True)
        ctx.model, ctx.x, ctx.acts, ctx.tsave = model, x, acts, tsave
        ctx.save_for_backward(flat)
        ctx.packed_key = model._state(x.device).packed_key
        ctx.out_ptr, ctx.folded = out.data_ptr(), None
        return out

    @staticmethod
    def backward(ctx, dout):
        model, x, acts = ctx.model, ctx.x, ctx.acts
        (flat,) = ctx.saved_tensors
        folded = None
        if ctx.folded is not None:
            g0, gloss, token_ptr = ctx.folded
            folded = g0 * gloss
            if dout.data_ptr() == token_ptr and all(st_ == 0 for st_ in dout.stride()):
                return None, folded, None
        st = model._state(x.device)
        dout = dout.contiguous().float()
        grads, gflat, dtsave = _backward_buffers(acts, flat, ctx.tsave)
        net = st.call_net(x, flat, acts, dout=dout, grads=grads, gflat=gflat, side=ctx.tsave, dtsave=dtsave)
        with L.device_guard(x.device):
            sp = L.stream_ptr(x.device)
            st.ensure_packed(net, ctx.packed_key, sp)
            _launch_net("sr_wdsr_net_backward", net, sp)
        return None, (gflat if folded is None else gflat + folded), None


class _Shared:
    __slots__ = ("out", "acts", "tsave", "dtsave", "grads", "gflat", "x", "packed_key", "net")


class _NetLoFunction(torch.autograd.Function):

    @staticmethod
    def forward(ctx, x, flat_lo, model, shared):
        flat = model.flat.detach()
        shared.out, shared.acts, shared.tsave = model._forward_impl(x, flat, True)
        shared.x, shared.packed_key = x, model._state(x.device).packed_key
        ctx.model, ctx.shared = model, shared
        ctx.save_for_backward(flat_lo)
        return x.new_zeros(1)

    @staticmethod
    def backward(ctx, gtoken):
        model, sh = ctx.model, ctx.shared
        (flat_lo,) = ctx.saved_tensors
        x = sh.x
        with L.device_guard(x.device):
            _launch_net("sr_wdsr_net_backward_part", sh.net, 2, L.stream_ptr(x.device))
        k = flat_lo.numel()
        return None, sh.gflat[:k], None, None


class _NetHiFunction(torch.autograd.Function):

    @staticmethod
    def forward(ctx, token, flat_hi, model, shared):
        ctx.model, ctx.shared = model, shared
        ctx.save_for_backward(flat_hi)
        return shared.out

    @staticmethod
    def backward(ctx, dout):
        model, sh = ctx.model, ctx.shared
        (flat_hi,) = ctx.saved_tensors
        x, acts = sh.x, sh.acts
        st = model._state(x.device)
        flat = model.flat.detach()
        dout = dout.contiguous().float()
        sh.grads, sh.gflat, sh.dtsave = _backward_buffers(acts, flat, sh.tsave)
        sh.net = net = st.call_net(x, flat, acts, dout=dout, grads=sh.grads, gflat=sh.gflat, side=sh.tsave, dtsave=sh.dtsave)
        ctx.dout = dout
        with L.device_guard(x.device):
            sp = L.stream_ptr(x.device)
# ... 24 lines not shown
```

Measured before the change: 3687 HR-Mpix/s.

## Save ReLU bitmasks in forward to skip conv1 recompute in paired backward

The forward pair kernel gains a masked variant that writes a packed ReLU sign bitmask for each block alongside the saved side images. The paired backward-data kernel then reads these bits to gate the gradient instead of reloading the input activations and recomputing the first expansion convolution. This removes the conv1 MMAs and the x-fragment loads and weight staging from backward, at the cost of extra mask writes and reads plus a per-step mask buffer allocation. It applies only to F=24 bf16 paired blocks in the train_step path.

After: 3704 HR-Mpix/s, median of 2. About the same (+0.4%).

```diff
diff --git a/include/sr_hotpath.h b/include/sr_hotpath.h
--- a/include/sr_hotpath.h
+++ b/include/sr_hotpath.h
@@ -28,6 +28,12 @@
                               const void* wblob, const float* cinit, float* partial_a, float* partial_b, int layers,
                               int wgs, int N, int H, int W, int F, int dtype, long x_ls, long dy_ls, long side_ls,
                               long w_ls, long c_ls, sr_stream_t stream);
+int sr_wdsr_relu_mask_words(int H, int W);
+int sr_wdsr_block2_fwd_mask(const void* x, void* ya, void* yb, const void* wa, const void* wb, const float* cia, const float* cib,
+                            void* tsa, void* tsb, void* mask_a, void* mask_b, int N, int H, int W, int F, int dtype,
+                            sr_stream_t stream);
+int sr_wdsr_block2_bwd_data_mask(const void* mask_a, const void* mask_b, const void* dyb, void* dxb, void* dxa, const void* wa,
+                                 const void* wb, void* dta, void* dtb, int N, int H, int W, int F, int dtype, sr_stream_t stream);
 
 int sr_wdsr_fwd_rs(const void* x, void* ya, void* yb, const void* wblob_a, const void* wblob_b, const float* cinit_a,
                    const float* cinit_b, void* tsave_a, void* tsave_b, int nblk, int N, int H, int W, int F, int dtype,
@@ -235,6 +241,7 @@
   int nb_split, chan_split, bias_split;
   int adam_in_wn_bwd;
   int one_block32;
+  void* hmask;
 } sr_wdsr_net_t;
 
 #define SR_NET_SAVE_ACTS 1
diff --git a/mobilesuperresolution_amd/_lib.py b/mobilesuperresolution_amd/_lib.py
--- a/mobilesuperresolution_amd/_lib.py
+++ b/mobilesuperresolution_amd/_lib.py
@@ -9,7 +9,7 @@
 _HERE = os.path.dirname(os.path.abspath(__file__))
 LIB_PATH = os.environ.get("SR_HOTPATH_LIB_PATH") or os.path.join(
     _HERE, "libsr_hotpath_dbg.so" if os.environ.get("SR_HOTPATH_DEBUG_LIB") == "1" else "libsr_hotpath.so")
-ABI_VERSION = 23
+ABI_VERSION = 24
 DTYPE_CODE = {torch.float32: 0, torch.bfloat16: 1}
 _HOT_DTYPES = {"fp32": torch.float32, "float32": torch.float32, "bf16": torch.bfloat16, "bfloat16": torch.bfloat16}
 
@@ -29,6 +29,9 @@
     "sr_wdsr_fwd_rs_repeat": ([_P] * 9 + [_I] * 7 + [_P], _I),
     "sr_wdsr_block_wgrad_saved": ([_P] * 8 + [_I] * 7 + [_L] * 5 + [_P], _I),
     "sr_wdsr_block2_bwd_data": ([_P] * 11 + [_I] * 5 + [_P], _I),
+    "sr_wdsr_relu_mask_words": ([_I, _I], _I),
+    "sr_wdsr_block2_fwd_mask": ([_P] * 11 + [_I] * 5 + [_P], _I),
+    "sr_wdsr_block2_bwd_data_mask": ([_P] * 9 + [_I] * 5 + [_P], _I),
     "sr_wdsr_block2_fwd_repeat": ([_P] * 7 + [_I] * 6 + [_P], _I),
     "sr_probe_launch_floor": ([_P, _I, _I, _I, _I, _I, _P], _I),
     "sr_probe_launch_floor_graph": ([_P, _I, _I, _I, _I, _I, _I, _P, _P], _I),
@@ -114,7 +117,7 @@
          ("x", _P), ("acts", _P), ("grads", _P), ("out", _P), ("dout", _P), ("tsave", _P), ("dtsave", _P),
          ("hr", _P), ("loss_kind", _I), ("loss_gscale", _F), ("loss_part", _P),
          ("nb_split", _I), ("chan_split", _I), ("bias_split", _I), ("adam_in_wn_bwd", _I),
-         ("one_block32", _I)])
+         ("one_block32", _I), ("hmask", _P)])
 
 
 class C3Warp(ctypes.Structure):
diff --git a/mobilesuperresolution_amd/csrc/sr_abi.hip b/mobilesuperresolution_amd/csrc/sr_abi.hip
--- a/mobilesuperresolution_amd/csrc/sr_abi.hip
+++ b/mobilesuperresolution_amd/csrc/sr_abi.hip
@@ -29,7 +29,7 @@
 #include "result_block.h"
 #include "frame_net.h"
 
-extern "C" int sr_abi_version(void) { return 23; }
+extern "C" int sr_abi_version(void) { return 24; }
 
 namespace {
 
@@ -131,11 +131,20 @@
 
 template <int F, int NBLK>
 static int launch_fwd_rs(const void* x, void* ya, void* yb, const void* wa, const void* wb, const float* cia, const float* cib,
-                         void* tsa, void* tsb, int N, int H, int W, hipStream_t st) {
+                         void* tsa, void* tsb, int N, int H, int W, hipStream_t st, void* ma = nullptr, void* mb = nullptr) {
   typedef typename WdsrDims<F>::Cfg C;
   typedef __bf16 T;
   constexpr int E = C::E, L = C::L;
   const auto [tiles_x, tiles_y] = block_tiles<C>(H, W);
+  if constexpr (NBLK == 2) {
+    if (ma || mb) {
+      if (!ma || !mb || !tsa || !tsb) return -2;
+      hipLaunchKernelGGL((wdsr_fwd_rs_mask_kernel<F, E, L>), dim3(tiles_x * tiles_y, N), dim3(512), 0, st, (const T*)x, (T*)ya, (T*)yb,
+                         (const T*)wa, (const T*)wb, cia, cib, (T*)tsa, (T*)tsb, H, W, tiles_x, (unsigned*)ma, (unsigned*)mb);
+      SR_HIP_CHECK_LAUNCH();
+      return 0;
+    }
+  }
   constexpr int persist_from = 768;
   const long total = (long)N * tiles_x * tiles_y;
   if constexpr (NBLK == 2) {
@@ -200,6 +209,34 @@
     return -1;
   });
 }
+extern "C" int sr_wdsr_relu_mask_words(int H, int W) {
+  if (H <= 0 || W <= 0) return -2;
+  const auto [tiles_x, tiles_y] = block_tiles(H, W);
+  const long words = (long)tiles_x * tiles_y * FwdMaskCfg<WdsrDims<24>::Cfg>::TILE_WORDS;
+  return words < (1L << 31) ? (int)words : -1;
+}
+extern "C" int sr_wdsr_block2_fwd_mask(const void* x, void* ya, void* yb, const void* wa, const void* wb, const float* cia,
+                                       const float* cib, void* tsa, void* tsb, void* mask_a, void* mask_b, int N, int H, int W,
+                                       int F, int dtype, sr_stream_t stream) {
+  if (!x || !yb || !wa || !wb || !cia || !cib || !tsa || !tsb || !mask_a || !mask_b || N <= 0 || H <= 0 || W <= 0 || N > 65535)
+    return -2;
+  if (F != 24 || dtype != SR_DTYPE_BF16) return -1;
+  return launch_fwd_rs<24, 2>(x, ya, yb, wa, wb, cia, cib, tsa, tsb, N, H, W, (hipStream_t)stream, mask_a, mask_b);
+}
+extern "C" int sr_wdsr_block2_bwd_data_mask(const void* mask_a, const void* mask_b, const void* dyb, void* dxb, void* dxa,
+                                            const void* wa, const void* wb, void* dta, void* dtb, int N, int H, int W, int F,
+                                            int dtype, sr_stream_t stream) {
+  if (!mask_a || !mask_b || !dyb || !dxb || !dxa || !wa || !wb || N <= 0 || H <= 0 || W <= 0 || N > 65535) return -2;
+  if (F != 24 || dtype != SR_DTYPE_BF16) return -1;
+  typedef WdsrDims<24> D;
+  const auto [tiles_x, tiles_y] = block_tiles(H, W);
+  hipLaunchKernelGGL((wdsr_bwd_rs_mask_kernel<24, D::E, D::L>), dim3(tiles_x * tiles_y, N), dim3(512), 0, (hipStream_t)stream,
+                     (const unsigned*)mask_a, (const unsigned*)mask_b, (const __bf16*)dyb, (__bf16*)dxb, (__bf16*)dxa, (const __bf16*)wa,
+                     (const __bf16*)wb, (__bf16*)dta, (__bf16*)dtb, H, W, tiles_x);
+  SR_HIP_CHECK_LAUNCH();
+  return 0;
+}
+
 extern "C" int sr_wdsr_block2_fwd(const void* x, void* ya, void* yb, const void* wa, const void* wb, const float* cia,
                                   const float* cib, void* tsa, void* tsb, int N, int H, int W, int F, int dtype,
                                   sr_stream_t stream) {
@@ -1062,6 +1099,9 @@
 static bool net_step_fuses_tail(const sr_wdsr_net_t* n) {
   return n->dtype == SR_DTYPE_BF16 && n->R == 4 && (n->F == 24 || n->F == 32) && n->hr && n->N <= 65535;
 }
+static bool net_keeps_mask(const sr_wdsr_net_t* n) {
+  return n->hmask && n->tsave && n->F == 24 && n->dtype == SR_DTYPE_BF16 && net_uses_pairs(n);
+}
 static size_t side_image_bytes(const sr_wdsr_net_t* n) {
   typedef WdsrDims<24>::Cfg C;
   const Tiles t = block_tiles<C>(n->H, n->W);
@@ -1080,6 +1120,8 @@
   const float* cinit(int i) const { return n->cinit_body + (size_t)i * n->n_idx_cinit; }
   char* tsave(int i) const { return keeps_side ? (char*)n->tsave + (size_t)i * side_bytes : nullptr; }
   char* dtsave(int i) const { return keeps_side ? (char*)n->dtsave + (size_t)i * side_bytes : nullptr; }
+  size_t mask_bytes = (size_t)n->N * (size_t)sr_wdsr_relu_mask_words(n->H, n->W) * 4;
+  char* hmask(int i) const { return (char*)n->hmask + (size_t)i * mask_bytes; }
 };
 
 extern "C" int sr_wdsr_net_forward(const sr_wdsr_net_t* n, int flags, sr_stream_t stream) {
@@ -1096,10 +1138,14 @@
   char* cur = acts;
   const bool pairs = net_uses_pairs(n) || (n->F == 24 && n->dtype == SR_DTYPE_BF16 &&
                                            ((!save_acts && net_tiles(n) >= 768) || fwd_stream_applies(n->N, n->H, n->W)));
+  const bool keeps_mask = v.keeps_side && net_keeps_mask(n);
   for (int i = 0, nb; i < n->NB; i += nb) {
     nb = pairs && i + 1 < n->NB ? 2 : 1;
     char* nxt = save_acts ? v.act(i + nb) : (cur == acts ? v.act(1) : acts);
-    if (nb == 2)
+    if (nb == 2 && keeps_mask)
+      rc = sr_wdsr_block2_fwd_mask(cur, v.act(i + 1), nxt, v.blob(i), v.blob(i + 1), v.cinit(i), v.cinit(i + 1), v.tsave(i),
+                                   v.tsave(i + 1), v.hmask(i), v.hmask(i + 1), n->N, n->H, n->W, n->F, n->dtype, stream);
+    else if (nb == 2)
       rc = sr_wdsr_block2_fwd(cur, save_acts ? v.act(i + 1) : nullptr, nxt, v.blob(i), v.blob(i + 1), v.cinit(i), v.cinit(i + 1),
                               v.tsave(i), v.tsave(i + 1), n->N, n->H, n->W, n->F, n->dtype, stream);
     else if (pairs)
@@ -1151,7 +1197,10 @@
   }
   for (int i = b1 - 1, nb; i >= b0; i -= nb) {
     nb = pairs && i >= b0 + 1 ? 2 : 1;
-    if (nb == 2)
+    if (nb == 2 && saved && net_keeps_mask(n) && !((i - 1) & 1))
+      rc = sr_wdsr_block2_bwd_data_mask(v.hmask(i - 1), v.hmask(i), v.grad(i + 1), v.grad(i), v.grad(i - 1), v.blob(i - 1), v.blob(i),
+                                        v.dtsave(i - 1), v.dtsave(i), n->N, n->H, n->W, n->F, n->dtype, stream);
+    else if (nb == 2)
       rc = sr_wdsr_block2_bwd_data(v.act(i - 1), v.act(i), v.grad(i + 1), v.grad(i), v.grad(i - 1), v.blob(i - 1), v.blob(i),
                                    v.cinit(i - 1), v.cinit(i), v.dtsave(i - 1), v.dtsave(i), n->N, n->H, n->W, n->F, n->dtype, stream);
     else if (saved)
diff --git a/mobilesuperresolution_amd/csrc/wdsr_bwd_rs.h b/mobilesuperresolution_amd/csrc/wdsr_bwd_rs.h
--- a/mobilesuperresolution_amd/csrc/wdsr_bwd_rs.h
+++ b/mobilesuperresolution_amd/csrc/wdsr_bwd_rs.h
@@ -43,13 +43,14 @@
     for (int i = 0; i < N; ++i) load_one(wl, lane, i);
   }
 };
-template <typename R> struct BwP2 {
-  static constexpr int N = R::NF1 + R::NF2T + R::NF1T;
-  bf16x8 w1[R::NF1], w2t[R::NF2T], w1t[R::NF1T];
+template <typename R, bool MASKED = false> struct BwP2 {
+  static constexpr int N1 = MASKED ? 0 : R::NF1;
+  static constexpr int N = N1 + R::NF2T + R::NF1T;
+  bf16x8 w1[MASKED ? 1 : R::NF1], w2t[R::NF2T], w1t[R::NF1T];
   SR_DEV void load_one(const __bf16* wl, int lane, int i) {
-    if (i < R::NF1) w1[i] = lds_chunk<__bf16>(wl, ((R::L_W1 + i) * 64 + lane) * 8);
-    else if (i < R::NF1 + R::NF2T) w2t[i - R::NF1] = lds_chunk<__bf16>(wl, ((R::L_W2T + i - R::NF1) * 64 + lane) * 8);
-    else if (i < N) w1t[i - R::NF1 - R::NF2T] = lds_chunk<__bf16>(wl, ((R::L_W1T + i - R::NF1 - R::NF2T) * 64 + lane) * 8);
+    if (i < N1) w1[i] = lds_chunk<__bf16>(wl, ((R::L_W1 + i) * 64 + lane) * 8);
+    else if (i < N1 + R::NF2T) w2t[i - N1] = lds_chunk<__bf16>(wl, ((R::L_W2T + i - N1) * 64 + lane) * 8);
+    else if (i < N) w1t[i - N1 - R::NF2T] = lds_chunk<__bf16>(wl, ((R::L_W1T + i - N1 - R::NF2T) * 64 + lane) * 8);
   }
   SR_DEV void load(const __bf16* wl, int lane) {
 #pragma unroll
@@ -122,9 +123,19 @@
   for (int tile = wave + R::NW; tile < NT; tile += R::NW) do_tile(tile, std::false_type{});
 }
 
-template <typename R, int RWO, int NPO, int HALOO>
+template <typename R> struct BwMask {
+  static constexpr int NMW = (R::C::NET + 1) / 2;
+  unsigned w[NMW];
+  template <int NPADM> SR_DEV void load(const unsigned* mtile, int tile, int lane) {
+    const int row = tile * 32 + (lane & 31), hh = lane >> 5;
+#pragma unroll
+    for (int q = 0; q < NMW; ++q) w[q] = mtile[q * (NPADM * 2) + row * 2 + hh];
+  }
+};
+template <typename R, int RWO, int NPO, int HALOO, bool MASKED = false>
 SR_DEV void bw_phase_dx(const __bf16* Ximg, const __bf16* ones, const __bf16* DT, const __bf16* DYimg, __bf16* DXimg, __bf16* dxout,
-                        const BwP2<R>& w, int H, int W, int ty0, int tx0, int wave, int lane) {
+                        const BwP2<R, MASKED>& w, int H, int W, int ty0, int tx0, int wave, int lane,
+                        const unsigned* mtile = nullptr, BwMask<R>* mk = nullptr) {
   typedef typename R::C C;
   typedef __attribute__((ext_vector_type(4))) unsigned u32x4_;
   typedef __attribute__((ext_vector_type(2))) unsigned u32x2_;
@@ -137,7 +148,13 @@
     const int hpc = hp < NPO ? hp : 0;
     const int hy = hpc / RWO, hx = hpc - hy * RWO;
     bf16x8 xb[C::KS1], dtb[2];
-    rw_x_frags<C, R::KXL>(xb, Ximg, ones, hpc, hh);
+    BwMask<R> mcur;
+    if constexpr (MASKED) {
+      mcur = *mk;
+      if (tile + R::NW < NT) mk->template load<NT * 32>(mtile, tile + R::NW, lane);
+    } else {
+      rw_x_frags<C, R::KXL>(xb, Ximg, ones, hpc, hh);
+    }
 #pragma unroll
     for (int s = 0; s < 2; ++s) dtb[s] = *reinterpret_cast<const bf16x8*>(DT + hpc * R::DTL + 16 * s + 8 * hh);
     f32x16 dx = rw_resid_init<C>(DYimg + ((hy + 1) * RWI + hx + 1) * R::KXL, hh);
@@ -150,27 +167,43 @@
       return mma16<__bf16>(w.w2t[2 * et + 1], dtb[1], d);
     };
     __builtin_amdgcn_s_setprio(2);
-    f32x16 h = conv1(0), dh = dhof(0);
+    f32x16 h = zero16(), dh = dhof(0);
+    if constexpr (!MASKED) h = conv1(0);
 #pragma unroll
     for (int et = 0; et < C::NET; ++et) {
       f32x16 hn = h, dhn = dh;
       if (et + 1 < C::NET) {
-        hn = conv1(et + 1);
+        if constexpr (!MASKED) hn = conv1(et + 1);
         dhn = dhof(et + 1);
       }
-      bf16x8 hr[2] = {acc_to_frag_relu<__bf16, 0>(h), acc_to_frag_relu<__bf16, 1>(h)};
       bf16x8 dq[2] = {acc_to_frag<__bf16, 0>(dh), acc_to_frag<__bf16, 1>(dh)};
-#pragma unroll
-      for (int s = 0; s < 2; ++s) {
-        const u32x4_ hq = __builtin_bit_cast(u32x4_, hr[s]);
-        u32x4_ dd = __builtin_bit_cast(u32x4_, dq[s]);
-#pragma unroll
-        for (int j = 0; j < 4; ++j) {
-          unsigned m;
-          asm volatile("v_pk_min_u16 %0, %1, %2" : "=v"(m) : "v"(hq[j]), "s"(0x00010001u));
-          asm volatile("v_pk_mul_lo_u16 %0, %1, %2" : "=v"(dd[j]) : "v"(dd[j]), "v"(m));
+      if constexpr (MASKED) {
+#pragma unroll
+        for (int s = 0; s < 2; ++s) {
+          u32x4_ dd = __builtin_bit_cast(u32x4_, dq[s]);
+#pragma unroll
+          for (int j = 0; j < 4; ++j) {
+            const int p = 8 * (et & 1) + 4 * s + j;
+            unsigned m = mcur.w[et / 2] & (0x00010001u << p);
+            if (p != 0) asm volatile("v_pk_min_u16 %0, %1, %2" : "=v"(m) : "v"(m), "s"(0x00010001u));
+            asm volatile("v_pk_mul_lo_u16 %0, %1, %2" : "=v"(dd[j]) : "v"(dd[j]), "v"(m));
+          }
+          dq[s] = __builtin_bit_cast(bf16x8, dd);
         }
-        dq[s] = __builtin_bit_cast(bf16x8, dd);
+      } else {
+        bf16x8 hr[2] = {acc_to_frag_relu<__bf16, 0>(h), acc_to_frag_relu<__bf16, 1>(h)};
+#pragma unroll
+        for (int s = 0; s < 2; ++s) {
+          const u32x4_ hq = __builtin_bit_cast(u32x4_, hr[s]);
+          u32x4_ dd = __builtin_bit_cast(u32x4_, dq[s]);
+#pragma unroll
+          for (int j = 0; j < 4; ++j) {
+            unsigned m;
+            asm volatile("v_pk_min_u16 %0, %1, %2" : "=v"(m) : "v"(hq[j]), "s"(0x00010001u));
+            asm volatile("v_pk_mul_lo_u16 %0, %1, %2" : "=v"(dd[j]) : "v"(dd[j]), "v"(m));
+          }
+          dq[s] = __builtin_bit_cast(bf16x8, dd);
+        }
       }
       asm volatile("s_nop 4" ::: "memory");
       if (2 * et < C::KS2) dx = mma16<__bf16>(w.w1t[2 * et], dq[0], dx);
@@ -203,12 +236,11 @@
   }
 }
 
-template <int F, int E, int L>
-__global__ __launch_bounds__(512) void wdsr_bwd_rs_kernel(const __bf16* __restrict__ xa, const __bf16* __restrict__ xb,
-                                                          const __bf16* __restrict__ dyb, __bf16* __restrict__ dxb,
-                                                          __bf16* __restrict__ dxa, const __bf16* __restrict__ wa,
-                                                          const __bf16* __restrict__ wb, __bf16* __restrict__ dta,
-                                                          __bf16* __restrict__ dtb, int H, int W, int tiles_x) {
+template <int F, int E, int L, bool MASKED>
+SR_DEV void wdsr_bwd_rs_body(const __bf16* __restrict__ xa, const __bf16* __restrict__ xb, const __bf16* __restrict__ dyb,
+                             __bf16* __restrict__ dxb, __bf16* __restrict__ dxa, const __bf16* __restrict__ wa,
+                             const __bf16* __restrict__ wb, __bf16* __restrict__ dta, __bf16* __restrict__ dtb, int H, int W,
+                             int tiles_x, const unsigned* __restrict__ ma, const unsigned* __restrict__ mb) {
   typedef BwdRsCfg<F, E, L> R;
   typedef typename R::C C;
   __shared__ __attribute__((aligned(16))) char smem_raw[R::LDS_BYTES];
@@ -246,12 +278,12 @@
     for (int fr = lo + ((wave - p0 - lo) & 7); fr < hi; fr += 8)
       dma_piece16(reinterpret_cast<const char*>(wsrc + (size_t)R::src_frag(fr) * 512 + lane * 8), lds_addr(WL) + fr * 1024);
   };
-  constexpr int SET2_REAL = R::pieces(R::np(1)) + R::NF1 + R::NF2T + R::NF1T;
+  constexpr int NPX1 = MASKED ? 0 : R::pieces(R::np(1)), NW2 = (MASKED ? 0 : R::NF1) + R::NF2T + R::NF1T;
+  constexpr int SET2_REAL = NPX1 + NW2;
   constexpr int SET2 = (SET2_REAL + 7) / 8 * 8;
   stage_w(wb, R::L_W3T, R::L_W3T + R::NF3, 0);
   stage_region(DY, dyb, ty0 - 2, tx0 - 2, R::rw(0), R::np(0), 6);
   {
-    constexpr int NPX1 = R::pieces(R::np(1));
 #pragma unroll 1
     for (int p = wave; p < SET2; p += 8) {
       if (p < NPX1) {
@@ -262,7 +294,7 @@
         if (px_ < R::np(1) && Y >= 0 && Y < H && X >= 0 && X < W) sp = reinterpret_cast<const char*>(xb + img + ((size_t)Y * W + X) * C::F + lc * 8);
         dma_piece16(sp, lds_addr(XB) + p * (R::PXP * C::FC * 16));
       } else {
-        const int k0 = p - NPX1, k = k0 < R::NF1 + R::NF2T + R::NF1T ? k0 : 0, fr = k < R::NF1 ? k : R::L_W2T + (k - R::NF1);
+        const int k0 = p - NPX1, k = k0 < NW2 ? k0 : 0, fr = MASKED ? R::L_W2T + k : (k < R::NF1 ? k : R::L_W2T + (k - R::NF1));
         dma_piece16(reinterpret_cast<const char*>(wb + (size_t)R::src_frag(fr) * 512 + lane * 8), lds_addr(WL) + fr * 1024);
       }
     }
@@ -280,13 +312,21 @@
   SR_STAMP();
 
   BwP1<R> w1;
-  BwP2<R> w2;
+  BwP2<R, MASKED> w2;
   w1.load(WL, lane);
   auto pf2 = [&](int lo, int hi) {
 #pragma unroll
-    for (int i = 0; i < BwP2<R>::N; ++i)
+    for (int i = 0; i < BwP2<R, MASKED>::N; ++i)
       if (i >= lo && i < hi) w2.load_one(WL, lane, i);
   };
+  constexpr int NPAD1 = R::npad(1), NPAD2 = R::npad(2);
+  static_assert(!MASKED || (FwdMaskCfg<C>::NPAD_B == NPAD1 && NPAD2 == C::TH * C::TW && BwMask<R>::NMW == FwdMaskCfg<C>::NWORDS),
+                "the mask planes of the forward kernel");
+  const unsigned* const mb_tile = MASKED ? mb + tile_g * FwdMaskCfg<C>::TILE_WORDS : nullptr;
+  const unsigned* const ma_tile = MASKED ? ma + tile_g * FwdMaskCfg<C>::TILE_WORDS : nullptr;
+  BwMask<R> mk;
+  static_assert((R::np(1) + 31) / 32 >= R::NW && (R::np(2) + 31) / 32 >= R::NW, "every wave has a first tile in both P2 phases");
+  if constexpr (MASKED) mk.template load<NPAD1>(mb_tile, wave, lane);
   __bf16* const dtb_tile = dtb ? dtb + tile_g * (C::TH * C::TW) * C::LP : nullptr;
   __bf16* const dta_tile = dta ? dta + tile_g * (C::TH * C::TW) * C::LP : nullptr;
   bw_phase_dt<R, R::rw(1), R::np(1), 1>(DY, DT, w1, dtb_tile, H, W, ty0, tx0, wave, lane, [](int, int) {});
@@ -296,23 +336,42 @@
   __syncthreads();
   w2.load(WL, lane);
   __syncthreads();
-  stage_w(wa, 0, R::NFR, 0);
-  SR_STAMP();
-  bw_phase_dx<R, R::rw(1), R::np(1), 1>(XB, ONES, DT, DY, DX, dxb + img, w2, H, W, ty0, tx0, wave, lane);
+  stage_w(wa, MASKED ? R::NF1 : 0, R::NFR, 0);
+  SR_STAMP();
+  bw_phase_dx<R, R::rw(1), R::np(1), 1, MASKED>(XB, ONES, DT, DY, DX, dxb + img, w2, H, W, ty0, tx0, wave, lane, mb_tile, &mk);
   SR_STAMP();
   static_assert((R::np(1) + 31) / 32 >= R::NW, "every wave stores at least one tile of dx_b after its weight pieces");
   wait_vmcnt<3>();
   __syncthreads();
   SR_STAMP();
-  stage_region(DY, xa, ty0, tx0, R::rw(2), R::np(2), 0);
+  if constexpr (MASKED) mk.template load<NPAD2>(ma_tile, wave, lane);
+  else stage_region(DY, xa, ty0, tx0, R::rw(2), R::np(2), 0);
   w1.load(WL, lane);
   bw_phase_dt<R, R::rw(2), R::np(2), 0>(DX, DT, w1, dta_tile, H, W, ty0, tx0, wave, lane, pf2);
   SR_STAMP();
   static_assert((R::np(2) + 31) / 32 >= R::NW, "every wave has a tile of dt_a");
-  if (dta_tile) wait_vmcnt<3>();
-  else wait_vmcnt<0>();
-  __syncthreads();
-  SR_STAMP();
-  bw_phase_dx<R, R::rw(2), R::np(2), 0>(DY, ONES, DT, DX, nullptr, dxa + img, w2, H, W, ty0, tx0, wave, lane);
-  SR_STAMP();
-}
+  if constexpr (!MASKED) {
+    if (dta_tile) wait_vmcnt<3>();
+    else wait_vmcnt<0>();
+  }
+  __syncthreads();
+  SR_STAMP();
+  bw_phase_dx<R, R::rw(2), R::np(2), 0, MASKED>(DY, ONES, DT, DX, nullptr, dxa + img, w2, H, W, ty0, tx0, wave, lane, ma_tile, &mk);
+  SR_STAMP();
+}
+template <int F, int E, int L>
+__global__ __launch_bounds__(512) void wdsr_bwd_rs_kernel(const __bf16* __restrict__ xa, const __bf16* __restrict__ xb,
+                                                          const __bf16* __restrict__ dyb, __bf16* __restrict__ dxb,
+                                                          __bf16* __restrict__ dxa, const __bf16* __restrict__ wa,
+                                                          const __bf16* __restrict__ wb, __bf16* __restrict__ dta,
+                                                          __bf16* __restrict__ dtb, int H, int W, int tiles_x) {
+  wdsr_bwd_rs_body<F, E, L, false>(xa, xb, dyb, dxb, dxa, wa, wb, dta, dtb, H, W, tiles_x, nullptr, nullptr);
+}
+template <int F, int E, int L>
+__global__ __launch_bounds__(512) void wdsr_bwd_rs_mask_kernel(const unsigned* __restrict__ ma, const unsigned* __restrict__ mb,
+                                                               const __bf16* __restrict__ dyb, __bf16* __restrict__ dxb,
+                                                               __bf16* __restrict__ dxa, const __bf16* __restrict__ wa,
+                                                               const __bf16* __restrict__ wb, __bf16* __restrict__ dta,
+                                                               __bf16* __restrict__ dtb, int H, int W, int tiles_x) {
+  wdsr_bwd_rs_body<F, E, L, true>(nullptr, nullptr, dyb, dxb, dxa, wa, wb, dta, dtb, H, W, tiles_x, ma, mb);
+}
diff --git a/mobilesuperresolution_amd/csrc/wdsr_fwd_rs.h b/mobilesuperresolution_amd/csrc/wdsr_fwd_rs.h
--- a/mobilesuperresolution_amd/csrc/wdsr_fwd_rs.h
+++ b/mobilesuperresolution_amd/csrc/wdsr_fwd_rs.h
@@ -85,8 +85,30 @@
   }
 };
 
-template <typename C, int PFN = 0, typename PF>
-SR_DEV f32x16 rw_t_tile(const bf16x8 (&xb)[C::KS1], const RwA<C>& w, const float* cl, int hh, PF pf) {
+template <typename C> struct RwMask {
+  static constexpr int NWORDS = (C::NET + 1) / 2;
+  static constexpr int pos(int et, int s, int j) { return 8 * (et & 1) + 4 * s + j; }
+  unsigned w[NWORDS];
+};
+template <typename C> SR_DEV void rw_mask_frag(RwMask<C>& mk, const bf16x8& f, int et, int s) {
+  typedef __attribute__((ext_vector_type(4))) unsigned u32x4_;
+  typedef __attribute__((ext_vector_type(2))) unsigned short u16x2_;
+  const u32x4_ q = __builtin_bit_cast(u32x4_, f);
+  unsigned one_bits;
+  asm("s_mov_b32 %0, 0x00010001" : "=s"(one_bits));
+  const u16x2_ one = __builtin_bit_cast(u16x2_, one_bits);
+#pragma unroll
+  for (int j = 0; j < 4; ++j) {
+    const unsigned qj = q[j];
+    const unsigned m = __builtin_bit_cast(unsigned, __builtin_elementwise_min(__builtin_bit_cast(u16x2_, qj), one));
+    const int p = RwMask<C>::pos(et, s, j);
+    mk.w[et / 2] = p == 0 ? m : ((m << p) | mk.w[et / 2]);
+  }
+}
+struct RwNoMask {};
+template <typename C, int PFN = 0, bool MASK = false, typename PF>
+SR_DEV f32x16 rw_t_tile(const bf16x8 (&xb)[C::KS1], const RwA<C>& w, const float* cl, int hh, PF pf,
+                        std::conditional_t<MASK, RwMask<C>, RwNoMask>* mk = nullptr) {
   typedef __attribute__((ext_vector_type(8))) short s16x8;
   f32x16 tacc = load_cinit(cl, hh);
   auto conv1_step = [&](f32x16 acc, int et, int s) { return mma16<__bf16>(w.w1[et * C::KS1 + s], xb[s], acc); };
@@ -126,6 +148,10 @@
     bf16x8 f1 = cvt4(h, 8);
     if (2 * et < C::KS2) tacc = mma16<__bf16>(w.w2[2 * et], f0, tacc);
     f1prev = relu8(f1);
+    if constexpr (MASK) {
+      rw_mask_frag<C>(*mk, f0, et, 0);
+      if (2 * et + 1 < C::KS2) rw_mask_frag<C>(*mk, f1prev, et, 1);
+    }
     h = hn;
 #pragma unroll
     for (int k = 0; k < 4; ++k) {
@@ -155,6 +181,15 @@
   p.tso = core ? ((hy - HALO) * C::TW + hx - HALO) * C::LP : -1;
   return p;
 }
+template <typename C, int MASKM, int NPADM>
+SR_DEV void rw_store_mask(const RwMask<C>& mk, const RwPix& p, unsigned* mtile, int hh) {
+  constexpr int PLANE = (MASKM == 1 ? C::TH * C::TW : NPADM) * 2;
+  const int row = MASKM == 1 ? p.tso / C::LP : p.hp;
+  if (MASKM == 2 || p.tso >= 0) {
+#pragma unroll
+    for (int q = 0; q < RwMask<C>::NWORDS; ++q) stream_store(mtile + q * PLANE + row * 2 + hh, mk.w[q]);
+  }
+}
 template <typename C, bool SAVE_T>
 SR_DEV void rw_store_t(const f32x16& tacc, const RwPix& p, __bf16* TT, __bf16* tsave_tile, int hh) {
   bf16x4 v[C::CPT];
@@ -190,10 +225,13 @@
   }
 }
 
-template <typename C, int KXL, int RW, int NP, int HALO, int NW, bool SAVE_T, typename PF, typename BS>
+template <typename C, int KXL, int RW, int NP, int HALO, int NW, bool SAVE_T, typename PF, typename BS, int MASKM = 0>
 SR_DEV void rw_phase_a(const __bf16* Xin, const __bf16* ones, __bf16* TT, const RwA<C>& w, const float* cl, __bf16* tsave_tile,
-                       int H, int W, int ty0, int tx0, int wave, int lane, PF prefetch, BS before_stores) {
-  constexpr int NT = (NP + 31) / 32;
+                       int H, int W, int ty0, int tx0, int wave, int lane, PF prefetch, BS before_stores,
+                       std::integral_constant<int, MASKM> = {}, unsigned* mtile = nullptr) {
+  constexpr int NT = (NP + 31) / 32, NPADM = NT * 32;
+  constexpr bool MASK = MASKM != 0;
+  std::conditional_t<MASK, RwMask<C>, RwNoMask> mk;
   const int r = lane & 31, hh = lane >> 5;
   if (wave >= NT) {
     prefetch(0, 64);
@@ -206,7 +244,7 @@
   SR_STAMP_AT(11);
   constexpr int PFN = 4;
   {
-    const f32x16 t = rw_t_tile<C, PFN>(xb, w, cl, hh, [&](int et) { prefetch(et * PFN, et * PFN + PFN); });
+    const f32x16 t = rw_t_tile<C, PFN, MASK>(xb, w, cl, hh, [&](int et) { prefetch(et * PFN, et * PFN + PFN); }, &mk);
     SR_STAMP_AT(12);
     const RwPix pc = p;
     if (wave + NW < NT) {
@@ -216,17 +254,19 @@
     prefetch(C::NET * PFN, 64);
     before_stores();
     rw_store_t<C, SAVE_T>(t, pc, TT, tsave_tile, hh);
+    if constexpr (MASK) rw_store_mask<C, MASKM, NPADM>(mk, pc, mtile, hh);
     SR_STAMP_AT(13);
   }
 #pragma unroll 1
   for (int tile = wave + NW; tile < NT; tile += NW) {
-    const f32x16 t = rw_t_tile<C>(xb, w, cl, hh, [](int) {});
+    const f32x16 t = rw_t_tile<C, 0, MASK>(xb, w, cl, hh, [](int) {}, &mk);
     const RwPix pc = p;
     if (tile + NW < NT) {
       p = rw_pix_a<C, RW, NP, HALO>((tile + NW) * 32 + r, H, W, ty0, tx0);
       rw_x_frags<C, KXL>(xb, Xin, ones, p.hp, hh);
     }
     rw_store_t<C, SAVE_T>(t, pc, TT, tsave_tile, hh);
+    if constexpr (MASK) rw_store_mask<C, MASKM, NPADM>(mk, pc, mtile, hh);
   }
 }
 
@@ -362,14 +402,21 @@
   SR_STAMP_AT(10);
 }
 
-template <int F, int E, int L, int NBLK, bool SAVE_T>
-__global__ __launch_bounds__(512) void wdsr_fwd_rs_kernel(const __bf16* __restrict__ x, __bf16* __restrict__ ya,
-                                                          __bf16* __restrict__ yb, const __bf16* __restrict__ wa,
-                                                          const __bf16* __restrict__ wb, const float* __restrict__ cia,
-                                                          const float* __restrict__ cib, __bf16* __restrict__ tsa,
-                                                          __bf16* __restrict__ tsb, int H, int W, int tiles_x) {
+template <typename C> struct FwdMaskCfg {
+  static constexpr int NWORDS = (C::NET + 1) / 2;
+  static constexpr int NPAD_B = ((C::TW + 2) * (C::TH + 2) + 31) / 32 * 32;
+  static constexpr int WORDS_A = NWORDS * C::TH * C::TW * 2, WORDS_B = NWORDS * NPAD_B * 2;
+  static constexpr int TILE_WORDS = WORDS_B;
+  static_assert(WORDS_A <= TILE_WORDS, "the core is the smaller region");
+};
+template <int F, int E, int L, int NBLK, bool SAVE_T, bool MASK>
+SR_DEV void wdsr_fwd_rs_body(const __bf16* __restrict__ x, __bf16* __restrict__ ya, __bf16* __restrict__ yb,
+                             const __bf16* __restrict__ wa, const __bf16* __restrict__ wb, const float* __restrict__ cia,
+                             const float* __restrict__ cib, __bf16* __restrict__ tsa, __bf16* __restrict__ tsb, int H, int W,
+                             int tiles_x, unsigned* __restrict__ ma, unsigned* __restrict__ mb) {
   typedef BlockCfg<F, E, L> C;
   typedef RsCfg<F, E, L, NBLK> R;
+  static_assert(!MASK || (SAVE_T && NBLK == 2), "the mask goes with the saved images of a pair");
   constexpr int NTHREADS = R::NTHREADS, NW = R::NWAVES;
   __shared__ __attribute__((aligned(16))) char smem_raw[R::LDS_BYTES];
   __bf16* const X0 = reinterpret_cast<__bf16*>(smem_raw);
@@ -438,8 +485,11 @@
     for (int i = 0; i < RwB<C>::N; ++i)
       if (i >= lo && i < hi) rwb.load_one(wl, lane, i);
   };
+  unsigned* const ma_tile = MASK ? ma + tile_g * FwdMaskCfg<C>::TILE_WORDS : nullptr;
+  unsigned* const mb_tile = MASK ? mb + tile_g * FwdMaskCfg<C>::TILE_WORDS : nullptr;
   rw_phase_a<C, KXL, R::rw(0), R::np(0), NBLK, NW, SAVE_T>(X0, ONES, TT, rwa, CL, tsa_tile, H, W, ty0, tx0, wave, lane,
-                                                             [&](int lo, int hi) { pf_b(WL, lo, hi); }, [] { wait_vmcnt<0>(); });
+                                                             [&](int lo, int hi) { pf_b(WL, lo, hi); }, [] { wait_vmcnt<0>(); },
+                                                             std::integral_constant<int, MASK ? 1 : 0>{}, ma_tile);
   SR_STAMP();
   __syncthreads();
   SR_STAMP();
@@ -452,13 +502,31 @@
     __syncthreads();
     SR_STAMP();
     rw_phase_a<C, KXL, R::rw(1), R::np(1), NBLK - 1, NW, SAVE_T>(X1, ONES, TT, rwa, CL + R::CL_FLOATS, tsb_tile, H, W, ty0, tx0, wave,
-                                                                 lane, [&](int lo, int hi) { pf_b(WL + R::W_ELEMS, lo, hi); }, [] {});
+                                                                 lane, [&](int lo, int hi) { pf_b(WL + R::W_ELEMS, lo, hi); }, [] {},
+                                                                 std::integral_constant<int, MASK ? 2 : 0>{}, mb_tile);
     SR_STAMP();
     __syncthreads();
     SR_STAMP();
     rw_phase_b<C, KXL, C::TW, C::TH * C::TW, 0, NW>(TT, X1, ONES, nullptr, yb + img, rwb, H, W, ty0, tx0, wave, lane, [](int, int) {});
   }
   SR_STAMP();
+}
+template <int F, int E, int L, int NBLK, bool SAVE_T>
+__global__ __launch_bounds__(512) void wdsr_fwd_rs_kernel(const __bf16* __restrict__ x, __bf16* __restrict__ ya,
+                                                          __bf16* __restrict__ yb, const __bf16* __restrict__ wa,
+                                                          const __bf16* __restrict__ wb, const float* __restrict__ cia,
+                                                          const float* __restrict__ cib, __bf16* __restrict__ tsa,
+                                                          __bf16* __restrict__ tsb, int H, int W, int tiles_x) {
+  wdsr_fwd_rs_body<F, E, L, NBLK, SAVE_T, false>(x, ya, yb, wa, wb, cia, cib, tsa, tsb, H, W, tiles_x, nullptr, nullptr);
+}
+template <int F, int E, int L>
+__global__ __launch_bounds__(512) void wdsr_fwd_rs_mask_kernel(const __bf16* __restrict__ x, __bf16* __restrict__ ya,
+                                                               __bf16* __restrict__ yb, const __bf16* __restrict__ wa,
+                                                               const __bf16* __restrict__ wb, const float* __restrict__ cia,
+                                                               const float* __restrict__ cib, __bf16* __restrict__ tsa,
+                                                               __bf16* __restrict__ tsb, int H, int W, int tiles_x,
+                                                               unsigned* __restrict__ ma, unsigned* __restrict__ mb) {
+  wdsr_fwd_rs_body<F, E, L, 2, true, true>(x, ya, yb, wa, wb, cia, cib, tsa, tsb, H, W, tiles_x, ma, mb);
 }
 
 template <typename C>
diff --git a/mobilesuperresolution_amd/models/basic_wdsr_b.py b/mobilesuperresolution_amd/models/basic_wdsr_b.py
--- a/mobilesuperresolution_amd/models/basic_wdsr_b.py
+++ b/mobilesuperresolution_amd/models/basic_wdsr_b.py
@@ -85,7 +85,7 @@
         return L.WdsrNet.from_buffer_copy(self.net)
 
     def call_net(self, x, flat, acts, out=None, dout=None, grads=None, gflat=None, side=None, dtsave=None, hr=None,
-                 kind=0, gscale=0.0) -> "L.WdsrNet":
+                 kind=0, gscale=0.0, hmask=None) -> "L.WdsrNet":
         net = self.call_struct()
         net.N, net.H, net.W = x.shape[0], x.shape[2], x.shape[3]
         net.flat, net.x, net.acts = flat.data_ptr(), x.data_ptr(), acts.data_ptr()
@@ -99,6 +99,8 @@
             net.tsave = side.data_ptr()
         if dtsave is not None:
             net.dtsave = dtsave.data_ptr()
+        if hmask is not None:
+            net.hmask = hmask.data_ptr()
         if hr is not None:
             net.hr, net.loss_kind, net.loss_gscale = hr.data_ptr(), kind, gscale
         return net
@@ -298,6 +300,15 @@
         lay = self.layout
         return (self.hot_dtype == torch.bfloat16 and lay.NB > 0 and os.environ.get("SR_RECOMPUTE_WGRAD", "0") != "1")
 
+    def _mask_buffer(self, x, side):
+        if side is None or self.layout.F != 24 or not getattr(self, "save_relu_mask", True):
+            return None
+        n, _, h, w = x.shape
+        words = L.lib().sr_wdsr_relu_mask_words(h, w)
+        if words <= 0:
+            raise L.HotpathError("sr_wdsr_relu_mask_words failed")
+        return torch.empty((self.layout.NB, n * words), dtype=torch.int32, device=x.device)
+
     def _side_shape(self, n, h, w):
         tiles = ((h + 11) // 12) * ((w + 23) // 24)
         return (self.layout.NB, n, tiles, 288, 24 if self.layout.F == 24 else 32)
@@ -388,8 +399,9 @@
                                       "DistributedDataParallel (forward / loss / backward / optimizer)")
         out, acts, side = self._forward_buffers(x, True)
         grads, gflat, dtsave = _backward_buffers(acts, flat, side)
+        hmask = self._mask_buffer(x, side)
         net = st.call_net(x, flat, acts, out=out, grads=grads, gflat=gflat, side=side, dtsave=dtsave, hr=hr,
-                          kind=self._LOSS_KINDS[kind], gscale=self._gscale(weight, out.numel()))
+                          kind=self._LOSS_KINDS[kind], gscale=self._gscale(weight, out.numel()), hmask=hmask)
         loss = torch.empty((), dtype=torch.float32, device=x.device)
         scal = state.next_scalars()
         import torch.distributed as dist
```
